# cv-stuttgart/PCFA

Measured on AMD Instinct MI355X. Metric: attack_steps_per_sec, higher is better.
Workload: dtype f32; 1 GPU; RAFT, 1 synthetic 436x1024 pair per GPU (padded 440x1024), disjoint delta, change_of_variables, delta_bound=0.005, zero target, L-BFGS max_iter=10; weights=random:1234, parallelism=pairs sharded 1/GPU, closure_launch=hipGraph replay

## Files before the change

### include/pcfa_hip.h

```cpp
#ifndef PCFA_HIP_H
#define PCFA_HIP_H

#include <stddef.h>
#include <stdint.h>

#ifdef __cplusplus
extern "C" {
#endif

#define PCFA_OK 0
#define PCFA_ERR_INVALID_ARG (-1)
#define PCFA_ERR_UNSUPPORTED (-2)
#define PCFA_ERR_WORKSPACE (-3)

#if defined(__GNUC__)
#define PCFA_API __attribute__((visibility("default")))
#else
#define PCFA_API
#endif

#define PCFA_MAX_LEVELS 8
#define PCFA_ABI_VERSION 2

#define PCFA_LOSS_AEE 0
#define PCFA_LOSS_MSE 1
#define PCFA_LOSS_COSIM 2

#define PCFA_BOX_CLIPPING 0
#define PCFA_BOX_CHANGE_OF_VARIABLES 1

PCFA_API int pcfa_abi_version(void);
PCFA_API int pcfa_timing_arm(void* start_event, void* stop_event, int nth);

PCFA_API int pcfa_null_launch(void* stream);
PCFA_API int pcfa_poison_lds(unsigned pattern, void* stream);
PCFA_API int pcfa_peek_lds(unsigned* out, int n, void* stream);
PCFA_API long long pcfa_calib_mfma_f32(float* scratch, int blocks, int iters, void* stream);
PCFA_API int pcfa_calib_copy(const float* src, float* dst, long long n_floats, void* stream);
PCFA_API const char* pcfa_status_string(int status);


PCFA_API long long pcfa_corr_slab_floats(int H, int W, int num_levels);
PCFA_API long long pcfa_corr_level_offset(int H, int W, int num_levels, int level, int* h_l, int* w_l);

PCFA_API long long pcfa_corr_tiled_index(int H, int W, int num_levels, int level, int y, int x);

PCFA_API int pcfa_corr_f2ext_fwd(const float* fmap2, float* f2ext, int B, int D, int H, int W,
                        int num_levels, void* stream);

PCFA_API int pcfa_corr_pyramid_fwd(const float* fmap1, const float* f2ext, float* pyr, int B, int D,
                          int H, int W, int num_levels, void* stream);

PCFA_API size_t pcfa_corr_pyramid_bwd_workspace_bytes(int B, int D, int H, int W, int num_levels);
PCFA_API int pcfa_corr_pyramid_bwd(const float* dpyr, const float* fmap1, const float* f2ext,
                          float* dfmap1, float* dfmap2, void* workspace, size_t workspace_bytes,
                          int B, int D, int H, int W, int num_levels, void* stream);
PCFA_API size_t pcfa_corr_pyramid_bwd_windows_workspace_bytes(int B, int D, int H, int W, int num_levels);
PCFA_API int pcfa_corr_pyramid_bwd_windows(const float* dpyr, const float* fmap1, const float* f2ext, float* dfmap1,
                                  float* dfmap2, void* workspace, size_t workspace_bytes,
                                  const float* const* coords, int n_coords, int radius, int B, int D, int H, int W,
                                  int num_levels, void* stream);

PCFA_API int pcfa_corr_lookup_fwd(const float* pyr, const float* coords, float* out, int B, int H, int W,
                         int num_levels, int radius, void* stream);

PCFA_API int pcfa_corr_lookup_bwd(float* dpyr, const float* coords, const float* grad_out, int B, int H,
                         int W, int num_levels, int radius, void* stream);

PCFA_API size_t pcfa_corr_ondemand_workspace_bytes(int B, int D, int H, int W, int num_levels);
PCFA_API int pcfa_corr_ondemand_prepare(const float* fmap1, const float* fmap2, void* workspace, int B, int D, int H,
                               int W, int num_levels, void* stream);
PCFA_API int pcfa_corr_ondemand_fwd(const void* workspace, const float* coords, float* out, int B, int D, int H, int W,
                           int num_levels, int radius, void* stream);
PCFA_API int pcfa_corr_ondemand_bwd(void* workspace, const float* coords, const float* grad_out, int accumulate, int B,
                           int D, int H, int W, int num_levels, int radius, void* stream);
PCFA_API int pcfa_corr_ondemand_finish(const void* workspace, float* dfmap1, float* dfmap2, int B, int D, int H, int W,
                              int num_levels, void* stream);

PCFA_API int pcfa_corr_ondemand_fwd_tiled(const void* workspace, const float* coords, float* out, int B, int D, int H,
                                 int W, int num_levels, int radius, void* stream);
PCFA_API int pcfa_corr_ondemand_bwd_tiled(void* workspace, const float* coords, const float* grad_out, int accumulate,
                                 int B, int D, int H, int W, int num_levels, int radius, void* stream);
PCFA_API int pcfa_corr_ondemand_tile_geometry(int* tile_w, int* tile_h, int* max_positions);
PCFA_API int pcfa_corr_ondemand_tile_routes(const void* workspace, int B, int D, int H, int W, int num_levels,
                                   int* counts, void* stream);

PCFA_API size_t pcfa_gemm_f32_workspace_bytes(int M, int N, int batch, int splits);
PCFA_API int pcfa_gemm_f32(const float* A, const float* B, float* C, int M, int N, int K, long long lda, long long ldb,
                  long long ldc, int a_kmajor, int b_kmajor, int batch, long long bsA, long long bsB, long long bsC,
                  float alpha, int splits, void* workspace, size_t workspace_bytes, void* stream);
PCFA_API size_t pcfa_gemm_bf16x3_workspace_bytes(int M, int N, int batch, int splits);
PCFA_API int pcfa_gemm_bf16x3(const float* A, const float* B, float* C, int M, int N, int K, long long lda,
                     long long ldb, long long ldc, int a_kmajor, int b_kmajor, int batch, long long bsA, long long bsB,
                     long long bsC, float alpha, int splits, void* workspace, size_t workspace_bytes, void* stream);
PCFA_API int pcfa_corr_pyramid_fwd_bf16x3(const float* fmap1, const float* f2ext, float* pyr, int B, int D, int H,
                                 int W, int num_levels, void* stream);
PCFA_API int pcfa_softmax_rows_fwd(const float* x, float* y, long long rows, int cols, void* stream);
PCFA_API int pcfa_softmax_rows_bwd(const float* y, const float* grad_y, float* grad_x, long long rows, int cols,
                          void* stream);

PCFA_API int pcfa_attn_stream_lse(const float* q, const float* k, float* lse, int BH, int N, int d, float scale,
                         void* stream);
PCFA_API int pcfa_attn_stream_fwd(const float* q, const float* k, const float* v, const float* lse, float* out, int BH,
                         int N, int d, float scale, void* stream);
PCFA_API int pcfa_attn_stream_dv(const float* q, const float* k, const float* g, const float* lse, float* dv, int BH,
                        int N, int d, float scale, void* stream);
PCFA_API int pcfa_attn_stream_delta(const float* g, const float* out, float* delta, long long rows, int d,
                           int accumulate, void* stream);
PCFA_API int pcfa_attn_stream_dqk(const float* q, const float* k, const float* lse, const float* G, const float* V,
                         const float* delta, float* dq, float* dk, int BH, int N, int d, int n, float scale,
                         void* stream);

PCFA_API long long pcfa_lookup_convc1_packed_floats(int Cout);
PCFA_API int pcfa_lookup_convc1_pack_weights(const float* weight, float* packed, int Cout, int Cin, void* stream);
PCFA_API int pcfa_lookup_convc1_fwd(const float* pyr, const float* coords, const float* packed, const float* bias,
                           float* out, int B, int H, int W, int num_levels, int radius, int Cout, int relu,
                           void* stream);
PCFA_API int pcfa_lookup_convc1_bwd(float* dpyr, const float* coords, const float* packed, const float* out,
                           const float* grad_out, int B, int H, int W, int num_levels, int radius, int Cout,
                           int relu, void* stream);

PCFA_API int pcfa_spatial_corr_out_size(int iH, int iW, int kH, int kW, int padH, int padW, int dilH,
                               int dilW, int dH, int dW, int* oH, int* oW);
PCFA_API int pcfa_spatial_corr_fwd(const float* in1, const float* in2, float* out, int B, int C, int iH,
                          int iW, int kH, int kW, int patchH, int patchW, int padH, int padW,
                          int dilH, int dilW, int dil_patchH, int dil_patchW, int dH, int dW,
                          void* stream);
PCFA_API int pcfa_spatial_corr_bwd(const float* in1, const float* in2, const float* grad_out,
                          float* grad_in1, float* grad_in2, int B, int C, int iH, int iW, int kH,
                          int kW, int patchH, int patchW, int padH, int padW, int dilH, int dilW,
                          int dil_patchH, int dil_patchW, int dH, int dW, void* stream);

PCFA_API int pcfa_cost_volume9_fwd(const float* in1, const float* in2, float* out, int B, int C, int iH, int iW,
                          float scale, float slope, void* stream);
PCFA_API int pcfa_cost_volume9_bwd(const float* in1, const float* in2, const float* fwd_out, const float* grad_out,
                          float* grad_in1, float* grad_in2, int B, int C, int iH, int iW, float scale,
                          float slope, void* stream);

PCFA_API int pcfa_flownet_corr_out_size(int H, int W, int pad_size, int kernel_size, int max_displacement,
                                        int stride1, int stride2, int* out_channels, int* oH, int* oW);
PCFA_API int pcfa_flownet_corr_fwd(const float* in1, const float* in2, float* out, int B, int C, int H, int W,
                                   int pad_size, int kernel_size, int max_displacement, int stride1, int stride2,
                                   void* stream);
PCFA_API int pcfa_flownet_corr_bwd(const float* in1, const float* in2, const float* grad_out, float* grad_in1,
                                   float* grad_in2, int B, int C, int H, int W, int pad_size, int kernel_size,
                                   int max_displacement, int stride1, int stride2, void* stream);
PCFA_API int pcfa_resample2d_fwd(const float* in1, const float* flow, float* out, int B, int C, int iH, int iW,
                                 int H, int W, int kernel_size, int bilinear, void* stream);
PCFA_API int pcfa_resample2d_bwd(const float* in1, const float* flow, const float* grad_out, float* grad_in1,
                                 float* grad_flow, int B, int C, int iH, int iW, int H, int W, int kernel_size,
                                 int bilinear, void* stream);
PCFA_API int pcfa_channelnorm_fwd(const float* in, float* out, int B, int C, long long plane, int norm_deg,
                                  void* stream);
PCFA_API int pcfa_channelnorm_bwd(const float* in, const float* out, const float* grad_out, float* grad_in, int B,
                                  int C, long long plane, int norm_deg, void* stream);


PCFA_API int pcfa_box_transform_fwd(const float* image, const float* delta, float* out, int B,
                           long long n_per_item, int change_of_variables, double eps_box,
                           float scale, void* stream);
PCFA_API int pcfa_box_transform_bwd(const float* image, const float* delta, const float* grad_out,
                           float* grad_image, float* grad_delta, int B, long long n_per_item,
                           int change_of_variables, double eps_box, float scale, void* stream);

PCFA_API int pcfa_pm1_pair_fwd(const float* image1, const float* image2, float* pair, float* ctx, int B, long long n,
                               void* stream);
PCFA_API int pcfa_pm1_pair_bwd(const float* grad_pair, const float* grad_ctx, float* grad_image1, float* grad_image2, int B,
                               long long n, void* stream);

PCFA_API int pcfa_extract_deltas_fwd(const float* nw_input, const float* image, float* delta,
                            long long n, int change_of_variables, double eps_box, void* stream);
PCFA_API int pcfa_extract_deltas_bwd(const float* nw_input, const float* grad_delta, float* grad_nw_input,
                            long long n, int change_of_variables, double eps_box, void* stream);

PCFA_API int pcfa_extract_deltas_joint_fwd(const float* nw_delta, const float* images_max,
                                  const float* images_min, float* delta, long long n,
                                  void* stream);
PCFA_API int pcfa_extract_deltas_joint_bwd(const float* nw_delta, const float* images_max,
                                  const float* images_min, const float* grad_delta,
                                  float* grad_nw_delta, long long n, void* stream);

PCFA_API int pcfa_fgsm_step(float* x1, float* x2, const float* g1, const float* g2, const float* img1, const float* img2,
                            float* d1, float* d2, float epsilon, int joint, long long n, void* stream);
PCFA_API int pcfa_fgsm_step_max_threads(void);

PCFA_API size_t pcfa_flow_loss_workspace_bytes(void);
PCFA_API int pcfa_flow_loss_fwd(const float* pred, const long long pred_strides[4], const float* target,
                       const long long target_strides[4], int B, int H, int W,
                       const float* delta1, long long n1, const float* delta2, long long n2,
                       float delta_bound, float mu, int f_type, float* out_scalars,
                       void* workspace, void* stream);
PCFA_API int pcfa_flow_loss_bwd(const float* pred, const long long pred_strides[4], const float* target,
                       const long long target_strides[4], int B, int H, int W,
                       const float* delta1, long long n1, const float* delta2, long long n2,
                       float mu, int f_type, int joint, const float* fwd_scalars,
                       const float* grad_loss, float* grad_pred, float* grad_delta1,
                       float* grad_delta2, void* stream);

PCFA_API int pcfa_gru_gates_fwd(const float* zc, const float* rc, const float* h, const float* bias_z,
                       const float* bias_r, const float* add_z, const float* add_r, float* z, float* r,
                       float* rh, long long n, int plane, int channels, void* stream);
PCFA_API int pcfa_gru_gates_bwd(const float* z, const float* r, const float* h, const float* dz, const float* drh,
                       float* dzc, float* drc, float* dh, long long n, void* stream);
PCFA_API int pcfa_gru_gates_bwd_acc(const float* z, const float* r, const float* h, const float* dz, const float* drh,
                           const float* dh_in, float* dzc, float* drc, float* dh, long long n, void* stream);
PCFA_API int pcfa_gru_update_fwd(const float* z, const float* qc, const float* h, const float* bias_q,
                        const float* add_q, float* q, float* hnew, long long n, int plane, int channels,
                        void* stream);
PCFA_API int pcfa_gru_update_bwd(const float* z, const float* q, const float* h, const float* g, float* dz,
                        float* dqc, float* dh, long long n, void* stream);

PCFA_API long long pcfa_sepconv5_packed_floats(int Cout, int Cin);
PCFA_API int pcfa_sepconv5_algo(int use_winograd);
PCFA_API int pcfa_sepconv5_uses_winograd(int B, int Ca, int Cb, int Cout, int H, int W, int vertical);
PCFA_API int pcfa_sepconv5_pack_weights(const float* w, float* fwd_packed, float* bwd_packed, int Cout, int Cin,
                               void* stream);
PCFA_API int pcfa_sepconv5_fwd(const float* in_a, int Ca, const float* in_b, int Cb, const float* w_packed,
                      float* out, int B, int Cout, int H, int W, int vertical, void* stream);

PCFA_API int pcfa_sepconv5_fwd_split(const float* in_a, int Ca, const float* in_b, int Cb, const float* w_packed,
                            float* out_a, int Cout_a, int accumulate_a, float* out_b, int accumulate_b, int B,
                            int Cout, int H, int W, int vertical, void* stream);
PCFA_API int pcfa_sepconv5_fwd_split_masked(const float* in_a, int Ca, const float* in_b, int Cb, const float* w_packed,
                                   float* out_a, int Cout_a, int accumulate_a, float* out_b, int accumulate_b,
                                   const float* mask_b, int mask_channels, int B, int Cout, int H, int W,
                                   int vertical, void* stream);

PCFA_API int pcfa_sepconv5_gru_gates_fwd(const float* h, int C, const float* rest, int Cr, const float* w_packed,
                                const float* add_zr, float* z, float* r, float* rh, int B, int H, int W,
                                int vertical, void* stream);
PCFA_API int pcfa_sepconv5_gru_update_fwd(const float* rh, int C, const float* rest, int Cr, const float* w_packed,
                                 const float* add_q, const float* z, const float* h, float* q, float* hnew, int B,
                                 int H, int W, int vertical, void* stream);
PCFA_API int pcfa_sepconv5_gru_gates_bwd(const float* dqc, int C, int Cr, const float* w_packed_bwd, const float* z,
                                const float* r, const float* h, const float* dz, const float* dh_in, float* dzr,
                                float* dh, float* d_rest, int accumulate_rest, int B, int H, int W, int vertical,
                                void* stream);
PCFA_API int pcfa_sepconv5_gru_update_bwd(const float* dzr, int C, int Cr, const float* w_packed_bwd, const float* dh_acc,
                                 const float* z_prev, const float* q_prev, const float* h_prev, float* dz_prev,
                                 float* dqc_prev, float* dh_prev, float* d_rest, int B, int H, int W, int vertical,
                                 void* stream);

PCFA_API long long pcfa_conv3x3_packed_floats(int K, int N);
PCFA_API int pcfa_conv3x3_pack_weights(const float* w, float* fwd_packed, float* bwd_packed, int Cout, int Cin,
                              void* stream);
PCFA_API int pcfa_conv3x3_fwd(const float* x, const float* packed, const float* bias, float* out, int B, int K, int N,
                     int H, int W, int relu, void* stream);
PCFA_API int pcfa_conv3x3_act_fwd(const float* x, const float* packed, const float* bias, float* out, int B, int K,
                         int N, int H, int W, int act, float slope, void* stream);
PCFA_API int pcfa_leaky_relu_fwd(const float* x, float* y, float slope, long long n, void* stream);
PCFA_API int pcfa_leaky_relu_bwd(const float* out, const float* grad_out, float* grad_x, float slope, long long n,
                        void* stream);
PCFA_API int pcfa_conv3x3_act_fwd_pair(const float* x, const float* packed, const float* bias, float* out, int K, int N,
                              const float* x2, const float* packed2, const float* bias2, float* out2, int K2, int N2,
                              int H, int W, int act, float slope, void* stream);
PCFA_API int pcfa_conv3x3_fused_bwd(const float* g, const float* packed_bwd, const float* mask, const float* addend,
                           float* grad_in, int B, int K, int N, int H, int W, void* stream);
PCFA_API int pcfa_conv3x3_masked_fwd(const float* x, const float* packed, const float* mask, float* out, int B, int K,
                            int N, int H, int W, void* stream);
PCFA_API int pcfa_conv3x3_algo(int B, int K, int N, int H, int W);
PCFA_API size_t pcfa_conv3x3_workspace_bytes(int B, int K, int N, int H, int W);
PCFA_API int pcfa_conv3x3_run(const float* x, const float* packed, const float* bias, const float* mask,
                     const float* addend, float* out, int B, int K, int N, int H, int W, int act, float slope,
                     int mask_channels, void* workspace, size_t workspace_bytes, void* stream);

PCFA_API int pcfa_bias_relu_fwd(const float* x, const float* bias, float* out, long long n, int plane, int channels,
                       void* stream);
PCFA_API int pcfa_relu_bwd(const float* out, const float* grad_out, float* grad_x, long long n, void* stream);
PCFA_API int pcfa_relu_bwd2(const float* out, const float* out2, const float* grad_out, float* grad_x, float* grad_x2,
                   long long n, void* stream);

PCFA_API int pcfa_conv_fewin_fwd(const float* x, const float* w, const float* bias, float* out, int B, int Cin, int N,
                                 int H, int W, int ksize, int relu, void* stream);
PCFA_API long long pcfa_conv_fewin_packed_floats(int Cin, int N, int ksize);
PCFA_API int pcfa_conv_fewin_pack(const float* w, float* packed, int Cin, int N, int ksize, void* stream);
PCFA_API int pcfa_conv_fewin_packed_fwd(const float* x, const float* packed, const float* bias, float* out, int B, int Cin,
                               int N, int H, int W, int ksize, int relu, void* stream);

PCFA_API int pcfa_conv_s2_supported(int Cin, int N, int ksize, int H, int W);
PCFA_API long long pcfa_conv_s2_packed_floats(int Cin, int N, int ksize);
PCFA_API int pcfa_conv_s2_pack(const float* w, float* packed, int Cin, int N, int ksize, void* stream);
PCFA_API int pcfa_conv_s2_fwd(const float* x, const float* packed, const float* bias, float* out, int B, int Cin, int N,
                              int H, int W, int ksize, int act, float slope, void* stream);
PCFA_API int pcfa_conv_s2_bwd_supported(int Cin, int N, int ksize, int H, int W);
PCFA_API long long pcfa_conv_s2_bwd_packed_floats(int Cin, int N, int ksize);
PCFA_API int pcfa_conv_s2_bwd_pack(const float* w, float* packed, int Cin, int N, int ksize, void* stream);
PCFA_API int pcfa_conv_s2_bwd(const float* grad_out, const float* packed, float* grad_x, int B, int Cin, int N, int H, int W,
                              int ksize, void* stream);
PCFA_API long long pcfa_conv_s2_ds_packed_floats(int Cin, int N);
PCFA_API int pcfa_conv_s2_ds_pack(const float* w, const float* wd, float* packed, int Cin, int N, void* stream);
PCFA_API int pcfa_conv_s2_ds_fwd(const float* x, const float* packed, const float* bias, float* out, const float* bias_d,
                                 float* out_d, int B, int Cin, int N, int H, int W, int act, float slope, void* stream);
PCFA_API long long pcfa_conv_s2_ds_bwd_packed_floats(int Cin, int N);
PCFA_API int pcfa_conv_s2_ds_bwd_pack(const float* w, const float* wd, float* packed, int Cin, int N, void* stream);
PCFA_API int pcfa_conv_s2_ds_bwd(const float* grad_out, const float* grad_out_d, const float* packed, float* grad_x, int B,
                                 int Cin, int N, int H, int W, void* stream);

PCFA_API int pcfa_pwc_warp_fwd(const float* x, const float* flo, float* out, int B, int C, int H, int W,
                               float mask_threshold, float flow_scale, void* stream);
PCFA_API int pcfa_pwc_warp_bwd(const float* x, const float* flo, const float* grad_out, float* grad_x,
                               float* grad_flo, int B, int C, int H, int W, float mask_threshold, float flow_scale,
                               void* stream);
PCFA_API size_t pcfa_pwc_warp_bwd_det_workspace_bytes(int B, int C, int H, int W);
PCFA_API int pcfa_pwc_warp_bwd_det(const float* x, const float* flo, const float* grad_out, float* grad_x,
                          float* grad_flo, void* workspace, size_t workspace_bytes, int B, int C, int H, int W,
                          float mask_threshold, float flow_scale, void* stream);

PCFA_API int pcfa_spynet_warp_fwd(const float* x, const float* flo, const float* hor, const float* ver, float* out, int B,
                                  int C, int H, int W, float sx, float sy, void* stream);
PCFA_API size_t pcfa_spynet_warp_bwd_workspace_bytes(int B, int C, int H, int W);
PCFA_API int pcfa_spynet_warp_bwd(const float* x, const float* flo, const float* hor, const float* ver,
                                  const float* grad_out, float* grad_x, float* grad_flo, void* workspace,
                                  size_t workspace_bytes, int B, int C, int H, int W, float sx, float sy, void* stream);

PCFA_API int pcfa_conv7x7_tile(int Cout, int* mt, int* cot);
PCFA_API long long pcfa_conv7x7_packed_floats(int Cin, int Cout);
PCFA_API int pcfa_conv7x7(const float* x, const float* mask, const float* packed, const float* bias, const float* addend,
                          float* out, int B, int Cin, int Cout, int H, int W, int relu, void* stream);

PCFA_API int pcfa_conv_gather_tile(int Cout, int* mt, int* cot);
PCFA_API int pcfa_conv_gather_supported(int stride, int taps, int npar);
PCFA_API long long pcfa_conv_gather_packed_floats(int Cin, int Cout, int taps, int npar);
PCFA_API int pcfa_conv_gather(const float* x, const float* mask, float mask_slope, const float* packed, const float* bias,
                              float* out, int B, int Cin, int H, int W, int Cout, int OH, int OW, int stride, int taps,
                              int npar, int off0, int off1, int act, float slope, void* stream);

PCFA_API size_t pcfa_resample2d_bwd_det_workspace_bytes(int B, int C, int H, int W);
PCFA_API int pcfa_resample2d_bwd_det(const float* in1, const float* flow, const float* grad_out, float* grad_in1,
                                     float* grad_flow, void* workspace, size_t workspace_bytes, int B, int C, int H, int W,
                                     void* stream);

PCFA_API int pcfa_upsample_nearest4_fwd(const float* in, float* out, int planes, int H, int W, float s, int div,
                                        void* stream);
PCFA_API int pcfa_upsample_nearest4_bwd(const float* grad_out, float* grad_in, int planes, int H, int W, float s, int div,
                                        void* stream);

PCFA_API size_t pcfa_conv3x3_fewout_workspace_bytes(int B, int K, int N, int H, int W);
PCFA_API int pcfa_conv3x3_fewout_fwd(const float* x, const float* w, const float* bias, float* out, void* workspace,
                                     int B, int K, int N, int H, int W, void* stream);
PCFA_API int pcfa_conv3x3_fewout_bwd(const float* grad_out, const float* w, const float* addend, float* grad_x, int B,
                                     int K, int N, int H, int W, void* stream);

PCFA_API size_t pcfa_deconv4s2_fewout_workspace_bytes(int B, int K, int N, int H, int W);
PCFA_API int pcfa_deconv4s2_fewout_fwd(const float* x, const float* w, const float* bias, float* out, void* workspace,
                                       int B, int K, int N, int H, int W, void* stream);
PCFA_API int pcfa_deconv4s2_fewout_bwd(const float* grad_out, const float* w, float* grad_x, int B, int K, int N, int H,
                                       int W, void* stream);

PCFA_API int pcfa_upsample_bilinear_fwd(const float* in, float* out, int planes, int H, int W, int factor, float mul,
                                        void* stream);
PCFA_API int pcfa_upsample_bilinear_bwd(const float* grad_out, float* grad_in, int planes, int H, int W, int factor,
                                        float mul, void* stream);

PCFA_API size_t pcfa_instnorm_workspace_bytes(int planes, long long plane);
PCFA_API int pcfa_instnorm_fwd(const float* x, float* y, float* mean_rstd, void* workspace, int planes,
                               long long plane, float eps, int relu, void* stream);
PCFA_API int pcfa_instnorm_bwd(const float* x, const float* mean_rstd, const float* grad_out, float* grad_x,
                               void* workspace, int planes, long long plane, int relu, void* stream);
PCFA_API int pcfa_add_relu_fwd(const float* a, const float* b, float* out, long long n, void* stream);
PCFA_API int pcfa_convex_upsample_fwd(const float* flow, const float* mask, float* out, int N, int H, int W, void* stream);
PCFA_API long long pcfa_convex_upsample_workspace_floats(int N, int H, int W);
PCFA_API int pcfa_convex_upsample_bwd(const float* flow, const float* mask, const float* grad_out, float* grad_flow,
                             float* grad_mask, float* workspace, int N, int H, int W, void* stream);

PCFA_API int pcfa_flow_step(const float* coords1, const float* delta, const float* coords0, float* coords1_new,
                   float* flow_new, long long n, void* stream);

PCFA_API int pcfa_sum_n(const float* const* srcs, int n, float* out, long long numel, void* stream);

PCFA_API int pcfa_avg_epe(const float* flow1, const long long strides1[4], const float* flow2,
                 const long long strides2[4], int B, int H, int W, float* out, void* workspace,
                 void* stream);
PCFA_API int pcfa_sum_squares(const float* x, long long n, float* out, void* workspace, void* stream);

PCFA_API size_t pcfa_lbfgs_workspace_floats(void);
PCFA_API int pcfa_lbfgs_pair(const float* g, float* g_prev, const float* d, float t, float* y_out, float* s_out,
                             float* scal4, float* workspace, int update_prev, long long n, void* stream);
PCFA_API int pcfa_lbfgs_direction(const float* g, const float* S, const float* Y, const float* ro, const float* H,
                                  float* al, float* d, float* workspace, int first, int count, int capacity,
                                  long long ld, long long n, void* stream);

PCFA_API size_t pcfa_lbfgs_gram_state_bytes(int capacity);
PCFA_API size_t pcfa_lbfgs_gram_workspace_bytes(int capacity, long long ld);
PCFA_API int pcfa_lbfgs_gram_reset(void* state, int capacity, void* stream);
PCFA_API int pcfa_lbfgs_gram_update(const float* g, float* g_prev, const float* d, float t, float* S, float* Y,
                                    void* state, void* workspace, int capacity, long long ld, void* stream);
PCFA_API int pcfa_lbfgs_gram_direction(const float* g, const float* S, const float* Y, void* state, float* d,
                                       float* out_gtd_dmax, void* workspace, int capacity, long long ld, void* stream);

#ifdef __cplusplus
}
#endif
#endif
```

### pcfa_amd/_hip.py

```python
import ctypes
import os
from ctypes import c_char_p, c_double, c_float, c_int, c_longlong, c_size_t, c_uint, c_void_p, POINTER

ABI_VERSION = 2
LIB_PATH = os.environ.get("PCFA_HIP_LIB") or os.path.join(os.path.dirname(os.path.abspath(__file__)), "lib",
                                                          "libpcfa_hip.so")

PCFA_LOSS = {"aee": 0, "mse": 1, "cosim": 2}


class HipLibraryError(RuntimeError):
    pass


_P = c_void_p
_S4 = POINTER(c_longlong)

SIGNATURES = {
    "pcfa_abi_version": (c_int, []),
    "pcfa_timing_arm": (c_int, [_P, _P, c_int]),
    "pcfa_null_launch": (c_int, [_P]),
    "pcfa_poison_lds": (c_int, [c_uint, _P]),
    "pcfa_peek_lds": (c_int, [_P, c_int, _P]),
    "pcfa_calib_mfma_f32": (c_longlong, [_P, c_int, c_int, _P]),
    "pcfa_calib_copy": (c_int, [_P, _P, c_longlong, _P]),
    "pcfa_status_string": (c_char_p, [c_int]),
    "pcfa_corr_slab_floats": (c_longlong, [c_int, c_int, c_int]),
    "pcfa_corr_level_offset": (c_longlong, [c_int, c_int, c_int, c_int, POINTER(c_int), POINTER(c_int)]),
    "pcfa_corr_tiled_index": (c_longlong, [c_int, c_int, c_int, c_int, c_int, c_int]),
    "pcfa_corr_f2ext_fwd": (c_int, [_P, _P, c_int, c_int, c_int, c_int, c_int, _P]),
    "pcfa_corr_pyramid_fwd": (c_int, [_P, _P, _P, c_int, c_int, c_int, c_int, c_int, _P]),
    "pcfa_corr_pyramid_bwd_workspace_bytes": (c_size_t, [c_int, c_int, c_int, c_int, c_int]),
    "pcfa_corr_pyramid_bwd": (c_int, [_P, _P, _P, _P, _P, _P, c_size_t, c_int, c_int, c_int, c_int, c_int, _P]),
    "pcfa_corr_pyramid_bwd_windows_workspace_bytes": (c_size_t, [c_int, c_int, c_int, c_int, c_int]),
    "pcfa_corr_pyramid_bwd_windows": (c_int, [_P, _P, _P, _P, _P, _P, c_size_t, POINTER(c_void_p), c_int, c_int, c_int,
                                              c_int, c_int, c_int, c_int, _P]),
    "pcfa_corr_lookup_fwd": (c_int, [_P, _P, _P, c_int, c_int, c_int, c_int, c_int, _P]),
    "pcfa_corr_lookup_bwd": (c_int, [_P, _P, _P, c_int, c_int, c_int, c_int, c_int, _P]),
    "pcfa_corr_ondemand_workspace_bytes": (c_size_t, [c_int, c_int, c_int, c_int, c_int]),
    "pcfa_corr_ondemand_prepare": (c_int, [_P, _P, _P, c_int, c_int, c_int, c_int, c_int, _P]),
    "pcfa_corr_ondemand_fwd": (c_int, [_P, _P, _P, c_int, c_int, c_int, c_int, c_int, c_int, _P]),
    "pcfa_corr_ondemand_bwd": (c_int, [_P, _P, _P, c_int, c_int, c_int, c_int, c_int, c_int, c_int, _P]),
    "pcfa_corr_ondemand_finish": (c_int, [_P, _P, _P, c_int, c_int, c_int, c_int, c_int, _P]),
    "pcfa_corr_ondemand_fwd_tiled": (c_int, [_P, _P, _P, c_int, c_int, c_int, c_int, c_int, c_int, _P]),
    "pcfa_corr_ondemand_bwd_tiled": (c_int, [_P, _P, _P, c_int, c_int, c_int, c_int, c_int, c_int, c_int, _P]),
    "pcfa_corr_ondemand_tile_geometry": (c_int, [POINTER(c_int), POINTER(c_int), POINTER(c_int)]),
    "pcfa_corr_ondemand_tile_routes": (c_int, [_P, c_int, c_int, c_int, c_int, c_int, _P, _P]),
    "pcfa_gemm_f32_workspace_bytes": (c_size_t, [c_int, c_int, c_int, c_int]),
    "pcfa_gemm_f32": (c_int, [_P, _P, _P, c_int, c_int, c_int, c_longlong, c_longlong, c_longlong, c_int, c_int, c_int,
                              c_longlong, c_longlong, c_longlong, c_float, c_int, _P, c_size_t, _P]),
    "pcfa_gemm_bf16x3_workspace_bytes": (c_size_t, [c_int, c_int, c_int, c_int]),
    "pcfa_gemm_bf16x3": (c_int, [_P, _P, _P, c_int, c_int, c_int, c_longlong, c_longlong, c_longlong, c_int, c_int,
                                 c_int, c_longlong, c_longlong, c_longlong, c_float, c_int, _P, c_size_t, _P]),
    "pcfa_corr_pyramid_fwd_bf16x3": (c_int, [_P, _P, _P, c_int, c_int, c_int, c_int, c_int, _P]),
    "pcfa_softmax_rows_fwd": (c_int, [_P, _P, c_longlong, c_int, _P]),
    "pcfa_softmax_rows_bwd": (c_int, [_P, _P, _P, c_longlong, c_int, _P]),
    "pcfa_attn_stream_lse": (c_int, [_P, _P, _P, c_int, c_int, c_int, c_float, _P]),
    "pcfa_attn_stream_fwd": (c_int, [_P, _P, _P, _P, _P, c_int, c_int, c_int, c_float, _P]),
    "pcfa_attn_stream_dv": (c_int, [_P, _P, _P, _P, _P, c_int, c_int, c_int, c_float, _P]),
    "pcfa_attn_stream_delta": (c_int, [_P, _P, _P, c_longlong, c_int, c_int, _P]),
    "pcfa_attn_stream_dqk": (c_int, [_P, _P, _P, _P, _P, _P, _P, _P, c_int, c_int, c_int, c_int, c_float, _P]),
    "pcfa_lookup_convc1_packed_floats": (c_longlong, [c_int]),
    "pcfa_lookup_convc1_pack_weights": (c_int, [_P, _P, c_int, c_int, _P]),
    "pcfa_lookup_convc1_fwd": (c_int, [_P, _P, _P, _P, _P, c_int, c_int, c_int, c_int, c_int, c_int, c_int, _P]),
    "pcfa_lookup_convc1_bwd": (c_int, [_P, _P, _P, _P, _P, c_int, c_int, c_int, c_int, c_int, c_int, c_int, _P]),
    "pcfa_spatial_corr_out_size": (c_int, [c_int] * 10 + [POINTER(c_int), POINTER(c_int)]),
    "pcfa_spatial_corr_fwd": (c_int, [_P, _P, _P] + [c_int] * 16 + [_P]),
    "pcfa_spatial_corr_bwd": (c_int, [_P, _P, _P, _P, _P] + [c_int] * 16 + [_P]),
    "pcfa_cost_volume9_fwd": (c_int, [_P, _P, _P, c_int, c_int, c_int, c_int, c_float, c_float, _P]),
    "pcfa_cost_volume9_bwd": (c_int, [_P, _P, _P, _P, _P, _P, c_int, c_int, c_int, c_int, c_float, c_float, _P]),
    "pcfa_flownet_corr_out_size": (c_int, [c_int] * 7 + [POINTER(c_int)] * 3),
    "pcfa_flownet_corr_fwd": (c_int, [_P, _P, _P] + [c_int] * 9 + [_P]),
    "pcfa_flownet_corr_bwd": (c_int, [_P, _P, _P, _P, _P] + [c_int] * 9 + [_P]),
    "pcfa_resample2d_fwd": (c_int, [_P, _P, _P] + [c_int] * 8 + [_P]),
    "pcfa_resample2d_bwd": (c_int, [_P, _P, _P, _P, _P] + [c_int] * 8 + [_P]),
    "pcfa_channelnorm_fwd": (c_int, [_P, _P, c_int, c_int, c_longlong, c_int, _P]),
    "pcfa_channelnorm_bwd": (c_int, [_P, _P, _P, _P, c_int, c_int, c_longlong, c_int, _P]),
    "pcfa_box_transform_fwd": (c_int, [_P, _P, _P, c_int, c_longlong, c_int, c_double, c_float, _P]),
    "pcfa_box_transform_bwd": (c_int, [_P, _P, _P, _P, _P, c_int, c_longlong, c_int, c_double, c_float, _P]),
    "pcfa_pm1_pair_fwd": (c_int, [_P, _P, _P, _P, c_int, c_longlong, _P]),
    "pcfa_pm1_pair_bwd": (c_int, [_P, _P, _P, _P, c_int, c_longlong, _P]),
    "pcfa_extract_deltas_fwd": (c_int, [_P, _P, _P, c_longlong, c_int, c_double, _P]),
    "pcfa_extract_deltas_bwd": (c_int, [_P, _P, _P, c_longlong, c_int, c_double, _P]),
    "pcfa_extract_deltas_joint_fwd": (c_int, [_P, _P, _P, _P, c_longlong, _P]),
    "pcfa_extract_deltas_joint_bwd": (c_int, [_P, _P, _P, _P, _P, c_longlong, _P]),
    "pcfa_fgsm_step": (c_int, [_P] * 8 + [c_float, c_int, c_longlong, _P]),
    "pcfa_fgsm_step_max_threads": (c_int, []),
    "pcfa_flow_loss_workspace_bytes": (c_size_t, []),
    "pcfa_flow_loss_fwd": (c_int, [_P, _S4, _P, _S4, c_int, c_int, c_int, _P, c_longlong, _P, c_longlong,
                                   c_float, c_float, c_int, _P, _P, _P]),
    "pcfa_flow_loss_bwd": (c_int, [_P, _S4, _P, _S4, c_int, c_int, c_int, _P, c_longlong, _P, c_longlong,
                                   c_float, c_int, c_int, _P, _P, _P, _P, _P, _P]),
    "pcfa_gru_gates_fwd": (c_int, [_P] * 10 + [c_longlong, c_int, c_int, _P]),
    "pcfa_gru_gates_bwd": (c_int, [_P] * 8 + [c_longlong, _P]),
    "pcfa_gru_update_fwd": (c_int, [_P] * 7 + [c_longlong, c_int, c_int, _P]),
    "pcfa_gru_update_bwd": (c_int, [_P] * 7 + [c_longlong, _P]),
    "pcfa_sepconv5_packed_floats": (c_longlong, [c_int, c_int]),
    "pcfa_sepconv5_algo": (c_int, [c_int]),
    "pcfa_sepconv5_uses_winograd": (c_int, [c_int] * 7),
    "pcfa_sepconv5_pack_weights": (c_int, [_P, _P, _P, c_int, c_int, _P]),
    "pcfa_sepconv5_fwd": (c_int, [_P, c_int, _P, c_int, _P, _P, c_int, c_int, c_int, c_int, c_int, _P]),
    "pcfa_sepconv5_fwd_split": (c_int, [_P, c_int, _P, c_int, _P, _P, c_int, c_int, _P, c_int, c_int, c_int, c_int, c_int,
                                        c_int, _P]),
    "pcfa_gru_gates_bwd_acc": (c_int, [_P, _P, _P, _P, _P, _P, _P, _P, _P, c_longlong, _P]),
    "pcfa_sepconv5_fwd_split_masked": (c_int, [_P, c_int, _P, c_int, _P, _P, c_int, c_int, _P, c_int, _P, c_int, c_int,
                                               c_int, c_int, c_int, c_int, _P]),
    "pcfa_sepconv5_gru_gates_fwd": (c_int, [_P, c_int, _P, c_int, _P, _P, _P, _P, _P, c_int, c_int, c_int, c_int, _P]),
    "pcfa_sepconv5_gru_update_fwd": (c_int, [_P, c_int, _P, c_int, _P, _P, _P, _P, _P, _P, c_int, c_int, c_int, c_int, _P]),
    "pcfa_sepconv5_gru_gates_bwd": (c_int, [_P, c_int, c_int, _P, _P, _P, _P, _P, _P, _P, _P, _P, c_int, c_int, c_int,
                                            c_int, c_int, _P]),
    "pcfa_sepconv5_gru_update_bwd": (c_int, [_P, c_int, c_int, _P, _P, _P, _P, _P, _P, _P, _P, _P, c_int, c_int, c_int,
                                             c_int, _P]),
    "pcfa_convex_upsample_fwd": (c_int, [_P, _P, _P, c_int, c_int, c_int, _P]),
    "pcfa_convex_upsample_workspace_floats": (c_longlong, [c_int, c_int, c_int]),
    "pcfa_convex_upsample_bwd": (c_int, [_P, _P, _P, _P, _P, _P, c_int, c_int, c_int, _P]),
    "pcfa_flow_step": (c_int, [_P, _P, _P, _P, _P, c_longlong, _P]),
    "pcfa_conv3x3_act_fwd_pair": (c_int, [_P, _P, _P, _P, c_int, c_int, _P, _P, _P, _P, c_int, c_int, c_int, c_int, c_int,
                                          c_float, _P]),
    "pcfa_relu_bwd2": (c_int, [_P, _P, _P, _P, _P, c_longlong, _P]),
    "pcfa_conv3x3_fused_bwd": (c_int, [_P, _P, _P, _P, _P, c_int, c_int, c_int, c_int, c_int, _P]),
    "pcfa_conv3x3_masked_fwd": (c_int, [_P, _P, _P, _P, c_int, c_int, c_int, c_int, c_int, _P]),
    "pcfa_conv3x3_algo": (c_int, [c_int] * 5),
    "pcfa_conv3x3_workspace_bytes": (c_size_t, [c_int] * 5),
    "pcfa_conv3x3_run": (c_int, [_P] * 6 + [c_int] * 6 + [c_float, c_int, _P, c_size_t, _P]),
    "pcfa_conv3x3_packed_floats": (c_longlong, [c_int, c_int]),
    "pcfa_conv3x3_pack_weights": (c_int, [_P, _P, _P, c_int, c_int, _P]),
    "pcfa_conv3x3_fwd": (c_int, [_P, _P, _P, _P, c_int, c_int, c_int, c_int, c_int, c_int, _P]),
    "pcfa_conv3x3_act_fwd": (c_int, [_P, _P, _P, _P, c_int, c_int, c_int, c_int, c_int, c_int, c_float, _P]),
    "pcfa_leaky_relu_fwd": (c_int, [_P, _P, c_float, c_longlong, _P]),
    "pcfa_leaky_relu_bwd": (c_int, [_P, _P, _P, c_float, c_longlong, _P]),
    "pcfa_lbfgs_gram_state_bytes": (c_size_t, [c_int]),
    "pcfa_lbfgs_gram_workspace_bytes": (c_size_t, [c_int, c_longlong]),
    "pcfa_lbfgs_gram_reset": (c_int, [_P, c_int, _P]),
    "pcfa_lbfgs_gram_update": (c_int, [_P, _P, _P, c_float, _P, _P, _P, _P, c_int, c_longlong, _P]),
    "pcfa_lbfgs_gram_direction": (c_int, [_P, _P, _P, _P, _P, _P, _P, c_int, c_longlong, _P]),
    "pcfa_lbfgs_workspace_floats": (c_size_t, []),
    "pcfa_lbfgs_pair": (c_int, [_P, _P, _P, c_float, _P, _P, _P, _P, c_int, c_longlong, _P]),
    "pcfa_lbfgs_direction": (c_int, [_P, _P, _P, _P, _P, _P, _P, _P, c_int, c_int, c_int, c_longlong, c_longlong,
                                     _P]),
    "pcfa_bias_relu_fwd": (c_int, [_P, _P, _P, c_longlong, c_int, c_int, _P]),
    "pcfa_relu_bwd": (c_int, [_P, _P, _P, c_longlong, _P]),
    "pcfa_conv_fewin_packed_floats": (c_longlong, [c_int, c_int, c_int]),
    "pcfa_conv_s2_supported": (c_int, [c_int, c_int, c_int, c_int, c_int]),
    "pcfa_conv_s2_packed_floats": (c_longlong, [c_int, c_int, c_int]),
    "pcfa_conv_s2_pack": (c_int, [_P, _P, c_int, c_int, c_int, _P]),
    "pcfa_conv_s2_fwd": (c_int, [_P, _P, _P, _P, c_int, c_int, c_int, c_int, c_int, c_int, c_int, c_float, _P]),
    "pcfa_conv_s2_bwd_supported": (c_int, [c_int, c_int, c_int, c_int, c_int]),
    "pcfa_conv_s2_bwd_packed_floats": (c_longlong, [c_int, c_int, c_int]),
    "pcfa_conv_s2_bwd_pack": (c_int, [_P, _P, c_int, c_int, c_int, _P]),
    "pcfa_conv_s2_bwd": (c_int, [_P, _P, _P, c_int, c_int, c_int, c_int, c_int, c_int, _P]),
    "pcfa_conv_s2_ds_packed_floats": (c_longlong, [c_int, c_int]),
    "pcfa_conv_s2_ds_pack": (c_int, [_P, _P, _P, c_int, c_int, _P]),
    "pcfa_conv_s2_ds_fwd": (c_int, [_P, _P, _P, _P, _P, _P, c_int, c_int, c_int, c_int, c_int, c_int, c_float, _P]),
    "pcfa_conv_s2_ds_bwd_packed_floats": (c_longlong, [c_int, c_int]),
    "pcfa_conv_s2_ds_bwd_pack": (c_int, [_P, _P, _P, c_int, c_int, _P]),
    "pcfa_conv_s2_ds_bwd": (c_int, [_P, _P, _P, _P, c_int, c_int, c_int, c_int, c_int, _P]),
    "pcfa_conv_fewin_pack": (c_int, [_P, _P, c_int, c_int, c_int, _P]),
    "pcfa_conv_fewin_packed_fwd": (c_int, [_P, _P, _P, _P, c_int, c_int, c_int, c_int, c_int, c_int, c_int, _P]),
    "pcfa_conv_fewin_fwd": (c_int, [_P, _P, _P, _P, c_int, c_int, c_int, c_int, c_int, c_int, c_int, _P]),
    "pcfa_pwc_warp_fwd": (c_int, [_P, _P, _P, c_int, c_int, c_int, c_int, c_float, c_float, _P]),
    "pcfa_pwc_warp_bwd": (c_int, [_P, _P, _P, _P, _P, c_int, c_int, c_int, c_int, c_float, c_float, _P]),
    "pcfa_pwc_warp_bwd_det_workspace_bytes": (c_size_t, [c_int, c_int, c_int, c_int]),
    "pcfa_pwc_warp_bwd_det": (c_int, [_P, _P, _P, _P, _P, _P, c_size_t, c_int, c_int, c_int, c_int, c_float, c_float, _P]),
    "pcfa_conv3x3_fewout_workspace_bytes": (c_size_t, [c_int, c_int, c_int, c_int, c_int]),
    "pcfa_conv3x3_fewout_fwd": (c_int, [_P, _P, _P, _P, _P, c_int, c_int, c_int, c_int, c_int, _P]),
    "pcfa_conv3x3_fewout_bwd": (c_int, [_P, _P, _P, _P, c_int, c_int, c_int, c_int, c_int, _P]),
    "pcfa_deconv4s2_fewout_workspace_bytes": (c_size_t, [c_int, c_int, c_int, c_int, c_int]),
    "pcfa_deconv4s2_fewout_fwd": (c_int, [_P, _P, _P, _P, _P, c_int, c_int, c_int, c_int, c_int, _P]),
    "pcfa_deconv4s2_fewout_bwd": (c_int, [_P, _P, _P, c_int, c_int, c_int, c_int, c_int, _P]),
    "pcfa_spynet_warp_fwd": (c_int, [_P, _P, _P, _P, _P, c_int, c_int, c_int, c_int, c_float, c_float, _P]),
    "pcfa_spynet_warp_bwd_workspace_bytes": (c_size_t, [c_int, c_int, c_int, c_int]),
    "pcfa_spynet_warp_bwd": (c_int, [_P, _P, _P, _P, _P, _P, _P, _P, c_size_t, c_int, c_int, c_int, c_int, c_float, c_float,
                                     _P]),
    "pcfa_conv7x7_tile": (c_int, [c_int, POINTER(c_int), POINTER(c_int)]),
    "pcfa_conv7x7_packed_floats": (c_longlong, [c_int, c_int]),
    "pcfa_conv7x7": (c_int, [_P, _P, _P, _P, _P, _P, c_int, c_int, c_int, c_int, c_int, c_int, _P]),
    "pcfa_conv_gather_tile": (c_int, [c_int, POINTER(c_int), POINTER(c_int)]),
    "pcfa_conv_gather_supported": (c_int, [c_int, c_int, c_int]),
    "pcfa_conv_gather_packed_floats": (c_longlong, [c_int, c_int, c_int, c_int]),
    "pcfa_conv_gather": (c_int, [_P, _P, c_float, _P, _P, _P] + [c_int] * 12 + [c_int, c_float, _P]),
    "pcfa_resample2d_bwd_det_workspace_bytes": (c_size_t, [c_int, c_int, c_int, c_int]),
    "pcfa_resample2d_bwd_det": (c_int, [_P, _P, _P, _P, _P, _P, c_size_t, c_int, c_int, c_int, c_int, _P]),
    "pcfa_upsample_nearest4_fwd": (c_int, [_P, _P, c_int, c_int, c_int, c_float, c_int, _P]),
    "pcfa_upsample_nearest4_bwd": (c_int, [_P, _P, c_int, c_int, c_int, c_float, c_int, _P]),
    "pcfa_upsample_bilinear_fwd": (c_int, [_P, _P, c_int, c_int, c_int, c_int, c_float, _P]),
    "pcfa_upsample_bilinear_bwd": (c_int, [_P, _P, c_int, c_int, c_int, c_int, c_float, _P]),
    "pcfa_instnorm_workspace_bytes": (c_size_t, [c_int, c_longlong]),
    "pcfa_instnorm_fwd": (c_int, [_P, _P, _P, _P, c_int, c_longlong, c_float, c_int, _P]),
    "pcfa_instnorm_bwd": (c_int, [_P, _P, _P, _P, _P, c_int, c_longlong, c_int, _P]),
    "pcfa_add_relu_fwd": (c_int, [_P, _P, _P, c_longlong, _P]),
    "pcfa_sum_n": (c_int, [POINTER(c_void_p), c_int, _P, c_longlong, _P]),
    "pcfa_avg_epe": (c_int, [_P, _S4, _P, _S4, c_int, c_int, c_int, _P, _P, _P]),
    "pcfa_sum_squares": (c_int, [_P, c_longlong, _P, _P, _P]),
}

_lib = None


def load(path=None):
    global _lib
    if _lib is not None and path is None:
        return _lib
    p = path or LIB_PATH
    if not os.path.exists(p):
        raise HipLibraryError(
            "libpcfa_hip.so not found at %s -- build it with `python -c 'import __graft_entry__ as g; g.build()'` "
            "or `make -C pcfa_amd/csrc`. pcfa_amd has no CPU fallback." % p)
    try:
        lib = ctypes.CDLL(p)
    except OSError as e:
        raise HipLibraryError("cannot load %s: %s" % (p, e))
    for name, (res, args) in SIGNATURES.items():
        try:
            fn = getattr(lib, name)
        except AttributeError:
            raise HipLibraryError("%s does not export %s (stale build?)" % (p, name))
        fn.restype = res
        fn.argtypes = args
    v = lib.pcfa_abi_version()
    if v != ABI_VERSION:
        raise HipLibraryError("ABI version mismatch: library %d, binding %d" % (v, ABI_VERSION))
    if path is None:
        _lib = lib
    return lib


def check(status, what):
    if status != 0:
        msg = load().pcfa_status_string(status)
        raise RuntimeError("%s failed: %s (status %d)" % (what, msg.decode() if msg else "?", status))


def strides4(t):
    return (c_longlong * 4)(*t.stride())
```

### pcfa_amd/config.py

```python
import dataclasses
import os


def _env_bool(name, default):
    v = os.environ.get(name)
    return default if v is None else v not in ("0", "", "false", "False")


@dataclasses.dataclass(frozen=True)
class Config:
    fused_lookup: bool = True
    overlap_encoders: bool = False
    conv_s2: bool = True
    conv_s2_bwd: bool = True
    fused_downsample: bool = True
    defer_relu: bool = True
    pyramid_bwd_windows: bool = True
    gma_gemm: str = "lib"
    gma_attention: str = "materialised"
    conv1x1: str = "lib"
    corr: str = "all_pairs"
    ondemand_lookup: str = "per_query"
    mfma: str = "f32"
    dilated_as_subgrids: tuple = (2, 4, 8, 16)
    deconv_fewout: bool = True
    defer_leaky: bool = True
    dense_block_fused_masks: bool = True
    warp_bwd_deterministic: bool = True
    pwc_fold_glue: bool = True
    spynet_ops: str = "lib"
    flownet2_ops: str = "lib"
    reuse_pair_graphs: bool = True
    max_cached_shapes: int = 4

    @classmethod
    def from_env(cls):
        return cls(fused_lookup=_env_bool("PCFA_FUSED_LOOKUP", True),
                   overlap_encoders=_env_bool("PCFA_OVERLAP_ENCODERS", False),
                   defer_relu=_env_bool("PCFA_DEFER_RELU", True),
                   gma_gemm=os.environ.get("PCFA_GMA_GEMM", "lib"),
                   gma_attention=os.environ.get("PCFA_GMA_ATTENTION", "materialised"),
                   conv1x1=os.environ.get("PCFA_CONV1X1", "lib"),
                   corr=os.environ.get("PCFA_CORR", "all_pairs"),
                   ondemand_lookup=os.environ.get("PCFA_ONDEMAND_LOOKUP", "per_query"),
                   mfma=os.environ.get("PCFA_MFMA", "f32"),
                   spynet_ops=os.environ.get("PCFA_SPYNET_OPS", "lib"),
                   flownet2_ops=os.environ.get("PCFA_FLOWNET2_OPS", "lib"),
                   max_cached_shapes=int(os.environ.get("PCFA_MAX_CACHED_SHAPES", "4")))

    def __post_init__(self):
        if self.gma_gemm not in ("lib", "hip"):
            raise ValueError("Config.gma_gemm must be 'lib' or 'hip', got %r" % (self.gma_gemm,))
        if self.gma_attention not in ("materialised", "streamed"):
            raise ValueError("Config.gma_attention must be 'materialised' or 'streamed', got %r" % (self.gma_attention,))
        if self.conv1x1 not in ("lib", "hip"):
            raise ValueError("Config.conv1x1 must be 'lib' or 'hip', got %r" % (self.conv1x1,))
        if self.corr not in ("all_pairs", "on_demand"):
            raise ValueError("Config.corr must be 'all_pairs' or 'on_demand', got %r" % (self.corr,))
        if self.ondemand_lookup not in ("per_query", "tiled"):
            raise ValueError("Config.ondemand_lookup must be 'per_query' or 'tiled', got %r" % (self.ondemand_lookup,))
        if self.mfma not in ("f32", "bf16x3"):
            raise ValueError("Config.mfma must be 'f32' or 'bf16x3', got %r" % (self.mfma,))
        if self.spynet_ops not in ("lib", "hip"):
            raise ValueError("Config.spynet_ops must be 'lib' or 'hip', got %r" % (self.spynet_ops,))
        if self.flownet2_ops not in ("lib", "hip"):
            raise ValueError("Config.flownet2_ops must be 'lib' or 'hip', got %r" % (self.flownet2_ops,))
        if self.max_cached_shapes < 1:
            raise ValueError("Config.max_cached_shapes must be >= 1")


DEFAULT = Config.from_env()


def attach(model, config=None):
    config = DEFAULT if config is None else config
    if not isinstance(config, Config):
        raise TypeError("config must be a pcfa_amd.config.Config")
    for m in model.modules():
        object.__setattr__(m, "_pcfa_config", config)
    return model


def cfg(module):
    return getattr(module, "_pcfa_config", DEFAULT)
```

### pcfa_amd/csrc/conv3x3.hip

```cpp
#include "common.hpp"
#include "conv3x3_f43.hpp"
#include "conv_tail.hpp"
#include <cstdlib>

namespace {

typedef float f32x16 __attribute__((ext_vector_type(16)));

constexpr int TC = 8;
constexpr int PC = 2 * TC + 2;
constexpr int PCP = 20;
constexpr int KC = 8;
constexpr int CB = 64;

__global__ void conv3x3_pack_kernel(const float* __restrict__ w, float* __restrict__ P, int Cout, int Cin,
                                    int backward, int K, int N, int nchunk, long long total) {
  for (long long e = (long long)blockIdx.x * blockDim.x + threadIdx.x; e < total;
       e += (long long)gridDim.x * blockDim.x) {
    const int pos = (int)(e & 15), lane = (int)((e >> 4) & 63), wv = (int)((e >> 10) & 3);
    const long long blk = e >> 12;
    const int c = (int)(blk % nchunk), nb = (int)(blk / nchunk);
    const int a = pos >> 2, kpi = pos & 3;
    const int i = wv, j = a;
    const int k = 8 * c + 2 * kpi + (lane >> 5), n = 32 * nb + (lane & 31);
    float g[3][3];
#pragma unroll
    for (int p = 0; p < 3; ++p)
#pragma unroll
      for (int q = 0; q < 3; ++q) {
        float v = 0.f;
        if (n < N && k < K) v = backward ? w[(((long long)k * Cin + n) * 3 + (2 - p)) * 3 + (2 - q)]
                                         : w[(((long long)n * Cin + k) * 3 + p) * 3 + q];
        g[p][q] = v;
      }
    float r[3];
#pragma unroll
    for (int q = 0; q < 3; ++q)
      r[q] = i == 0 ? g[0][q] : i == 1 ? 0.5f * (g[0][q] + g[1][q] + g[2][q])
                              : i == 2 ? 0.5f * (g[0][q] - g[1][q] + g[2][q]) : g[2][q];
    P[e] = j == 0 ? r[0] : j == 1 ? 0.5f * (r[0] + r[1] + r[2]) : j == 2 ? 0.5f * (r[0] - r[1] + r[2]) : r[2];
  }
}

#ifdef PCFA_C3_STAMPS
__device__ unsigned long long c3_stamp_sums[8];
__device__ __forceinline__ unsigned long long c3_now() {
  unsigned long long t;
  __builtin_amdgcn_sched_barrier(0);
  asm volatile("s_memtime %0\n\ts_waitcnt lgkmcnt(0)" : "=s"(t)::"memory");
  __builtin_amdgcn_sched_barrier(0);
  return t;
}
#define C3_STAMP(k)                                                                              \
  do {                                                                                           \
    const unsigned long long now_ = c3_now();                                                    \
    if (k != 0) stamp_acc[k] += now_ - stamp_prev;                                               \
    stamp_prev = now_;                                                                           \
  } while (0)
#else
#define C3_STAMP(k) do {} while (0)
#endif

struct Second {
  const float* x;
  const float* U;
  const float* bias;
  float* out;
  int K, N, nb0;
  int mask_n;
  int ksl;
  int cper;
  PcfaXcdMap xcd;
};

template <int ACT, int CBT, int MT, bool KFULL, int NRING, int KS = 1>
__global__ __launch_bounds__(256 * MT * KS) __attribute__((amdgpu_waves_per_eu(KS == 2 ? 2 : (MT == 1 && NRING == 2 && CBT == 32 ? 3 : (CBT == 64 ? 1 : 2))))) void conv3x3_winograd_kernel(
    const float* __restrict__ x, const float* __restrict__ U, const float* __restrict__ bias,
    const float* __restrict__ mask, const float* __restrict__ addend, float* __restrict__ out, int K, int N, int Npad,
    int H, int W, int blocks_x, float slope, Second second) {
  constexpr int NT = 256 * MT;
  constexpr int TR = 4 * MT, TB = TR * TC;
  constexpr int PR = 2 * TR + 2;
  constexpr int RAW = KC * PR * PCP;
  constexpr int RAW_LOADS = (KC * PR * PC + NT - 1) / NT;
  constexpr int MS = TB + 1;
  constexpr int NB = CBT / 32;
  static_assert(KS == 1 || (KS == 2 && MT == 1 && CBT == 32), "split-K rides on the 256-thread tile");
  constexpr int EPI = 16 * 16 * (TB + 1);
  constexpr int RED = KS == 2 ? 4 * 4 * 16 * 64 : 0;
  constexpr int LDS0 = 2 * KS * RAW > EPI ? 2 * KS * RAW : EPI;
  constexpr int LDSF = RED > LDS0 ? RED : LDS0;
  __shared__ __attribute__((aligned(16))) float smem[LDSF];
  const int kgrp = KS == 1 ? 0 : (int)(threadIdx.x >> 8);
  float* sRaw = smem + kgrp * 2 * RAW;

  const int tid = KS == 1 ? (int)threadIdx.x : (int)(threadIdx.x & 255);
  const int lane = tid & 63, wave = (tid >> 6) & 3, mt = tid >> 8;
  const int l31 = lane & 31, lh = lane >> 5;
  int tileblk = blockIdx.x, nby = blockIdx.y;
  if (second.xcd.a != 0 && !pcfa_xcd_item(second.xcd, (int)blockIdx.x, tileblk, nby)) return;
  const int by = tileblk / blocks_x, bx = tileblk - by * blocks_x;
  const int y0 = by * (2 * TR), x0 = bx * (2 * TC);
  if (nby >= second.nb0) {
    nby -= second.nb0;
    x = second.x;
    U = second.U;
    bias = second.bias;
    out = second.out;
    K = second.K;
    N = second.N;
    mask = nullptr;
    addend = nullptr;
  }
  const int mask_n = second.mask_n;
  const int n0 = nby * CBT;
  if (n0 >= N) return;
  const long long plane = (long long)H * W;
  const int ksl = second.ksl, img = blockIdx.z / ksl, slice = blockIdx.z - img * ksl;
  x += (long long)img * K * plane;
  out += ((long long)slice * (gridDim.z / ksl) + img) * N * plane;
  if (mask != nullptr) mask += (long long)img * N * plane;
  if (addend != nullptr) addend += (long long)img * N * plane;

  unsigned praw[RAW_LOADS];
  int rdst[RAW_LOADS];
  int rch[RAW_LOADS];
  bool rok[RAW_LOADS];
#pragma unroll
  for (int i = 0; i < RAW_LOADS; ++i) {
    const int e = tid + NT * i;
    const int ch = e / (PR * PC), rem = e - ch * (PR * PC);
    const int r = rem / PC, c = rem - r * PC;
    const int yy = y0 - 1 + r, xx = x0 - 1 + c;
    rch[i] = min(ch, KC - 1);
    rdst[i] = e < KC * PR * PC ? (ch * PR + r) * PCP + c : PC;
    rok[i] = e < KC * PR * PC && yy >= 0 && yy < H && xx >= 0 && xx < W;
    praw[i] = (unsigned)(min(max(yy, 0), H - 1) * W + min(max(xx, 0), W - 1) + (KFULL ? rch[i] * (int)plane : 0));
  }
  static_assert(CBT == 32, "the packed weight layout is per 32-channel block");
  const int nchunk = (K + KC - 1) / KC;
  const float* pu = U + (((long long)nby * nchunk * 4 + wave) * 64 + lane) * 16;

  float ring_raw[NRING][RAW_LOADS];
  float4 ring_u[NRING][4];
  auto load_u = [&](int c0, float4 (&ru)[4]) {
    const float4* q = reinterpret_cast<const float4*>(pu + (long long)(c0 / KC) * (4 * 64 * 16));
#pragma unroll
    for (int i = 0; i < 4; ++i) ru[i] = q[i];
  };
  auto load_raw = [&](int c0, float (&rraw)[RAW_LOADS]) {
    if (KFULL) {
      const unsigned xo = (unsigned)(c0 * (int)plane);
#pragma unroll
      for (int i = 0; i < RAW_LOADS; ++i)
#ifdef PCFA_C3_TIMING_NO_RAW
        rraw[i] = (float)(praw[i] + xo);
#else
        rraw[i] = x[praw[i] + xo];
#endif
    } else {
#pragma unroll
      for (int i = 0; i < RAW_LOADS; ++i)
        rraw[i] = x[praw[i] + (unsigned)(min(c0 + rch[i], K - 1) * (int)plane)];
    }
  };
  auto store_chunk = [&](int c0, int buf, const float (&rraw)[RAW_LOADS]) {
    float* sRawb = sRaw + buf * RAW;
#pragma unroll
    for (int i = 0; i < RAW_LOADS; ++i)
      sRawb[rdst[i]] = (rok[i] && (KFULL || c0 + rch[i] < K)) ? rraw[i] : 0.f;
  };
  f32x16 acc[4][NB];
#pragma unroll
  for (int a = 0; a < 4; ++a)
#pragma unroll
    for (int b = 0; b < NB; ++b)
#pragma unroll
      for (int r = 0; r < 16; ++r) acc[a][b][r] = 0.f;

  const int ra = wave == 0 ? 0 : 1, rb = wave == 3 ? 3 : 2;
  const float sa = wave == 2 ? -1.f : 1.f, sb = (wave == 1 || wave == 2) ? 1.f : -1.f;
  const int m_tile = mt * 32 + l31;
  const float* prow = sRaw + (lh * PR + 2 * (m_tile >> 3)) * PCP + 2 * (m_tile & 7);
  auto load_chunk = [&](int c0, float (&rraw)[RAW_LOADS], float4 (&ru)[4]) {
    load_u(c0, ru);
    load_raw(c0, rraw);
  };
  auto mfma_chunk = [&](int buf, const float4 (&ru)[4], auto&& mid1, auto&& mid2) {
    const float* p0 = prow + buf * RAW;
    float2 a0 = *reinterpret_cast<const float2*>(p0 + ra * PCP), a1 = *reinterpret_cast<const float2*>(p0 + ra * PCP + 2);
    float2 b0 = *reinterpret_cast<const float2*>(p0 + rb * PCP), b1 = *reinterpret_cast<const float2*>(p0 + rb * PCP + 2);
#pragma unroll
    for (int kp = 0; kp < KC; kp += 2) {
      float2 na0 = a0, na1 = a1, nb0 = b0, nb1 = b1;
      if (kp + 2 < KC) {
        const float* p = p0 + (kp + 2) * (PR * PCP);
        na0 = *reinterpret_cast<const float2*>(p + ra * PCP);
        na1 = *reinterpret_cast<const float2*>(p + ra * PCP + 2);
        nb0 = *reinterpret_cast<const float2*>(p + rb * PCP);
        nb1 = *reinterpret_cast<const float2*>(p + rb * PCP + 2);
        __builtin_amdgcn_sched_barrier(0);
      }
      const float t0 = fmaf(sb, b0.x, sa * a0.x), t1 = fmaf(sb, b0.y, sa * a0.y);
      const float t2 = fmaf(sb, b1.x, sa * a1.x), t3 = fmaf(sb, b1.y, sa * a1.y);
      const float av[4] = {t0 - t2, t1 + t2, t2 - t1, t1 - t3};
#pragma unroll
      for (int a = 0; a < 4; ++a) {
        const float bv = kp == 0 ? ru[a].x : kp == 2 ? ru[a].y : kp == 4 ? ru[a].z : ru[a].w;
        acc[a][0] = __builtin_amdgcn_mfma_f32_32x32x2f32(av[a], bv, acc[a][0], 0, 0, 0);
      }
      if (kp == 0) {
        mid1();
        __builtin_amdgcn_sched_barrier(0);
      } else if (kp == 2) {
        mid2();
        __builtin_amdgcn_sched_barrier(0);
      }
      a0 = na0; a1 = na1; b0 = nb0; b1 = nb1;
    }
  };

  const int cbeg = ksl > 1 ? slice * second.cper : 0, cend = ksl > 1 ? min(nchunk, cbeg + second.cper) : nchunk;
  const int nchunk_g = (cend - cbeg) / KS;
  auto gc0 = [&](int cl) { return (cbeg + cl * KS + kgrp) * KC; };
  const int lastc = gc0(nchunk_g - 1);
#ifdef PCFA_C3_STAMPS
  unsigned long long stamp_prev = 0, stamp_acc[5] = {0, 0, 0, 0, 0};
#endif
#pragma unroll
  for (int j = 0; j < NRING; ++j) load_chunk(min(gc0(j), lastc), ring_raw[j], ring_u[j]);
  store_chunk(gc0(0), 0, ring_raw[0]);
  __syncthreads();
  for (int cbase = 0; cbase < nchunk_g; cbase += NRING) {
#pragma unroll
    for (int j = 0; j < NRING; ++j) {
      const int c = cbase + j;
      if (c < nchunk_g) {
        const int cur = c & 1, nxt = cur ^ 1;
        C3_STAMP(0);
        mfma_chunk(cur, ring_u[j],
                   [&] {
                     store_chunk(gc0(c + 1), nxt, ring_raw[(j + 1) % NRING]);
                     load_u(min(gc0(c - 1 + NRING), lastc), ring_u[(j + NRING - 1) % NRING]);
                   },
                   [&] { load_raw(min(gc0(c + NRING), lastc), ring_raw[j]); });
        __builtin_amdgcn_sched_barrier(0);
        C3_STAMP(1);
        C3_STAMP(2);
        C3_STAMP(3);
        __syncthreads();
        C3_STAMP(4);
      }
    }
  }

#ifdef PCFA_C3_STAMPS
  if (lane == 0 && wave == 0) {
    for (int k = 1; k < 5; ++k) atomicAdd(&c3_stamp_sums[k], stamp_acc[k]);
    atomicAdd(&c3_stamp_sums[0], (unsigned long long)nchunk);
  }
#endif
  if (KS == 2) {
    float* red = smem;
    if (kgrp == 1) {
#pragma unroll
      for (int a = 0; a < 4; ++a)
#pragma unroll
        for (int r = 0; r < 16; ++r) red[((wave * 4 + a) * 16 + r) * 64 + lane] = acc[a][0][r];
    }
    __syncthreads();
    if (kgrp == 0) {
#pragma unroll
      for (int a = 0; a < 4; ++a)
#pragma unroll
        for (int r = 0; r < 16; ++r) acc[a][0][r] += red[((wave * 4 + a) * 16 + r) * 64 + lane];
    }
    __syncthreads();
  }
  const bool worker = kgrp == 0;
  static_assert(EPI == 16 * 16 * MS, "epilogue image size");
  float* sM = smem;
  const int e_tile = tid % TB, e_cl = tid / TB;
  const int e_tr = e_tile >> 3, e_tc = e_tile & 7;
  const int oy = y0 + 2 * e_tr, ox = x0 + 2 * e_tc;
#pragma unroll
  for (int pass = 0; pass < CBT / 16; ++pass) {
    const int nb = pass >> 1, half = pass & 1;
    float mk[2][4] = {{1.f, 1.f, 1.f, 1.f}, {1.f, 1.f, 1.f, 1.f}};
    float ad[2][4] = {{0.f, 0.f, 0.f, 0.f}, {0.f, 0.f, 0.f, 0.f}};
    if (addend != nullptr && worker) {
#pragma unroll
      for (int q = 0; q < 2; ++q) {
        const int n = n0 + pass * 16 + e_cl + 8 * q;
        if (n < N && oy < H && ox < W) {
          const float* ap = addend + (long long)n * plane + (long long)oy * W + ox;
          ad[q][0] = ap[0];
          if (ox + 1 < W) ad[q][1] = ap[1];
          if (oy + 1 < H) {
            ad[q][2] = ap[W];
            if (ox + 1 < W) ad[q][3] = ap[W + 1];
          }
        }
      }
    }
    if (mask != nullptr && worker) {
#pragma unroll
      for (int q = 0; q < 2; ++q) {
        const int n = n0 + pass * 16 + e_cl + 8 * q;
        if (n < N && (mask_n == 0 || n < mask_n) && oy < H && ox < W) {
          const float* mp = mask + (long long)n * plane + (long long)oy * W + ox;
          mk[q][0] = mp[0];
          if (ox + 1 < W) mk[q][1] = mp[1];
          if (oy + 1 < H) {
            mk[q][2] = mp[W];
            if (ox + 1 < W) mk[q][3] = mp[W + 1];
          }
        }
      }
    }
    if ((l31 >> 4) == half && worker) {
      const int cl = l31 & 15;
#pragma unroll
      for (int a = 0; a < 4; ++a) {
        float* m = &sM[((wave * 4 + a) * 16 + cl) * MS];
#pragma unroll
        for (int r = 0; r < 16; ++r) m[mt * 32 + (r & 3) + 8 * (r >> 2) + 4 * lh] = acc[a][nb][r];
      }
    }
    __syncthreads();
#pragma unroll
    for (int q = 0; q < 2; ++q) {
      const int cl = e_cl + 8 * q;
      const int n = n0 + pass * 16 + cl;
      float m[16];
#pragma unroll
      for (int xi = 0; xi < 16; ++xi) m[xi] = sM[(xi * 16 + cl) * MS + e_tile];
      float t0[4], t1[4];
#pragma unroll
      for (int j = 0; j < 4; ++j) {
        t0[j] = m[j] + m[4 + j] + m[8 + j];
        t1[j] = m[4 + j] - m[8 + j] - m[12 + j];
      }
      const float bv = (bias != nullptr && n < N) ? bias[n] : 0.f;
      const float y00 = t0[0] + t0[1] + t0[2] + bv, y01 = t0[1] - t0[2] - t0[3] + bv;
      const float y10 = t1[0] + t1[1] + t1[2] + bv, y11 = t1[1] - t1[2] - t1[3] + bv;
      if (n < N && oy < H && ox < W && worker) {
        const long long oo = (long long)n * plane + (long long)oy * W + ox;
        const bool mall = mask != nullptr && mask_n == 0, mpre = mask != nullptr && mask_n > 0 && n < mask_n;
        const bool add = addend != nullptr;
        const float4 y = conv_tail<ACT>(make_float4(y00, y01, y10, y11), slope, mall, mpre,
                                        [&] { return make_float4(mk[q][0], mk[q][1], mk[q][2], mk[q][3]); }, add,
                                        [&] { return make_float4(ad[q][0], ad[q][1], ad[q][2], ad[q][3]); });
        float* o = out + oo;
        o[0] = y.x;
        if (ox + 1 < W) o[1] = y.y;
        if (oy + 1 < H) {
          o[W] = y.z;
          if (ox + 1 < W) o[W + 1] = y.w;
        }
      }
    }
    __syncthreads();
  }
}

}

static long long f23_packed_floats(int K, int N) {
  return 16LL * (((long long)K + KC - 1) / KC * KC) * (((long long)N + CB - 1) / CB * CB);
}

extern "C" long long pcfa_conv3x3_packed_floats(int K, int N) {
  if (K < 1 || N < 1) return -1;
  return f23_packed_floats(K, N) + pcfa_f43_packed_floats(K, N);
}

extern "C" int pcfa_conv3x3_pack_weights(const float* w, float* fwd_packed, float* bwd_packed, int Cout, int Cin,
                                         void* stream) {
  if (!w || (!fwd_packed && !bwd_packed) || Cout < 1 || Cin < 1) return PCFA_ERR_INVALID_ARG;
  hipStream_t s = (hipStream_t)stream;
  for (int dir = 0; dir < 2; ++dir) {
    float* dst = dir == 0 ? fwd_packed : bwd_packed;
    if (!dst) continue;
    const int K = dir == 0 ? Cin : Cout, N = dir == 0 ? Cout : Cin;
    const int nchunk = (K + KC - 1) / KC;
    const long long total = f23_packed_floats(K, N);
    pcfa_launch(conv3x3_pack_kernel, dim3((unsigned)min((total + 255) / 256, 8192LL)), dim3(256), 0, s, w, dst, Cout,
                Cin, dir, K, N, nchunk, total);
    PCFA_LAUNCH_CHECK();
    const int rc = pcfa_f43_pack(w, dst + total, Cout, Cin, dir, s);
    if (rc != PCFA_OK) return rc;
  }
  return PCFA_OK;
}

__global__ void leaky_relu_bwd_kernel(const float* __restrict__ out, const float* __restrict__ g, float* __restrict__ gx,
                                      float slope, long long n) {
  for (long long i = (long long)blockIdx.x * blockDim.x + threadIdx.x; i < n; i += (long long)gridDim.x * blockDim.x)
    gx[i] = out[i] > 0.f ? g[i] : g[i] * slope;
}

__global__ void leaky_relu_fwd_kernel(const float* __restrict__ x, float* __restrict__ y, float slope, long long n) {
  for (long long i = (long long)blockIdx.x * blockDim.x + threadIdx.x; i < n; i += (long long)gridDim.x * blockDim.x)
    y[i] = act_apply<2>(x[i], slope);
}

#ifdef PCFA_C3_STAMPS
extern "C" __attribute__((visibility("default"))) int dev_c3_stamps(unsigned long long* host8, int reset) {
  if (hipMemcpyFromSymbol(host8, HIP_SYMBOL(c3_stamp_sums), 8 * sizeof(unsigned long long)) != hipSuccess) return -1;
  if (reset) {
    unsigned long long z[8] = {0, 0, 0, 0, 0, 0, 0, 0};
    if (hipMemcpyToSymbol(HIP_SYMBOL(c3_stamp_sums), z, sizeof(z)) != hipSuccess) return -1;
  }
  return 0;
}
#endif

extern "C" int pcfa_leaky_relu_fwd(const float* x, float* y, float slope, long long n, void* stream) {
  if (!x || !y || n < 1) return PCFA_ERR_INVALID_ARG;
  pcfa_launch(leaky_relu_fwd_kernel, dim3((unsigned)min((n + 255) / 256, 4096LL)), dim3(256), 0, (hipStream_t)stream, x, y,
              slope, n);
  PCFA_LAUNCH_CHECK();
  return PCFA_OK;
}

extern "C" int pcfa_leaky_relu_bwd(const float* out, const float* grad_out, float* grad_x, float slope, long long n,
                                   void* stream) {
  if (!out || !grad_out || !grad_x || n < 1) return PCFA_ERR_INVALID_ARG;
  pcfa_launch(leaky_relu_bwd_kernel, dim3((unsigned)min((n + 255) / 256, 4096LL)), dim3(256), 0, (hipStream_t)stream,
              out, grad_out, grad_x, slope, n);
  PCFA_LAUNCH_CHECK();
  return PCFA_OK;
}

static int conv3x3_launch(const float* x, const float* packed, const float* bias, const float* mask, float* out, int B,
                          int K, int N, int H, int W, int act, float slope, void* stream, const float* x2 = nullptr,
                          const float* packed2 = nullptr, const float* bias2 = nullptr, float* out2 = nullptr,
                          int K2 = 0, int N2 = 0, const float* addend = nullptr, int mask_n = 0, int ksl = 1);

extern "C" int pcfa_conv3x3_fwd(const float* x, const float* packed, const float* bias, float* out, int B, int K,
                                int N, int H, int W, int relu, void* stream) {
  return conv3x3_launch(x, packed, bias, nullptr, out, B, K, N, H, W, relu ? 1 : 0, 0.f, stream);
}

extern "C" int pcfa_conv3x3_act_fwd(const float* x, const float* packed, const float* bias, float* out, int B, int K,
                                    int N, int H, int W, int act, float slope, void* stream) {
  return conv3x3_launch(x, packed, bias, nullptr, out, B, K, N, H, W, act, slope, stream);
}

extern "C" int pcfa_conv3x3_masked_fwd(const float* x, const float* packed, const float* mask, float* out, int B, int K,
                                       int N, int H, int W, void* stream) {
  if (!mask) return PCFA_ERR_INVALID_ARG;
  return conv3x3_launch(x, packed, nullptr, mask, out, B, K, N, H, W, 0, 0.f, stream);
}

extern "C" int pcfa_conv3x3_act_fwd_pair(const float* x, const float* packed, const float* bias, float* out, int K, int N,
                                         const float* x2, const float* packed2, const float* bias2, float* out2, int K2,
                                         int N2, int H, int W, int act, float slope, void* stream) {
  if (!x2 || !packed2 || !out2 || K2 < 1 || N2 < 1 || !aligned16(packed2)) return PCFA_ERR_INVALID_ARG;
  if ((K % KC == 0) != (K2 % KC == 0)) return PCFA_ERR_UNSUPPORTED;
  if (f23_packed_floats(K2, N2) > 0x7fffffffLL || (long long)K2 * H * W > 0x7fffffffLL) return PCFA_ERR_UNSUPPORTED;
  return conv3x3_launch(x, packed, bias, nullptr, out, 1, K, N, H, W, act, slope, stream, x2, packed2, bias2, out2, K2,
                        N2);
}

extern "C" int pcfa_conv3x3_fused_bwd(const float* g, const float* packed_bwd, const float* mask, const float* addend,
                                      float* grad_in, int B, int K, int N, int H, int W, void* stream) {
  return conv3x3_launch(g, packed_bwd, nullptr, mask, grad_in, B, K, N, H, W, 0, 0.f, stream, nullptr, nullptr, nullptr,
                        nullptr, 0, 0, addend);
}

static int f23_kslices(int B, int K, int N, int H, int W) {
  static const int env = getenv("PCFA_CONV3X3_KSL") ? atoi(getenv("PCFA_CONV3X3_KSL")) : -1;
  if (env == 0 || ((long long)H * W) % 4 != 0) return 1;
  const int nchunk = (K + KC - 1) / KC;
  const long long nwg = (long long)pcfa_cdiv(W, 2 * TC) * pcfa_cdiv(H, 8) * ((N + 31) / 32) * B;
  long long want = env > 0 ? env : min(256 / max(nwg, 1LL), (long long)nchunk / 2);
  if (env < 0 && (B > 2 || (long long)H * W > 2048 || nwg > 128)) want = 1;
  if (want < 2 || nchunk < 2) return 1;
  want = min(want, (long long)nchunk);
  const int cper = (int)((nchunk + want - 1) / want);
  return (nchunk + cper - 1) / cper;
}

static bool use_f43(int B, int K, int N, int H, int W) {
  static const int forced = [] {
    const char* e = getenv("PCFA_CONV3X3_ALGO");
    if (e == nullptr) return 0;
    if (e[0] == 'r') return 4;
    return e[1] == '4' ? 43 : 23;
  }();
  if (!pcfa_f43_supported(B, K, N, H, W)) return false;
  if (forced == 43 || forced == 23) return forced == 43;
  if (B == 1) {
    const long long px = (long long)H * W;
    if (px <= 2048 && f23_kslices(B, K, N, H, W) > 1) return false;
    if (px <= 4096 && K >= 176) return true;
    if (px > 4096 && px <= 16384 && K >= 384) return true;
    if (px >= 16384 && px < 100000 && (long long)K * N >= 15000) return true;
  }
  if (forced != 4) return false;
  if (H < 24 || W < 64 || K < 16) return false;
  const int ks = pcfa_f43_ksplit(B, K, N, H, W);
  if (ks > 1) return ks == 2 && (long long)K * N >= 192LL * 256;
  return (long long)H * W >= 100000;
}

extern "C" int pcfa_conv3x3_algo(int B, int K, int N, int H, int W) {
  if (B < 1 || K < 1 || N < 1 || H < 1 || W < 1) return 0;
  return use_f43(B, K, N, H, W) ? 43 : 23;
}

extern "C" size_t pcfa_conv3x3_workspace_bytes(int B, int K, int N, int H, int W) {
  if (B < 1 || K < 1 || N < 1 || H < 1 || W < 1) return 0;
  const int ksl = f23_kslices(B, K, N, H, W);
  const size_t sliced = ksl > 1 ? (size_t)ksl * B * N * H * W * sizeof(float) : 0;
  return max(use_f43(B, K, N, H, W) ? pcfa_f43_workspace_bytes(B, K, N, H, W) : (size_t)0, sliced);
}

extern "C" int pcfa_conv3x3_run(const float* x, const float* packed, const float* bias, const float* mask,
                                const float* addend, float* out, int B, int K, int N, int H, int W, int act,
                                float slope, int mask_channels, void* workspace, size_t workspace_bytes, void* stream) {
  if (!x || !packed || !out || B < 1 || K < 1 || N < 1 || H < 1 || W < 1 || act < 0 || act > 2 || mask_channels < 0 ||
      mask_channels > N || (mask_channels > 0 && (!mask || act != 0)) || (mask && act == 2))
    return PCFA_ERR_INVALID_ARG;
  if (use_f43(B, K, N, H, W)) {
    const int rc = pcfa_f43_run(x, packed + f23_packed_floats(K, N), bias, mask, addend, out, B, K, N, H, W, act,
                                slope, mask_channels, workspace, workspace_bytes, (hipStream_t)stream);
    if (rc != PCFA_ERR_UNSUPPORTED) return rc;
  }
  const int ksl = f23_kslices(B, K, N, H, W);
  if (ksl > 1 && workspace && aligned16(workspace) && aligned16(out) && (!mask || aligned16(mask)) &&
      (!addend || aligned16(addend)) && workspace_bytes >= (size_t)ksl * B * N * H * W * sizeof(float)) {
    float* part = (float*)workspace;
    const int rc = conv3x3_launch(x, packed, nullptr, nullptr, part, B, K, N, H, W, 0, 0.f, stream, nullptr, nullptr,
                                  nullptr, nullptr, 0, 0, nullptr, 0, ksl);
    if (rc != PCFA_OK) return rc;
    return pcfa_f43_finish(part, bias, mask, addend, out, ksl, B, N, H, W, act, slope, mask_channels, (hipStream_t)stream,
                           23);
  }
  return conv3x3_launch(x, packed, bias, mask, out, B, K, N, H, W, act, slope, stream, nullptr, nullptr, nullptr,
                        nullptr, 0, 0, addend, mask_channels);
}

static int conv3x3_launch(const float* x, const float* packed, const float* bias, const float* mask, float* out, int B,
                          int K, int N, int H, int W, int act, float slope, void* stream, const float* x2,
                          const float* packed2, const float* bias2, float* out2, int K2, int N2, const float* addend,
                          int mask_n, int ksl) {
  if (act < 0 || act > 2 || mask_n < 0 || (mask_n > 0 && (act != 0 || !mask))) return PCFA_ERR_INVALID_ARG;
  if (!x || !packed || !out || B < 1 || K < 1 || N < 1 || H < 1 || W < 1 || !aligned16(packed))
    return PCFA_ERR_INVALID_ARG;
  const int Npad = (N + CB - 1) / CB * CB;
  const int blocks_x = pcfa_cdiv(W, 2 * TC), blocks_y = pcfa_cdiv(H, 8);
  const long long gx = (long long)blocks_x * blocks_y;
  if (gx > 0x7fffffffLL || B > 65535 || Npad / CB > 65535 || (long long)K * H * W > 0x7fffffffLL ||
      f23_packed_floats(K, N) > 0x7fffffffLL)
    return PCFA_ERR_UNSUPPORTED;
  dim3 grid((unsigned)gx, Npad / CB, B), block(256);
  hipStream_t s = (hipStream_t)stream;
  int mt = 1;
  if (const char* e = getenv("PCFA_CONV3X3_MT")) mt = atoi(e) == 2 ? 2 : 1;
  if (ksl > 1 || x2 != nullptr) mt = 1;
  if (mt == 2) {
    const int by2 = pcfa_cdiv(H, 16);
    grid.x = (unsigned)(blocks_x * by2);
    block.x = 512;
  }
  grid.y = Npad / 32;
  const int nchunk_all = (K + KC - 1) / KC, cper = (nchunk_all + ksl - 1) / ksl;
  if (ksl > 1) {
    if (x2 != nullptr || bias || mask || addend || act != 0 || (cper * (ksl - 1)) >= nchunk_all) return PCFA_ERR_INVALID_ARG;
    grid.z = (unsigned)(B * ksl);
    if (grid.z > 65535) return PCFA_ERR_UNSUPPORTED;
  }
  Second second{x2, packed2, bias2, out2, K2, N2, (int)grid.y, mask_n, ksl, cper, PcfaXcdMap{0, 0, 0, 0}};
  if (x2 != nullptr) {
    grid.y += (unsigned)((N2 + CB - 1) / CB * CB / 32);
    if (grid.y > 65535) return PCFA_ERR_UNSUPPORTED;
  }
  const long long nwg = (long long)grid.x * grid.y * grid.z;
  static const bool xcd_on = !(getenv("PCFA_XCD_MAP") && atoi(getenv("PCFA_XCD_MAP")) == 0);
  if (xcd_on && mt == 1 && (long long)grid.x * grid.y >= 1024) {
    second.xcd = pcfa_xcd_pick((int)grid.x, (int)grid.y, 4.0 * K * H * W, 4.0 * 16 * K * 32 * grid.y);
    if (second.xcd.a != 0) {
      grid.x = pcfa_xcd_grid(second.xcd);
      grid.y = 1;
    }
  }
#define PCFA_C3_ARGS grid, block, 0, s, x, packed, bias, mask, addend, out, K, N, Npad, H, W, blocks_x, slope, second
#define PCFA_C3_LAUNCH(MT_, KF_, NR_)                                                              \
  do {                                                                                             \
    if (act == 1) pcfa_launch(conv3x3_winograd_kernel<1, 32, MT_, KF_, NR_>, PCFA_C3_ARGS);        \
    else if (act == 2) pcfa_launch(conv3x3_winograd_kernel<2, 32, MT_, KF_, NR_>, PCFA_C3_ARGS);   \
    else pcfa_launch(conv3x3_winograd_kernel<0, 32, MT_, KF_, NR_>, PCFA_C3_ARGS);                 \
  } while (0)
  const bool kfull = K % KC == 0;
  static const int ks_env = getenv("PCFA_CONV3X3_KS") ? atoi(getenv("PCFA_CONV3X3_KS")) : 0;
  if (ksl == 1 && mt == 1 && x2 == nullptr && K % (2 * KC) == 0 && (ks_env ? ks_env == 2 : nwg <= 256)) {
    block.x = 512;
    if (act == 1) pcfa_launch(conv3x3_winograd_kernel<1, 32, 1, true, 2, 2>, PCFA_C3_ARGS);
    else if (act == 2) pcfa_launch(conv3x3_winograd_kernel<2, 32, 1, true, 2, 2>, PCFA_C3_ARGS);
    else pcfa_launch(conv3x3_winograd_kernel<0, 32, 1, true, 2, 2>, PCFA_C3_ARGS);
    PCFA_LAUNCH_CHECK();
    return PCFA_OK;
  }
  int deep = 0;
  if (const char* e = getenv("PCFA_CONV3X3_RING")) deep = atoi(e) == 3;
  if (mt == 2) {
    if (kfull) PCFA_C3_LAUNCH(2, true, 2); else PCFA_C3_LAUNCH(2, false, 2);
  } else if (deep) {
    if (kfull) PCFA_C3_LAUNCH(1, true, 3); else PCFA_C3_LAUNCH(1, false, 3);
  } else {
    if (kfull) PCFA_C3_LAUNCH(1, true, 2); else PCFA_C3_LAUNCH(1, false, 2);
  }
#undef PCFA_C3_LAUNCH
#undef PCFA_C3_ARGS
  PCFA_LAUNCH_CHECK();
  return PCFA_OK;
}
```

### pcfa_amd/nets/raft.py

```python

import torch
import torch.nn as nn
import torch.nn.functional as F

from .. import ops
from ..config import cfg


def _norm(kind, planes):
    if kind == 'batch':
        return nn.BatchNorm2d(planes)
    if kind == 'instance':
        return nn.InstanceNorm2d(planes)
    if kind == 'group':
        return nn.GroupNorm(num_groups=planes // 8, num_channels=planes)
    if kind == 'none':
        return nn.Sequential()
    raise ValueError("unknown norm_fn %r" % kind)


def _fold_batchnorm(conv, bn, cache, tag):
    tensors = (conv.weight, conv.bias, bn.weight, bn.bias, bn.running_mean, bn.running_var)
    key = tuple((t.data_ptr(), t._version) for t in tensors if t is not None) + (conv.weight.device,)
    hit = cache.get(tag)
    if hit is None or hit[0] != key:
        with torch.no_grad():
            s = torch.rsqrt(bn.running_var + bn.eps)
            if bn.weight is not None:
                s = s * bn.weight
            b = -bn.running_mean if conv.bias is None else conv.bias - bn.running_mean
            b = b * s
            if bn.bias is not None:
                b = b + bn.bias
            hit = (key, (conv.weight * s[:, None, None, None]).contiguous(), b.contiguous())
        cache[tag] = hit
    return hit[1], hit[2]




def _conv_norm(conv, norm, x, relu, cache, tag, skip=False, grad_premasked=False, mask_input_grad=False):
    frozen = not (conv.weight.requires_grad or (conv.bias is not None and conv.bias.requires_grad))
    if (frozen and isinstance(norm, nn.BatchNorm2d) and not norm.training and norm.track_running_stats
            and not (norm.affine and (norm.weight.requires_grad or norm.bias.requires_grad))):
        w, b = _fold_batchnorm(conv, norm, cache, tag)
        if _is_plain3x3(conv):
            return ops.get().conv3x3(x, w, b, relu, skip=skip, grad_premasked=grad_premasked,
                                     mask_input_grad=mask_input_grad)
        assert not (skip or grad_premasked or mask_input_grad)
        if _is_stride2(conv, x, cfg(conv)):
            return ops.get().conv_s2(x, w, b, relu, own_bwd=cfg(conv).conv_s2_bwd)
        if relu:
            return ops.get().bias_relu(conv._conv_forward(x, w, None), b)
        return conv._conv_forward(x, w, b)
    if (frozen and isinstance(norm, nn.InstanceNorm2d) and not norm.affine and not norm.track_running_stats):
        xs = None
        if _is_plain3x3(conv):
            y = ops.get().conv3x3(x, conv.weight, None, False, skip=skip)
            if skip:
                y, xs = y
        elif _is_stride2(conv, x, cfg(conv)):
            assert not skip
            y = ops.get().conv_s2(x, conv.weight, None, False, own_bwd=cfg(conv).conv_s2_bwd)
        else:
            assert not skip
            y = conv._conv_forward(x, conv.weight, None)
        y = ops.get().instance_norm_relu(y, norm.eps, relu)
        return (y, xs) if skip else y
    assert not skip
    y = norm(conv(x))
    return F.relu(y, inplace=True) if relu else y


def _is_stride2(conv, x, conf):
    k = conv.kernel_size[0]
    return (conf.conv_s2 and conv.kernel_size == (k, k) and conv.stride == (2, 2) and conv.padding == (k // 2, k // 2)
            and conv.dilation == (1, 1) and conv.groups == 1 and conv.padding_mode == "zeros"
            and ops.get().conv_s2_supported(x, conv.weight))


def _can_skip(conv, norm):
    frozen = not (conv.weight.requires_grad or (conv.bias is not None and conv.bias.requires_grad))
    if not (frozen and _is_plain3x3(conv)):
        return False
    if isinstance(norm, nn.BatchNorm2d):
        return (not norm.training and norm.track_running_stats
                and not (norm.affine and (norm.weight.requires_grad or norm.bias.requires_grad)))
    return isinstance(norm, nn.InstanceNorm2d) and not norm.affine and not norm.track_running_stats


class ResidualBlock(nn.Module):
    def __init__(self, in_planes, planes, norm_fn='group', stride=1):
        super().__init__()
        self.conv1 = nn.Conv2d(in_planes, planes, kernel_size=3, padding=1, stride=stride)
        self.conv2 = nn.Conv2d(planes, planes, kernel_size=3, padding=1)
        self.relu = nn.ReLU(inplace=True)
        self.norm1 = _norm(norm_fn, planes)
        self.norm2 = _norm(norm_fn, planes)
        self.downsample = None
        if stride != 1:
            self.norm3 = _norm(norm_fn, planes)
            self.downsample = nn.Sequential(nn.Conv2d(in_planes, planes, kernel_size=1, stride=stride), self.norm3)
        self._fold_cache = {}

    def _entry_pair(self, x):
        conv1, convd, n1, nd = self.conv1, self.downsample[0], self.norm1, self.downsample[1]
        o = ops.get()
        if not (cfg(self).fused_downsample and _all_frozen(self) and conv1.stride == (2, 2) and convd.stride == (2, 2)
                and convd.kernel_size == (1, 1) and convd.padding == (0, 0) and _is_stride2(conv1, x, cfg(self))
                and o.conv_s2_ds_supported(x, conv1.weight, convd.weight)):
            return None
        if all(isinstance(n, nn.BatchNorm2d) and not n.training and n.track_running_stats for n in (n1, nd)):
            w1, b1 = _fold_batchnorm(conv1, n1, self._fold_cache, "1")
            wd, bd = _fold_batchnorm(convd, nd, self._fold_cache, "d")
            if not o.conv_s2_ds_supported(x, w1, wd):
                return None
            return o.conv_s2_ds(x, w1, wd, b1, bd, relu=True)
        if all(isinstance(n, nn.InstanceNorm2d) and not n.affine and not n.track_running_stats for n in (n1, nd)):
            y, xd = o.conv_s2_ds(x, conv1.weight, convd.weight)
            return o.instance_norm_relu(y, n1.eps, True), o.instance_norm_relu(xd, nd.eps, False)
        return None

    def forward(self, x):
        pair = self._entry_pair(x) if self.downsample is not None else None
        if pair is not None:
            y, xd = pair
            y = _conv_norm(self.conv2, self.norm2, y, True, self._fold_cache, "2")
            return ops.get().add_relu(xd, y)
        if self.downsample is None and _all_frozen(self) and _can_skip(self.conv1, self.norm1):
            y, x = _conv_norm(self.conv1, self.norm1, x, True, self._fold_cache, "1", skip=True,
                              grad_premasked=cfg(self).defer_relu and isinstance(self.norm1, nn.BatchNorm2d) and isinstance(self.norm2, nn.BatchNorm2d)
                              and _can_skip(self.conv2, self.norm2))
        else:
            y = _conv_norm(self.conv1, self.norm1, x, True, self._fold_cache, "1")
        chain = (cfg(self).defer_relu and _all_frozen(self) and isinstance(self.norm2, nn.BatchNorm2d) and _can_skip(self.conv2, self.norm2)
                 and _can_skip(self.conv1, self.norm1) and self.downsample is None)
        y = _conv_norm(self.conv2, self.norm2, y, True, self._fold_cache, "2", grad_premasked=chain, mask_input_grad=chain)
        if self.downsample is not None:
            x = _conv_norm(self.downsample[0], self.downsample[1], x, False, self._fold_cache, "d")
        if _all_frozen(self):
            return ops.get().add_relu(x, y, b_is_relu=chain)
        return self.relu(x + y)


class BasicEncoder(nn.Module):

    def __init__(self, output_dim=128, norm_fn='batch', dropout=0.0):
        super().__init__()
        self.norm_fn = norm_fn
        self.norm1 = nn.GroupNorm(num_groups=8, num_channels=64) if norm_fn == 'group' else _norm(norm_fn, 64)
        self.conv1 = nn.Conv2d(3, 64, kernel_size=7, stride=2, padding=3)
        self.relu1 = nn.ReLU(inplace=True)
        self.layer1 = self._stage(64, 64, 1)
        self.layer2 = self._stage(64, 96, 2)
        self.layer3 = self._stage(96, 128, 2)
        self.conv2 = nn.Conv2d(128, output_dim, kernel_size=1)
        self.dropout = nn.Dropout2d(p=dropout) if dropout > 0 else None
        self._fold_cache = {}
        for m in self.modules():
            if isinstance(m, nn.Conv2d):
                nn.init.kaiming_normal_(m.weight, mode='fan_out', nonlinearity='relu')
            elif isinstance(m, (nn.BatchNorm2d, nn.InstanceNorm2d, nn.GroupNorm)):
                if m.weight is not None:
                    nn.init.constant_(m.weight, 1)
                if m.bias is not None:
                    nn.init.constant_(m.bias, 0)

    def _stage(self, cin, cout, stride):
        return nn.Sequential(ResidualBlock(cin, cout, self.norm_fn, stride=stride),
                             ResidualBlock(cout, cout, self.norm_fn, stride=1))

    def forward(self, x, split=None):
        pair = isinstance(x, (tuple, list)) or split is not None
        if split is not None:
            n = split
        elif pair:
            n = x[0].shape[0]
            x = torch.cat(x, dim=0)
        x = _conv_norm(self.conv1, self.norm1, x, True, self._fold_cache, "1")
        x = self.layer3(self.layer2(self.layer1(x)))
        x = _conv1x1(self.conv2, x, cfg(self))
        if self.training and self.dropout is not None:
            x = self.dropout(x)
        if pair:
            x = torch.split(x, [n, n], dim=0)
        return x


def _all_frozen(module):
    return not any(p.requires_grad for p in module.parameters())


def _conv_nobias(conv, x):
    return conv._conv_forward(x, conv.weight, None)


def _is_plain3x3(conv, min_out=16):
    return (conv.kernel_size == (3, 3) and conv.stride == (1, 1) and conv.padding == (1, 1) and conv.dilation == (1, 1)
            and conv.groups == 1 and conv.padding_mode == "zeros" and conv.out_channels >= min_out)


def _is_plain1x1(conv):
    return (conv.kernel_size == (1, 1) and conv.stride == (1, 1) and conv.padding == (0, 0) and conv.dilation == (1, 1)
            and conv.groups == 1)


def mfma_kw(config):
    return {} if config.mfma == "f32" else {"mfma": config.mfma}


def _conv1x1(conv, x, config):
    if config.conv1x1 == "hip" and x.is_cuda and _is_plain1x1(conv) and _frozen_conv(conv):
        return ops.get().conv1x1(x, conv.weight, conv.bias, mfma=config.mfma)
    return conv(x)


def _frozen_conv(conv):
    return not (conv.weight.requires_grad or (conv.bias is not None and conv.bias.requires_grad))


def _conv_relu(conv, x):
    if _is_plain3x3(conv) and _frozen_conv(conv):
        return ops.get().conv3x3(x, conv.weight, conv.bias, True)
    o = ops.get()
    k = conv.kernel_size[0]
    if (_frozen_conv(conv) and not x.requires_grad and conv.kernel_size == (k, k) and conv.stride == (1, 1)
            and conv.padding == (k // 2, k // 2) and conv.dilation == (1, 1) and conv.groups == 1
            and conv.padding_mode == "zeros" and (conv.in_channels, k) in o.FEWIN_SHAPES):
        return o.conv_fewin(x, conv.weight, conv.bias, True)
    return o.bias_relu(_conv_nobias(conv, x), conv.bias)


def _predict_flow(conv, x):
    if (conv.kernel_size == (3, 3) and conv.stride == (1, 1) and conv.padding == (1, 1) and conv.dilation == (1, 1)
            and conv.groups == 1 and conv.padding_mode == "zeros" and conv.out_channels <= 4 and _frozen_conv(conv)):
        return ops.get().conv3x3_fewout(x, conv.weight, conv.bias)
    return conv(x)


class FlowHead(nn.Module):
    def __init__(self, input_dim=128, hidden_dim=256):
        super().__init__()
        self.conv1 = nn.Conv2d(input_dim, hidden_dim, 3, padding=1)
        self.conv2 = nn.Conv2d(hidden_dim, 2, 3, padding=1)
        self.relu = nn.ReLU(inplace=True)

    def forward(self, x):
        return _predict_flow(self.conv2, _conv_relu(self.conv1, x))


class SepConvGRU(nn.Module):

    def __init__(self, hidden_dim=128, input_dim=192 + 128, const_dim=128):
        super().__init__()
        c = hidden_dim + input_dim
        self.hidden_dim, self.const_dim = hidden_dim, const_dim
        self.convz1 = nn.Conv2d(c, hidden_dim, (1, 5), padding=(0, 2))
        self.convr1 = nn.Conv2d(c, hidden_dim, (1, 5), padding=(0, 2))
        self.convq1 = nn.Conv2d(c, hidden_dim, (1, 5), padding=(0, 2))
        self.convz2 = nn.Conv2d(c, hidden_dim, (5, 1), padding=(2, 0))
        self.convr2 = nn.Conv2d(c, hidden_dim, (5, 1), padding=(2, 0))
        self.convq2 = nn.Conv2d(c, hidden_dim, (5, 1), padding=(2, 0))
        self._split_cache = {}

    @staticmethod
    def _half(h, x, convz, convr, convq):
        o = ops.get()
        hx = torch.cat([h, x], dim=1)
        z, rh = o.gru_gates(_conv_nobias(convz, hx), _conv_nobias(convr, hx), h, convz.bias, convr.bias)
        return o.gru_update(z, _conv_nobias(convq, torch.cat([rh, x], dim=1)), h, convq.bias)

    def forward(self, h, x):
        h = self._half(h, x, self.convz1, self.convr1, self.convq1)
        return self._half(h, x, self.convz2, self.convr2, self.convq2)

    def frozen(self):
        return not any(p.requires_grad for p in self.parameters())

    def _split(self, tag, convs):
        key = tuple((c.weight.data_ptr(), c.weight._version) for c in convs) + (convs[0].weight.device,)
        hit = self._split_cache.get(tag)
        if hit is None or hit[0] != key:
            hd, cd = self.hidden_dim, self.const_dim
            with torch.no_grad():
                w = torch.cat([c.weight for c in convs], dim=0)
                b = torch.cat([c.bias for c in convs], dim=0).contiguous()
                w_dyn = torch.cat([w[:, :hd], w[:, hd + cd:]], dim=1).contiguous()
                w_const = w[:, hd:hd + cd].contiguous()
            hit = (key, w_dyn, w_const, b)
            self._split_cache[tag] = hit
        return hit[1:]

    def precompute(self, inp):
        ctx = {}
        for tag, convs in (("zr1", (self.convz1, self.convr1)), ("q1", (self.convq1,)),
                           ("zr2", (self.convz2, self.convr2)), ("q2", (self.convq2,))):
            w_dyn, w_const, b = self._split(tag, convs)
            ctx[tag] = (w_dyn, ops.get().sepconv5(inp, None, w_const) + b.view(1, -1, 1, 1))
        return ctx

    def per_iteration(self, ctx, iters):
        fans = {tag: ops.get().fanout(p, iters) for tag, (_, p) in ctx.items()}
        return [{tag: (ctx[tag][0], fans[tag][i]) for tag in ctx} for i in range(iters)]

    def step(self, h, ctx, rest, rest_relu_channels=0):
        return ops.get().gru_step(h, rest, tuple(ctx[zr] + ctx[q] for zr, q in (("zr1", "q1"), ("zr2", "q2"))),
                                  rest_relu_channels)


class LookupRef:

    def __init__(self, corr_fn, coords):
        self.corr_fn, self.coords = corr_fn, coords

    def tensor(self):
        return self.corr_fn(self.coords)

    def conv_relu(self, conv):
        fused = getattr(self.corr_fn, "lookup_conv_relu", None)
        if fused is not None and _frozen_conv(conv) and cfg(conv).fused_lookup:
            out = fused(self.coords, conv.weight, conv.bias, True)
            if out is not None:
                return out
        x = self.tensor()
        c = cfg(conv)
        if c.corr == "on_demand" and c.conv1x1 == "hip" and x.is_cuda and _is_plain1x1(conv) and _frozen_conv(conv):
            return ops.get().bias_relu(ops.get().conv1x1(x, conv.weight, None, mfma=c.mfma), conv.bias)
        return _conv_relu(conv, x)


class BasicMotionEncoder(nn.Module):
    def __init__(self, corr_levels=4, corr_radius=4):
        super().__init__()
        cor_planes = corr_levels * (2 * corr_radius + 1) ** 2
        self.convc1 = nn.Conv2d(cor_planes, 256, 1, padding=0)
        self.convc2 = nn.Conv2d(256, 192, 3, padding=1)
        self.convf1 = nn.Conv2d(2, 128, 7, padding=3)
        self.convf2 = nn.Conv2d(128, 64, 3, padding=1)
        self.conv = nn.Conv2d(64 + 192, 128 - 2, 3, padding=1)

    RELU_CHANNELS = 128 - 2

    def can_defer_relu(self, flow):
        return (flow.shape[0] == 1 and _all_frozen(self)
                and all(_is_plain3x3(c) for c in (self.convc2, self.convf2, self.conv)))

    def forward(self, flow, corr, defer_relu=False):
        cor1 = corr.conv_relu(self.convc1) if isinstance(corr, LookupRef) else _conv_relu(self.convc1, corr)
        if self.can_defer_relu(flow):
            o = ops.get()
            flo1 = _conv_relu(self.convf1, flow)
            cf = o.conv3x3_cat([(cor1, self.convc2.weight, self.convc2.bias), (flo1, self.convf2.weight, self.convf2.bias)],
                               grad_premasked=defer_relu)
            return o.conv3x3_cat([(cf, self.conv.weight, self.conv.bias)], (flow,), grad_premasked=defer_relu,
                                 mask_input_grads=defer_relu)
        if defer_relu:
            raise RuntimeError("BasicMotionEncoder: defer_relu needs the in-place path (check can_defer_relu first)")
        cor = _conv_relu(self.convc2, cor1)
        flo = _conv_relu(self.convf2, _conv_relu(self.convf1, flow))
        out = _conv_relu(self.conv, torch.cat([cor, flo], dim=1))
        return torch.cat([out, flow], dim=1)


def _mask_head():
    return nn.Sequential(nn.Conv2d(128, 256, 3, padding=1), nn.ReLU(inplace=True), nn.Conv2d(256, 64 * 9, 1, padding=0))


def mask_logits(head, net, cache):
    c0, c2 = head[0], head[2]
    if not (_frozen_conv(c0) and _frozen_conv(c2) and _is_plain3x3(c0)):
        return .25 * head(net)
    key = (c2.weight.data_ptr(), c2.weight._version, c2.bias.data_ptr(), c2.bias._version)
    if cache.get("key") != key:
        with torch.no_grad():
            cache["key"], cache["w"], cache["b"] = key, (.25 * c2.weight).contiguous(), (.25 * c2.bias).contiguous()
    y = _conv_relu(c0, net)
    if cfg(head).conv1x1 == "hip" and y.is_cuda and _is_plain1x1(c2):
        return ops.get().conv1x1(y, cache["w"], cache["b"], mfma=cfg(head).mfma)
    return c2._conv_forward(y, cache["w"], cache["b"])


class BasicUpdateBlock(nn.Module):
    def __init__(self, corr_levels=4, corr_radius=4, hidden_dim=128):
        super().__init__()
        self.encoder = BasicMotionEncoder(corr_levels, corr_radius)
        self.gru = SepConvGRU(hidden_dim=hidden_dim, input_dim=128 + hidden_dim)
        self.flow_head = FlowHead(hidden_dim, hidden_dim=256)
        self.mask = _mask_head()
        self._mask_cache = {}

    def forward(self, net, inp, corr, flow, want_mask=True, gru_ctx=None):
        defer = cfg(self).defer_relu and gru_ctx is not None and self.encoder.can_defer_relu(flow)
        motion_features = self.encoder(flow, corr, defer_relu=defer)
        if gru_ctx is not None:
            net = self.gru.step(net, gru_ctx, motion_features, self.encoder.RELU_CHANNELS if defer else 0)
        else:
            net = self.gru(net, torch.cat([inp, motion_features], dim=1))
        delta_flow = self.flow_head(net)
        mask = mask_logits(self.mask, net, self._mask_cache) if want_mask else None
        return net, mask, delta_flow


def _f32(x):
    return x if x.dtype == torch.float64 else x.float()


def coords_grid(batch, ht, wd, device, dtype=torch.float32):
    ys, xs = torch.meshgrid(torch.arange(ht, device=device), torch.arange(wd, device=device), indexing="ij")
    return torch.stack([xs, ys], dim=0).to(dtype)[None].repeat(batch, 1, 1, 1)


def convex_upsample(flow, mask):
    return ops.get().convex_upsample(flow, mask)


class RAFT(nn.Module):
    def __init__(self, args=None):
        super().__init__()
        self.args = dict(args or {})
        if self.args.get("small", False):
            raise NotImplementedError("RAFT-small is not part of the PCFA configurations (raft_config.json: small=false)")
        self.hidden_dim = hdim = 128
        self.context_dim = cdim = 128
        self.args["corr_levels"] = 4
        self.args["corr_radius"] = 4
        self.args.setdefault("dropout", 0)
        self.fnet = BasicEncoder(output_dim=256, norm_fn='instance', dropout=self.args["dropout"])
        self.cnet = BasicEncoder(output_dim=hdim + cdim, norm_fn='batch', dropout=self.args["dropout"])
        self.update_block = BasicUpdateBlock(4, 4, hidden_dim=hdim)

    def freeze_bn(self):
        for m in self.modules():
            if isinstance(m, nn.BatchNorm2d):
                m.eval()

    def forward(self, image1, image2, iters=12, flow_init=None, upsample=True, test_mode=False):
        images12, image1 = ops.get().pm1_pair(image1, image2)
        hdim, cdim = self.hidden_dim, self.context_dim

        side = None
        if cfg(self).overlap_encoders and image1.is_cuda and hasattr(ops.get(), "side_stream"):
            main = torch.cuda.current_stream()
            side = ops.get().side_stream(image1.device)
            side.wait_stream(main)
            with torch.cuda.stream(side):
                cnet_out = self.cnet(image1)
        fmap1, fmap2 = self.fnet(images12, split=image1.shape[0])
        if cfg(self).corr == "on_demand":
            corr_fn = ops.get().OnDemandCorrBlock(_f32(fmap1), _f32(fmap2), num_levels=self.args["corr_levels"],
                                                  radius=self.args["corr_radius"], lookup=cfg(self).ondemand_lookup)
        else:
            corr_fn = ops.get().CorrBlock(_f32(fmap1), _f32(fmap2), num_levels=self.args["corr_levels"],
                                          radius=self.args["corr_radius"], bwd_windows=cfg(self).pyramid_bwd_windows,
                                          **mfma_kw(cfg(self)))
        if side is not None:
            main.wait_stream(side)
        else:
            cnet_out = self.cnet(image1)

        net, inp = torch.split(cnet_out, [hdim, cdim], dim=1)
        net, inp = torch.tanh(net), torch.relu(inp)

        N, _, H, W = image1.shape
        coords0 = coords_grid(N, H // 8, W // 8, image1.device, _f32(image1).dtype)
        coords1 = coords_grid(N, H // 8, W // 8, image1.device, _f32(image1).dtype)
        if flow_init is not None:
            coords1 = coords1 + flow_init

        gru = self.update_block.gru
        gru_ctx = gru.per_iteration(gru.precompute(inp), iters) if gru.frozen() else None
        flow_predictions = []
        flow_up = None
        flow_cur = coords1 - coords0
        for itr in range(iters):
            coords1 = coords1.detach()
            corr = LookupRef(corr_fn, coords1)
            flow = flow_cur.detach()
            need_up = (not test_mode) or itr == iters - 1
            net, up_mask, delta_flow = self.update_block(net, inp, corr, flow, want_mask=need_up,
                                                         gru_ctx=None if gru_ctx is None else gru_ctx[itr])
            coords1, flow_cur = ops.get().flow_step(coords1, delta_flow, coords0)
            if need_up:
                flow_up = convex_upsample(flow_cur, up_mask)
                flow_predictions.append(flow_up)
        if test_mode:
            return flow_cur, flow_up
        return flow_predictions
```

### pcfa_amd/ops/conv.py

```python
import ctypes
import os

import torch

from .. import _hip
from . import core
from .core import _call, _dev, _ptr, _ptr_off, cached_pack, current_lane


FEWIN_SHAPES = {(2, 7), (1, 7), (2, 5), (2, 3)}
_FEWIN_PACKED = os.environ.get("PCFA_FEWIN_PACKED", "1") != "0"


def _pack_cin_n_k(w, pack, packed_floats):
    N, Cin, k, _ = w.shape
    w = w.contiguous()
    packed = torch.empty(int(getattr(_hip.load(), packed_floats)(Cin, N, k)), device=w.device, dtype=torch.float32)
    _call(pack, _ptr(w), _ptr(packed), Cin, N, k)
    return packed


def _fewin_packed(weight):
    return cached_pack("fewin", (weight,),
                       lambda w: _pack_cin_n_k(w, "pcfa_conv_fewin_pack", "pcfa_conv_fewin_packed_floats"))


class _Conv1x1(torch.autograd.Function):

    @staticmethod
    def forward(ctx, x, w, b, mfma="f32"):
        _dev(x, w)
        if mfma not in ("f32", "bf16x3"):
            raise ValueError("conv1x1: mfma must be 'f32' or 'bf16x3', got %r" % (mfma,))
        entry = "pcfa_gemm_f32" if mfma == "f32" else "pcfa_gemm_bf16x3"
        if w.dim() != 4 or tuple(w.shape[2:]) != (1, 1) or x.dim() != 4 or x.shape[1] != w.shape[1]:
            raise ValueError("conv1x1: weight %s does not fit input %s" % (tuple(w.shape), tuple(x.shape)))
        if x.dtype != torch.float32 or w.dtype != torch.float32:
            raise ValueError("conv1x1: float32 only")
        x = x.contiguous()
        B, K, H, W = x.shape
        N, hw = w.shape[0], H * W
        w2 = w.reshape(N, K).contiguous()
        out = torch.empty((B, N, H, W), device=x.device, dtype=torch.float32)
        _call(entry, _ptr(w2), _ptr(x), _ptr(out), N, hw, K, K, hw, hw, 0, 1, B, 0, K * hw, N * hw, 1.0, 1,
              _ptr(None), ctypes.c_size_t(0))
        if b is not None:
            out.add_(b.view(1, N, 1, 1))
        ctx.save_for_backward(w2)
        ctx.dims = (B, K, N, H, W)
        ctx.entry = entry
        return out

    @staticmethod
    @torch.autograd.function.once_differentiable
    def backward(ctx, g):
        if ctx.needs_input_grad[1] or ctx.needs_input_grad[2]:
            raise RuntimeError("conv1x1 is the frozen-weight path: no weight / bias gradient")
        (w2,) = ctx.saved_tensors
        B, K, N, H, W = ctx.dims
        hw = H * W
        g = g.contiguous()
        gx = torch.empty((B, K, H, W), device=g.device, dtype=torch.float32)
        _call(ctx.entry, _ptr(w2), _ptr(g), _ptr(gx), K, hw, N, K, hw, hw, 1, 1, B, 0, N * hw, K * hw, 1.0, 1,
              _ptr(None), ctypes.c_size_t(0))
        return gx, None, None, None


def conv1x1(x, weight, bias=None, mfma="f32"):
    return _Conv1x1.apply(x, weight, bias, mfma)


def conv_fewin(x, weight, bias=None, relu=False):
    _dev(x, weight, bias)
    if x.requires_grad or weight.requires_grad or (bias is not None and bias.requires_grad):
        raise RuntimeError("conv_fewin is forward-only: input and parameters must not require gradients")
    N, Cin, kh, kw = weight.shape
    if kh != kw or (Cin, kh) not in FEWIN_SHAPES or x.shape[1] != Cin:
        raise ValueError("conv_fewin: unsupported weight %s for input %s" % (tuple(weight.shape), tuple(x.shape)))
    x = x.contiguous()
    B, _, H, W = x.shape
    out = torch.empty((B, N, H, W), device=x.device, dtype=torch.float32)
    if _FEWIN_PACKED:
        _call("pcfa_conv_fewin_packed_fwd", _ptr(x), _ptr(_fewin_packed(weight)), _ptr(bias), _ptr(out), B, Cin, N, H, W,
              kh, int(bool(relu)))
    else:
        _call("pcfa_conv_fewin_fwd", _ptr(x), _ptr(weight.contiguous()), _ptr(bias), _ptr(out), B, Cin, N, H, W, kh,
              int(bool(relu)))
    return out


def _s2_packed(weight):
    return cached_pack("s2", (weight,), lambda w: _pack_cin_n_k(w, "pcfa_conv_s2_pack", "pcfa_conv_s2_packed_floats"))


def _s2_bwd_packed(weight):
    return cached_pack("s2_bwd", (weight,),
                       lambda w: _pack_cin_n_k(w, "pcfa_conv_s2_bwd_pack", "pcfa_conv_s2_bwd_packed_floats"))


def conv_s2_supported(x, weight):
    N, Cin, kh, kw = weight.shape
    return bool(x.dim() == 4 and kh == kw and x.shape[1] == Cin and not weight.requires_grad and x.is_cuda
                and _hip.load().pcfa_conv_s2_supported(Cin, N, kh, x.shape[2], x.shape[3]))


def _act_bwd(out, g, act, slope=0.):
    if not act:
        return g
    gm = torch.empty_like(g)
    if act == 1:
        _call("pcfa_relu_bwd", _ptr(out), _ptr(g), _ptr(gm), g.numel())
    else:
        _call("pcfa_leaky_relu_bwd", _ptr(out), _ptr(g), _ptr(gm), float(slope), g.numel())
    return gm


class _ConvS2(torch.autograd.Function):
    @staticmethod
    def forward(ctx, x, weight, bias, act, slope, grad_premasked=False, own_bwd=True):
        _dev(x, weight, bias)
        ctx.grad_premasked = bool(grad_premasked)
        ctx.own_bwd = bool(own_bwd)
        x = x.contiguous()
        B, Cin, H, W = x.shape
        N, _, k, _ = weight.shape
        Ho, Wo = (H + 2 * (k // 2) - k) // 2 + 1, (W + 2 * (k // 2) - k) // 2 + 1
        out = torch.empty((B, N, Ho, Wo), device=x.device, dtype=torch.float32)
        _call("pcfa_conv_s2_fwd", _ptr(x), _ptr(_s2_packed(weight)), _ptr(bias), _ptr(out), B, Cin, N, H, W, k, act,
              float(slope))
        ctx.act, ctx.slope, ctx.xshape = act, float(slope), tuple(x.shape)
        ctx.save_for_backward(weight, out if (act and not ctx.grad_premasked) else None)
        return out

    @staticmethod
    def backward(ctx, g):
        weight, out = ctx.saved_tensors
        g = g.contiguous()
        if not ctx.grad_premasked:
            g = _act_bwd(out, g, ctx.act, ctx.slope)
        N, Cin, k, _ = weight.shape
        B, _, H, W = ctx.xshape
        if ctx.own_bwd and _hip.load().pcfa_conv_s2_bwd_supported(Cin, N, k, H, W):
            gx = torch.empty(ctx.xshape, device=g.device, dtype=torch.float32)
            _call("pcfa_conv_s2_bwd", _ptr(g), _ptr(_s2_bwd_packed(weight)), _ptr(gx), B, Cin, N, H, W, k)
        else:
            gx = torch.nn.grad.conv2d_input(ctx.xshape, weight, g, stride=2, padding=k // 2)
        return gx, None, None, None, None, None, None


def _s2_ds_packed(weight, weight_d):
    def make(w, wd):
        lib = _hip.load()
        N, Cin, _, _ = w.shape
        w, wd = w.contiguous(), wd.contiguous()
        pf = torch.empty(int(lib.pcfa_conv_s2_ds_packed_floats(Cin, N)), device=w.device, dtype=torch.float32)
        pb = torch.empty(int(lib.pcfa_conv_s2_ds_bwd_packed_floats(Cin, N)), device=w.device, dtype=torch.float32)
        _call("pcfa_conv_s2_ds_pack", _ptr(w), _ptr(wd), _ptr(pf), Cin, N)
        _call("pcfa_conv_s2_ds_bwd_pack", _ptr(w), _ptr(wd), _ptr(pb), Cin, N)
        return pf, pb
    return cached_pack("s2_ds", (weight, weight_d), make)


def conv_s2_ds_supported(x, weight, weight_d):
    N, Cin, kh, kw = weight.shape
    if not (x.dim() == 4 and x.is_cuda and (kh, kw) == (3, 3) and tuple(weight_d.shape) == (N, Cin, 1, 1)
            and x.shape[1] == Cin and not weight.requires_grad and not weight_d.requires_grad):
        return False
    lib = _hip.load()
    return bool(lib.pcfa_conv_s2_supported(Cin, N, 3, x.shape[2], x.shape[3])
                and lib.pcfa_conv_s2_bwd_supported(Cin, N, 3, x.shape[2], x.shape[3]))


class _ConvS2DS(torch.autograd.Function):
    @staticmethod
    def forward(ctx, x, weight, weight_d, bias, bias_d, act):
        _dev(x, weight, weight_d, bias, bias_d)
        x = x.contiguous()
        B, Cin, H, W = x.shape
        N = weight.shape[0]
        Ho, Wo = (H - 1) // 2 + 1, (W - 1) // 2 + 1
        out = torch.empty((B, N, Ho, Wo), device=x.device, dtype=torch.float32)
        out_d = torch.empty_like(out)
        pf, pb = _s2_ds_packed(weight, weight_d)
        _call("pcfa_conv_s2_ds_fwd", _ptr(x), _ptr(pf), _ptr(bias), _ptr(out), _ptr(bias_d), _ptr(out_d), B, Cin, N, H, W,
              act, 0.0)
        ctx.act, ctx.xshape, ctx.packed_bwd = act, tuple(x.shape), pb
        ctx.save_for_backward(out if act else None)
        return out, out_d

    @staticmethod
    def backward(ctx, g, gd):
        (out,) = ctx.saved_tensors
        B, Cin, H, W = ctx.xshape
        g = g.contiguous()
        gd = gd.contiguous()
        g = _act_bwd(out, g, ctx.act)
        gx = torch.empty(ctx.xshape, device=g.device, dtype=torch.float32)
        _call("pcfa_conv_s2_ds_bwd", _ptr(g), _ptr(gd), _ptr(ctx.packed_bwd), _ptr(gx), B, Cin, g.shape[1], H, W)
        return gx, None, None, None, None, None


def conv_s2_ds(x, weight, weight_d, bias=None, bias_d=None, relu=False):
    _dev(x, weight, weight_d, bias, bias_d)
    if not conv_s2_ds_supported(x, weight, weight_d):
        raise ValueError("conv_s2_ds: unsupported weights %s / %s for input %s"
                         % (tuple(weight.shape), tuple(weight_d.shape), tuple(x.shape)))
    if any(b is not None and b.requires_grad for b in (bias, bias_d)):
        raise RuntimeError("conv_s2_ds: frozen parameters only")
    return _ConvS2DS.apply(x, weight, weight_d, bias, bias_d, int(bool(relu)))


def conv_s2(x, weight, bias=None, relu=False, leaky_slope=None, grad_premasked=False, own_bwd=True):
    _dev(x, weight, bias)
    if weight.requires_grad or (bias is not None and bias.requires_grad):
        raise RuntimeError("conv_s2: frozen parameters only")
    if not conv_s2_supported(x, weight):
        raise ValueError("conv_s2: unsupported weight %s for input %s" % (tuple(weight.shape), tuple(x.shape)))
    act = 2 if leaky_slope is not None else int(bool(relu))
    if grad_premasked and not act:
        raise ValueError("conv_s2: grad_premasked needs an activation")
    return _ConvS2.apply(x, weight, bias, act, 0.0 if leaky_slope is None else leaky_slope, bool(grad_premasked),
                         bool(own_bwd))


class _Conv3x3FewOut(torch.autograd.Function):
    @staticmethod
    def forward(ctx, x, weight, bias, skip=False):
        _dev(x, weight, bias)
        ctx.set_materialize_grads(False)
        if weight.dim() != 4 or tuple(weight.shape[2:]) != (3, 3) or not 1 <= weight.shape[0] <= 4:
            raise ValueError("conv3x3_fewout expects a [N<=4, K, 3, 3] weight, got %s" % (tuple(weight.shape),))
        x = x.contiguous()
        B, K, H, W = x.shape
        N = weight.shape[0]
        if weight.shape[1] != K:
            raise ValueError("conv3x3_fewout: input %s does not match weight %s" % (tuple(x.shape), tuple(weight.shape)))
        w = weight.detach().contiguous()
        out = torch.empty((B, N, H, W), device=x.device, dtype=torch.float32)
        nws = int(_hip.load().pcfa_conv3x3_fewout_workspace_bytes(B, K, N, H, W))
        ws = torch.empty(nws // 4, device=x.device, dtype=torch.float32) if nws else None
        _call("pcfa_conv3x3_fewout_fwd", _ptr(x), _ptr(w), _ptr(bias), _ptr(out), _ptr(ws), B, K, N, H, W)
        ctx.save_for_backward(w)
        ctx.dims = (B, K, N, H, W)
        if skip:
            return out, x.view_as(x)
        return out

    @staticmethod
    @torch.autograd.function.once_differentiable
    def backward(ctx, g, g_skip=None):
        if ctx.needs_input_grad[1] or ctx.needs_input_grad[2]:
            raise RuntimeError("conv3x3_fewout is the frozen-weight path: no weight / bias gradient")
        if g is None:
            return g_skip, None, None, None
        (w,) = ctx.saved_tensors
        B, K, N, H, W = ctx.dims
        g = g.contiguous()
        gx = torch.empty((B, K, H, W), device=g.device, dtype=torch.float32)
        _call("pcfa_conv3x3_fewout_bwd", _ptr(g), _ptr(w), _ptr(None if g_skip is None else g_skip.contiguous()), _ptr(gx),
              B, K, N, H, W)
        return gx, None, None, None


def conv3x3_fewout(x, weight, bias=None, skip=False):
    return _Conv3x3FewOut.apply(x, weight, bias, skip)


class _InstNormRelu(torch.autograd.Function):

    @staticmethod
    def forward(ctx, x, eps, relu):
        _dev(x)
        x = x.contiguous()
        B, C, H, W = x.shape
        planes, plane = B * C, H * W
        lib = _hip.load()
        ws = torch.empty((int(lib.pcfa_instnorm_workspace_bytes(planes, plane)) + 3) // 4, device=x.device,
                         dtype=torch.float32)
        y = torch.empty_like(x)
        stats = torch.empty((planes, 2), device=x.device, dtype=torch.float32)
        _call("pcfa_instnorm_fwd", _ptr(x), _ptr(y), _ptr(stats), _ptr(ws), planes, plane, float(eps), int(bool(relu)))
        ctx.save_for_backward(x, stats)
        ctx.dims = (planes, plane, int(bool(relu)))
        return y

    @staticmethod
    @torch.autograd.function.once_differentiable
    def backward(ctx, g):
        x, stats = ctx.saved_tensors
        planes, plane, relu = ctx.dims
        g = g.contiguous()
        lib = _hip.load()
        ws = torch.empty((int(lib.pcfa_instnorm_workspace_bytes(planes, plane)) + 3) // 4, device=x.device,
                         dtype=torch.float32)
        gx = torch.empty_like(x)
        _call("pcfa_instnorm_bwd", _ptr(x), _ptr(stats), _ptr(g), _ptr(gx), _ptr(ws), planes, plane, relu)
        return gx, None, None


def instance_norm_relu(x, eps=1e-5, relu=False):
    return _InstNormRelu.apply(x, eps, relu)


class _AddRelu(torch.autograd.Function):
    @staticmethod
    def forward(ctx, a, b, b_is_relu):
        _dev(a, b)
        if a.shape != b.shape:
            raise ValueError("add_relu: shapes differ: %s vs %s" % (tuple(a.shape), tuple(b.shape)))
        a, b = a.contiguous(), b.contiguous()
        out = torch.empty_like(a)
        _call("pcfa_add_relu_fwd", _ptr(a), _ptr(b), _ptr(out), a.numel())
        ctx.b_is_relu = bool(b_is_relu)
        ctx.save_for_backward(out, *((b,) if ctx.b_is_relu else ()))
        return out

    @staticmethod
    @torch.autograd.function.once_differentiable
    def backward(ctx, g):
        out = ctx.saved_tensors[0]
        g = g.contiguous()
        gm = torch.empty_like(g)
        if ctx.b_is_relu:
            gb = torch.empty_like(g)
            _call("pcfa_relu_bwd2", _ptr(out), _ptr(ctx.saved_tensors[1]), _ptr(g), _ptr(gm), _ptr(gb), g.numel())
            return gm, gb, None
        _call("pcfa_relu_bwd", _ptr(out), _ptr(g), _ptr(gm), g.numel())
        return gm, gm, None


def add_relu(a, b, b_is_relu=False):
    return _AddRelu.apply(a, b, b_is_relu)


def _sepconv5_packed(weight):
    def make(w):
        cout, cin = w.shape[:2]
        w = w.contiguous()
        lib = _hip.load()
        fwd = torch.empty(int(lib.pcfa_sepconv5_packed_floats(cout, cin)), device=w.device, dtype=torch.float32)
        bwd = torch.empty(int(lib.pcfa_sepconv5_packed_floats(cin, cout)), device=w.device, dtype=torch.float32)
        _call("pcfa_sepconv5_pack_weights", _ptr(w), _ptr(fwd), _ptr(bwd), cout, cin)
        return fwd, bwd
    return cached_pack("sepconv5", (weight,), make)


class _SepConv5(torch.autograd.Function):
    @staticmethod
    def forward(ctx, a, b, weight):
        _dev(a, b, weight)
        if weight.dim() != 4 or tuple(weight.shape[2:]) not in ((1, 5), (5, 1)) or weight.dtype != torch.float32:
            raise ValueError("sepconv5 expects a float32 (1,5) or (5,1) Conv2d weight, got %s" % (tuple(weight.shape),))
        vertical = int(weight.shape[2] == 5)
        a = a.contiguous()
        b = None if b is None else b.contiguous()
        B, Ca, H, W = a.shape
        Cb = 0 if b is None else b.shape[1]
        cout = weight.shape[0]
        if weight.shape[1] != Ca + Cb or (b is not None and (b.shape[0], b.shape[2], b.shape[3]) != (B, H, W)):
            raise ValueError("sepconv5: operands %s / %s do not match weight %s"
                             % (tuple(a.shape), None if b is None else tuple(b.shape), tuple(weight.shape)))
        fwd, bwd = _sepconv5_packed(weight)
        out = torch.empty((B, cout, H, W), device=a.device, dtype=torch.float32)
        _call("pcfa_sepconv5_fwd", _ptr(a), Ca, _ptr(b), Cb, _ptr(fwd), _ptr(out), B, cout, H, W, vertical)
        ctx.bwd, ctx.dims = bwd, (B, Ca, Cb, cout, H, W, vertical)
        return out

    @staticmethod
    def backward(ctx, grad_out):
        if ctx.needs_input_grad[2]:
            raise RuntimeError("sepconv5 is the frozen-weight path: no weight gradient (use the module's "
                               "reference forward when training)")
        B, Ca, Cb, cout, H, W, vertical = ctx.dims
        g = grad_out.contiguous()
        gin = torch.empty((B, Ca + Cb, H, W), device=g.device, dtype=torch.float32)
        _call("pcfa_sepconv5_fwd", _ptr(g), cout, None, 0, _ptr(ctx.bwd), _ptr(gin), B, Ca + Cb, H, W, vertical)
        return gin[:, :Ca], (gin[:, Ca:] if Cb else None), None


def _conv3x3_packed(weight):
    def make(w):
        cout, cin = w.shape[:2]
        lib = _hip.load()
        w = w.contiguous()
        fwd = torch.empty(int(lib.pcfa_conv3x3_packed_floats(cin, cout)), device=w.device, dtype=torch.float32)
        bwd = torch.empty(int(lib.pcfa_conv3x3_packed_floats(cout, cin)), device=w.device, dtype=torch.float32)
        _call("pcfa_conv3x3_pack_weights", _ptr(w), _ptr(fwd), _ptr(bwd), cout, cin)
        return fwd, bwd
    return cached_pack("conv3x3", (weight,), make)


_CONV_WS = {}
_CONV_WS_RETIRED = []


_SIDE_STREAMS = {}
_SIDE_HANDLES = set()


def side_stream(device):
    idx = device.index if device.index is not None else torch.cuda.current_device()
    k = current_lane()
    s = _SIDE_STREAMS.get((idx, k))
    if s is None:
        s = _SIDE_STREAMS[(idx, k)] = core.own_stream(device, k)
        _SIDE_HANDLES.add(s.cuda_stream)
    return s


def _conv_workspace(device, nbytes):
    dev_idx = device.index if device.index is not None else torch.cuda.current_device()
    idx = (dev_idx, torch.cuda.current_stream(device).cuda_stream in _SIDE_HANDLES, current_lane())
    ws = _CONV_WS.get(idx)
    if ws is None or ws.numel() * 4 < nbytes:
        if torch.cuda.is_current_stream_capturing():
            raise RuntimeError("conv3x3 workspace would have to grow inside a graph capture (no eager warm-up of this "
                               "shape ran before it)")
        if ws is not None:
            _CONV_WS_RETIRED.append(ws)
        ws = torch.empty((nbytes + 3) // 4, device=device, dtype=torch.float32)
        _CONV_WS[idx] = ws
    return ws


def _conv3x3_run(device, x_ptr, packed, bias_ptr, mask_ptr, addend_ptr, out_ptr, B, K, N, H, W, act=0, slope=0.,
                 mask_channels=0):
    nws = int(_hip.load().pcfa_conv3x3_workspace_bytes(B, K, N, H, W))
    ws = _conv_workspace(device, nws) if nws else None
    _call("pcfa_conv3x3_run", x_ptr, _ptr(packed), bias_ptr, mask_ptr, addend_ptr, out_ptr, B, K, N, H, W, int(act),
          float(slope), int(mask_channels), _ptr(ws), nws)


class _Conv3x3(torch.autograd.Function):
    @staticmethod
    def forward(ctx, x, weight, bias, relu, slope=None, skip=False, flags=0, input_slope=0.):
        _dev(x, weight, bias)
        ctx.skip = bool(skip)
        ctx.grad_premasked, ctx.mask_input_grad = bool(flags & 1), bool(flags & 2)
        ctx.input_slope = float(input_slope)
        ctx.set_materialize_grads(False)
        if weight.dim() != 4 or tuple(weight.shape[2:]) != (3, 3) or weight.dtype != torch.float32:
            raise ValueError("conv3x3 expects a float32 3x3 Conv2d weight, got %s" % (tuple(weight.shape),))
        x = x.contiguous()
        B, K, H, W = x.shape
        N = weight.shape[0]
        if weight.shape[1] != K:
            raise ValueError("conv3x3: input %s does not match weight %s" % (tuple(x.shape), tuple(weight.shape)))
        fwd, bwd = _conv3x3_packed(weight)
        out = torch.empty((B, N, H, W), device=x.device, dtype=torch.float32)
        act = 2 if slope is not None else int(bool(relu))
        _conv3x3_run(x.device, _ptr(x), fwd, _ptr(bias), None, None, _ptr(out), B, K, N, H, W, act, float(slope or 0.))
        ctx.bwd, ctx.dims, ctx.act, ctx.slope = bwd, (B, K, N, H, W), act, float(slope or 0.)
        if ctx.grad_premasked and not act:
            raise ValueError("conv3x3: grad_premasked needs an activation (relu=True or leaky_slope)")
        ctx.save_for_backward(*(([out] if act and not ctx.grad_premasked else []) + ([x] if ctx.mask_input_grad else [])))
        if ctx.skip:
            return out, x.view_as(x)
        return out

    @staticmethod
    def backward(ctx, g, g_skip=None):
        if ctx.needs_input_grad[1] or ctx.needs_input_grad[2]:
            raise RuntimeError("conv3x3 is the frozen-weight path: no weight / bias gradient")
        B, K, N, H, W = ctx.dims
        if g is None:
            return (None if g_skip is None else g_skip), None, None, None, None, None, None, None
        g = g.contiguous()
        if ctx.act and not ctx.grad_premasked:
            g = _act_bwd(ctx.saved_tensors[0], g, ctx.act, ctx.slope)
        gin = torch.empty((B, K, H, W), device=g.device, dtype=torch.float32)
        if g_skip is not None or ctx.mask_input_grad:
            xin = ctx.saved_tensors[-1] if ctx.mask_input_grad else None
            _conv3x3_run(g.device, _ptr(g), ctx.bwd, None, _ptr(xin),
                         _ptr(None if g_skip is None else g_skip.contiguous()), _ptr(gin), B, N, K, H, W,
                         slope=ctx.input_slope if ctx.mask_input_grad else 0.)
        else:
            _conv3x3_run(g.device, _ptr(g), ctx.bwd, None, None, None, _ptr(gin), B, N, K, H, W)
        return gin, None, None, None, None, None, None, None


_PAIR_LAUNCH = os.environ.get("PCFA_CONV3X3_PAIR", "1") != "0"


class _Conv3x3Cat(torch.autograd.Function):

    @staticmethod
    def forward(ctx, n_conv, flags, *args):
        xs, ws, bs = args[0:3 * n_conv:3], args[1:3 * n_conv:3], args[2:3 * n_conv:3]
        tails = args[3 * n_conv:]
        ctx.grad_premasked, ctx.mask_input_grads = bool(flags & 1), bool(flags & 2)
        _dev(*xs, *ws, *tails)
        xs = [x.contiguous() for x in xs]
        B, _, H, W = xs[0].shape
        if B != 1:
            raise ValueError("conv3x3_cat: batch size 1 only")
        plane = H * W
        widths = [w.shape[0] for w in ws] + [t.shape[1] for t in tails]
        buf = torch.empty((1, sum(widths), H, W), device=xs[0].device, dtype=torch.float32)
        off, packs, fwds, offs = 0, [], [], []
        for x, w, b in zip(xs, ws, bs):
            if tuple(x.shape) != (1, w.shape[1], H, W) or tuple(w.shape[2:]) != (3, 3):
                raise ValueError("conv3x3_cat: input %s does not fit weight %s" % (tuple(x.shape), tuple(w.shape)))
            fwd, bwd = _conv3x3_packed(w)
            fwds.append(fwd)
            offs.append(off)
            packs.append((bwd, w.shape[1], w.shape[0], off))
            off += w.shape[0]
        lib = _hip.load()
        f23 = all(lib.pcfa_conv3x3_algo(1, w.shape[1], w.shape[0], H, W) == 23 for w in ws)
        if n_conv == 2 and (ws[0].shape[1] % 8 == 0) == (ws[1].shape[1] % 8 == 0) and _PAIR_LAUNCH and f23:
            i, j = (0, 1) if ws[0].shape[0] * ws[0].shape[1] >= ws[1].shape[0] * ws[1].shape[1] else (1, 0)
            _call("pcfa_conv3x3_act_fwd_pair", _ptr(xs[i]), _ptr(fwds[i]), _ptr(bs[i]), _ptr_off(buf, offs[i] * plane),
                  ws[i].shape[1], ws[i].shape[0], _ptr(xs[j]), _ptr(fwds[j]), _ptr(bs[j]),
                  _ptr_off(buf, offs[j] * plane), ws[j].shape[1], ws[j].shape[0], H, W, 1, 0.)
        else:
            for x, w, b, fwd, o_ in zip(xs, ws, bs, fwds, offs):
                _conv3x3_run(x.device, _ptr(x), fwd, _ptr(b), None, None, _ptr_off(buf, o_ * plane), 1, w.shape[1],
                             w.shape[0], H, W, 1, 0.)
        for t in tails:
            buf[:, off:off + t.shape[1]].copy_(t)
            off += t.shape[1]
        ctx.packs, ctx.dims, ctx.n_conv, ctx.tail_widths = packs, (H, W), n_conv, [t.shape[1] for t in tails]
        ctx.save_for_backward(buf, *(xs if ctx.mask_input_grads else ()))
        return buf

    @staticmethod
    def backward(ctx, g):
        buf = ctx.saved_tensors[0]
        H, W = ctx.dims
        plane = H * W
        g = g.contiguous()
        grads = [None, None]
        for i, (bwd, k, n, off) in enumerate(ctx.packs):
            if ctx.needs_input_grad[3 + 3 * i] or ctx.needs_input_grad[4 + 3 * i]:
                raise RuntimeError("conv3x3_cat is the frozen-weight path: no weight / bias gradient")
            gx = None
            if ctx.needs_input_grad[2 + 3 * i]:
                if ctx.grad_premasked:
                    gm = g[:, off:off + n]
                else:
                    gm = torch.empty((1, n, H, W), device=g.device, dtype=torch.float32)
                    _call("pcfa_relu_bwd", _ptr_off(buf, off * plane), _ptr_off(g, off * plane), _ptr(gm), n * plane)
                gx = torch.empty((1, k, H, W), device=g.device, dtype=torch.float32)
                if ctx.mask_input_grads:
                    _conv3x3_run(g.device, _ptr(gm), bwd, None, _ptr(ctx.saved_tensors[1 + i]), None, _ptr(gx), 1, n, k,
                                 H, W)
                else:
                    _conv3x3_run(g.device, _ptr(gm), bwd, None, None, None, _ptr(gx), 1, n, k, H, W)
            grads += [gx, None, None]
        off = sum(p[2] for p in ctx.packs)
        for j, tw in enumerate(ctx.tail_widths):
            grads.append(g[:, off:off + tw] if ctx.needs_input_grad[2 + 3 * ctx.n_conv + j] else None)
            off += tw
        return tuple(grads)


def conv3x3_cat(convs, tails=(), grad_premasked=False, mask_input_grads=False):
    flat = []
    for x, w, b in convs:
        flat += [x, w, b]
    return _Conv3x3Cat.apply(len(convs), int(bool(grad_premasked)) | 2 * int(bool(mask_input_grads)), *flat, *tails)


class _DenseBlock(torch.autograd.Function):

    @staticmethod
    def forward(ctx, slope, fused_masks, nparts, *rest):
        parts, wb = rest[:nparts], rest[nparts:]
        weights, biases = wb[0::2], wb[1::2]
        ctx.fused_masks = bool(fused_masks)
        _dev(*parts, *weights)
        x0 = parts[0]
        B, _, H, W = x0.shape
        if B != 1:
            raise ValueError("dense_block: batch size 1 only")
        if any(p.shape[0] != 1 or tuple(p.shape[2:]) != (H, W) or p.dtype != torch.float32 for p in parts):
            raise ValueError("dense_block: input parts %s do not share batch 1 / size / fp32" % ([tuple(p.shape) for p in parts],))
        ctx.part_widths = [p.shape[1] for p in parts]
        K0 = sum(ctx.part_widths)
        widths = [w.shape[0] for w in weights]
        total = K0 + sum(widths)
        buf = torch.empty((1, total, H, W), device=x0.device, dtype=torch.float32)
        plane = H * W
        start = total - K0
        if nparts == 1:
            buf[:, start:].copy_(x0)
        else:
            torch.cat(parts, 1, out=buf[:, start:])
        packs = []
        k = K0
        for w, b, n in zip(weights, biases, widths):
            if tuple(w.shape[1:]) != (k, 3, 3):
                raise ValueError("dense_block: weight %s does not fit %d input channels" % (tuple(w.shape), k))
            fwd, bwd = _conv3x3_packed(w)
            _conv3x3_run(x0.device, _ptr_off(buf, start * plane), fwd, _ptr(b), None, None,
                         _ptr_off(buf, (start - n) * plane), 1, k, n, H, W, 2, float(slope))
            packs.append((bwd, k, n, start))
            start -= n
            k += n
        ctx.packs, ctx.dims, ctx.slope = packs, (total, K0, H, W), float(slope)
        ctx.save_for_backward(buf)
        return buf

    @staticmethod
    def backward(ctx, g):
        if any(ctx.needs_input_grad[3 + len(ctx.part_widths):]):
            raise RuntimeError("dense_block is the frozen-weight path: no weight / bias gradient")
        (buf,) = ctx.saved_tensors
        total, K0, H, W = ctx.dims
        plane = H * W
        g = g.contiguous()
        gb = torch.empty_like(g)
        npk = len(ctx.packs)
        for i in range(npk - 1, -1, -1):
            bwd, k, n, start = ctx.packs[i]
            if i == npk - 1 or not ctx.fused_masks:
                gm = torch.empty((1, n, H, W), device=g.device, dtype=torch.float32)
                _call("pcfa_leaky_relu_bwd", _ptr_off(buf, (start - n) * plane),
                      _ptr_off(g if i == npk - 1 else gb, (start - n) * plane), _ptr(gm), ctx.slope, n * plane)
                gm_ptr = _ptr(gm)
            else:
                gm_ptr = _ptr_off(gb, (start - n) * plane)
            dst = _ptr_off(gb, start * plane)
            src = _ptr_off(g, start * plane) if i == npk - 1 else dst
            if i > 0 and ctx.fused_masks:
                _conv3x3_run(g.device, gm_ptr, bwd, None, _ptr_off(buf, start * plane), src, dst, 1, n, k, H, W,
                             slope=ctx.slope, mask_channels=ctx.packs[i - 1][2])
            else:
                _conv3x3_run(g.device, gm_ptr, bwd, None, None, src, dst, 1, n, k, H, W)
        grads, c0 = [], total - K0
        for wdt, need in zip(ctx.part_widths, ctx.needs_input_grad[3:]):
            grads.append(gb[:, c0:c0 + wdt] if need else None)
            c0 += wdt
        return (None, None, None) + tuple(grads) + (None,) * (2 * len(ctx.packs))


def dense_block(x, layers, slope=0.1, fused_masks=True):
    flat = []
    for w, b in layers:
        flat += [w, b]
    parts = tuple(x) if isinstance(x, (tuple, list)) else (x,)
    return _DenseBlock.apply(slope, fused_masks, len(parts), *[p.contiguous() for p in parts], *flat)


def conv3x3(x, weight, bias=None, relu=False, leaky_slope=None, skip=False, grad_premasked=False, mask_input_grad=False,
            input_slope=0.):
    return _Conv3x3.apply(x, weight, bias, relu, leaky_slope, skip,
                          int(bool(grad_premasked)) | 2 * int(bool(mask_input_grad)), float(input_slope))
```

### pcfa_amd/ops/corr.py

```python
import ctypes
import os

import torch

from .. import _hip
from . import core
from .core import _call, _dev, _note_work, _pair, _ptr, _ptr_off, _stream, cached_pack


class _CorrState:
    __slots__ = ("B", "D", "H", "W", "L", "r", "slab", "pyr", "f2ext", "dpyr", "token_grad", "coords_bwd", "bwd_windows", "mfma")


class _CorrBuild(torch.autograd.Function):

    @staticmethod
    def forward(ctx, fmap1, fmap2, state):
        lib = _hip.load()
        B, D, H, W = fmap1.shape
        f1 = fmap1.contiguous()
        f2 = fmap2.contiguous()
        slab = state.slab
        state.f2ext = torch.empty((B, D, slab), device=f1.device, dtype=torch.float32)
        state.pyr = torch.empty((B * H * W, slab), device=f1.device, dtype=torch.float32)
        _call("pcfa_corr_f2ext_fwd", _ptr(f2), _ptr(state.f2ext), B, D, H, W, state.L)
        _call("pcfa_corr_pyramid_fwd" if state.mfma == "f32" else "pcfa_corr_pyramid_fwd_bf16x3", _ptr(f1),
              _ptr(state.f2ext), _ptr(state.pyr), B, D, H, W, state.L)
        ctx.state = state
        ctx.save_for_backward(f1)
        return torch.zeros(1, device=f1.device, dtype=torch.float32)

    @staticmethod
    def backward(ctx, grad_token):
        st = ctx.state
        (f1,) = ctx.saved_tensors
        if st.dpyr is None:
            z = torch.zeros_like(f1)
            st.token_grad = None
            return z, z.clone(), None
        lib = _hip.load()
        B, D, H, W = st.B, st.D, st.H, st.W
        df1 = torch.empty_like(f1)
        df2 = torch.empty_like(f1)
        cs = st.coords_bwd if (st.coords_bwd and len(st.coords_bwd) <= 32 and st.bwd_windows and st.L <= 4) else []
        if cs:
            nbytes = lib.pcfa_corr_pyramid_bwd_windows_workspace_bytes(B, D, H, W, st.L)
            ws = torch.empty((nbytes + 3) // 4, device=f1.device, dtype=torch.float32)
            ptrs = (ctypes.c_void_p * len(cs))(*[c.data_ptr() for c in cs])
            _call("pcfa_corr_pyramid_bwd_windows", _ptr(st.dpyr), _ptr(f1), _ptr(st.f2ext), _ptr(df1), _ptr(df2), _ptr(ws),
                  ctypes.c_size_t(nbytes), ptrs, len(cs), st.r, B, D, H, W, st.L)
            if core.work_recorder() is not None:
                base = (int(lib.pcfa_corr_pyramid_bwd_workspace_bytes(B, D, H, W, st.L)) + 15) & ~15
                nbA, nbB = -(-(H * W) // 128), -(-st.slab // 128)
                seg = ws.view(torch.int32)[base // 4: base // 4 + 10 * B * (nbA + nbB)].cpu().view(-1, 10).long()
                live = torch.arange(4)[None, :] < seg[:, :1]
                k = ((seg[:, 2:9:2] - seg[:, 1:8:2]) * live).sum(1)
                dense = 2.0 * B * D * (H * W) ** 2
                _note_work("corr_pyramid_gemm_dfmap1", dense, 2.0 * D * 128 * float(k[:B * nbA].sum()))
                _note_work("corr_pyramid_gemm_df2ext", dense, 2.0 * D * 128 * float(k[B * nbA:].sum()))
        else:
            nbytes = lib.pcfa_corr_pyramid_bwd_workspace_bytes(B, D, H, W, st.L)
            ws = torch.empty((nbytes + 3) // 4, device=f1.device, dtype=torch.float32)
            _call("pcfa_corr_pyramid_bwd", _ptr(st.dpyr), _ptr(f1), _ptr(st.f2ext), _ptr(df1), _ptr(df2), _ptr(ws),
                  ctypes.c_size_t(nbytes), B, D, H, W, st.L)
        st.dpyr = None
        st.token_grad = None
        st.coords_bwd = None
        return df1, df2, None


def _token_grad(st, device):
    if st.token_grad is None:
        st.token_grad = torch.zeros(1, device=device, dtype=torch.float32)
        return st.token_grad
    return None


class _CorrLookup(torch.autograd.Function):
    @staticmethod
    def forward(ctx, token, coords, state):
        if coords.requires_grad and torch.is_grad_enabled():
            raise RuntimeError("CorrBlock lookup: coords.requires_grad is not supported (detach the coordinates, as "
                               "models/raft/raft.py:122-123 does)")
        lib = _hip.load()
        st = state
        c = coords.contiguous()
        n1 = 2 * st.r + 1
        out = torch.empty((st.B, st.L * n1 * n1, st.H, st.W), device=c.device, dtype=torch.float32)
        _call("pcfa_corr_lookup_fwd", _ptr(st.pyr), _ptr(c), _ptr(out), st.B, st.H, st.W, st.L, st.r)
        ctx.state = st
        ctx.save_for_backward(c)
        return out

    @staticmethod
    def backward(ctx, grad_out):
        st = ctx.state
        (c,) = ctx.saved_tensors
        lib = _hip.load()
        if st.dpyr is None:
            st.dpyr = torch.zeros_like(st.pyr)
            st.coords_bwd = []
        st.coords_bwd.append(c)
        g = grad_out.contiguous()
        _call("pcfa_corr_lookup_bwd", _ptr(st.dpyr), _ptr(c), _ptr(g), st.B, st.H, st.W, st.L, st.r)
        return _token_grad(st, g.device), None, None


def _convc1_packed(weight):
    def make(w):
        cout = w.shape[0]
        w = w.reshape(cout, -1).contiguous()
        packed = torch.empty(int(_hip.load().pcfa_lookup_convc1_packed_floats(cout)), device=w.device, dtype=torch.float32)
        _call("pcfa_lookup_convc1_pack_weights", _ptr(w), _ptr(packed), cout, w.shape[1])
        return packed
    return cached_pack("convc1", (weight,), make)


class _CorrLookupConv(torch.autograd.Function):

    @staticmethod
    def forward(ctx, token, coords, state, weight, bias, relu):
        if coords.requires_grad and torch.is_grad_enabled():
            raise RuntimeError("CorrBlock lookup: coords.requires_grad is not supported (detach the coordinates, as "
                               "models/raft/raft.py:122-123 does)")
        st = state
        c = coords.contiguous()
        packed = _convc1_packed(weight)
        out = torch.empty((st.B, weight.shape[0], st.H, st.W), device=c.device, dtype=torch.float32)
        _call("pcfa_lookup_convc1_fwd", _ptr(st.pyr), _ptr(c), _ptr(packed), _ptr(bias), _ptr(out), st.B, st.H, st.W,
              st.L, st.r, weight.shape[0], int(relu))
        ctx.state, ctx.packed, ctx.relu, ctx.cout = st, packed, int(relu), weight.shape[0]
        ctx.save_for_backward(c, out)
        return out

    @staticmethod
    def backward(ctx, grad_out):
        if ctx.needs_input_grad[3] or ctx.needs_input_grad[4]:
            raise RuntimeError("lookup_conv is the frozen-weight path: no weight / bias gradient")
        st = ctx.state
        c, out = ctx.saved_tensors
        if st.dpyr is None:
            st.dpyr = torch.zeros_like(st.pyr)
            st.coords_bwd = []
        st.coords_bwd.append(c)
        g = grad_out.contiguous()
        _call("pcfa_lookup_convc1_bwd", _ptr(st.dpyr), _ptr(c), _ptr(ctx.packed), _ptr(out), _ptr(g), st.B, st.H, st.W,
              st.L, st.r, ctx.cout, ctx.relu)
        return _token_grad(st, g.device), None, None, None, None, None


class CorrBlock:

    def __init__(self, fmap1, fmap2, num_levels=4, radius=4, bwd_windows=True, mfma="f32"):
        _dev(fmap1, fmap2)
        if mfma not in ("f32", "bf16x3"):
            raise ValueError("CorrBlock: mfma must be 'f32' or 'bf16x3', got %r" % (mfma,))
        if fmap1.shape != fmap2.shape or fmap1.dim() != 4:
            raise ValueError("CorrBlock expects two [B,D,H,W] feature maps of equal shape")
        lib = _hip.load()
        self.num_levels = num_levels
        self.radius = radius
        st = _CorrState()
        st.B, st.D, st.H, st.W = fmap1.shape
        st.L, st.r = num_levels, radius
        st.slab = lib.pcfa_corr_slab_floats(st.H, st.W, num_levels)
        if st.slab <= 0 or (st.H >> (num_levels - 1)) < 1 or (st.W >> (num_levels - 1)) < 1:
            raise ValueError("feature map %dx%d too small for %d pyramid levels" % (st.H, st.W, num_levels))
        st.dpyr = None
        st.token_grad = None
        st.coords_bwd = None
        st.bwd_windows = bool(bwd_windows)
        st.mfma = mfma
        self._state = st
        self._token = _CorrBuild.apply(fmap1, fmap2, st)

    def __call__(self, coords):
        _dev(coords)
        return _CorrLookup.apply(self._token, coords, self._state)

    def lookup_conv_relu(self, coords, weight, bias, relu=True):
        if (self.num_levels != 4 or self.radius != 4 or bias is None or weight.dim() != 4
                or tuple(weight.shape) != (256, 324, 1, 1) or weight.requires_grad or bias.requires_grad):
            return None
        _dev(coords, weight, bias)
        return _CorrLookupConv.apply(self._token, coords, self._state, weight, bias, relu)

    @property
    def corr_pyramid(self):
        st = self._state
        return [st.pyr[:, idx.to(st.pyr.device)].reshape(-1, 1, h, w)
                for (idx, h, w) in tiled_index_maps(st.H, st.W, st.L)]


class _OnDemandState:
    __slots__ = ("B", "D", "H", "W", "L", "r", "ws", "token_grad", "accumulating", "suffix")


class _OnDemandBuild(torch.autograd.Function):

    @staticmethod
    def forward(ctx, fmap1, fmap2, state):
        lib = _hip.load()
        st = state
        f1 = fmap1.contiguous()
        f2 = fmap2.contiguous()
        nbytes = int(lib.pcfa_corr_ondemand_workspace_bytes(st.B, st.D, st.H, st.W, st.L))
        st.ws = torch.empty(nbytes, device=f1.device, dtype=torch.uint8)
        _call("pcfa_corr_ondemand_prepare", _ptr(f1), _ptr(f2), _ptr(st.ws), st.B, st.D, st.H, st.W, st.L)
        ctx.state = st
        ctx.shape = f1.shape
        return torch.zeros(1, device=f1.device, dtype=torch.float32)

    @staticmethod
    def backward(ctx, grad_token):
        st = ctx.state
        if not st.accumulating:
            z = torch.zeros(ctx.shape, device=st.ws.device, dtype=torch.float32)
            st.token_grad = None
            return z, z.clone(), None
        df1 = torch.empty(ctx.shape, device=st.ws.device, dtype=torch.float32)
        df2 = torch.empty_like(df1)
        _call("pcfa_corr_ondemand_finish", _ptr(st.ws), _ptr(df1), _ptr(df2), st.B, st.D, st.H, st.W, st.L)
        st.accumulating = False
        st.token_grad = None
        return df1, df2, None


class _OnDemandLookup(torch.autograd.Function):
    @staticmethod
    def forward(ctx, token, coords, state):
        st = state
        c = coords.contiguous()
        n1 = 2 * st.r + 1
        out = torch.empty((st.B, st.L * n1 * n1, st.H, st.W), device=c.device, dtype=torch.float32)
        _call("pcfa_corr_ondemand_fwd" + st.suffix, _ptr(st.ws), _ptr(c), _ptr(out), st.B, st.D, st.H, st.W, st.L, st.r)
        ctx.state = st
        ctx.save_for_backward(c)
        return out

    @staticmethod
    def backward(ctx, grad_out):
        st = ctx.state
        (c,) = ctx.saved_tensors
        g = grad_out.contiguous()
        _call("pcfa_corr_ondemand_bwd" + st.suffix, _ptr(st.ws), _ptr(c), _ptr(g), int(st.accumulating), st.B, st.D, st.H, st.W,
              st.L, st.r)
        st.accumulating = True
        return _token_grad(st, g.device), None, None


class OnDemandCorrBlock:

    def __init__(self, fmap1, fmap2, num_levels=4, radius=4, lookup="per_query"):
        _dev(fmap1, fmap2)
        if lookup not in ("per_query", "tiled"):
            raise ValueError("OnDemandCorrBlock: lookup must be 'per_query' or 'tiled', got %r" % (lookup,))
        if fmap1.shape != fmap2.shape or fmap1.dim() != 4:
            raise ValueError("OnDemandCorrBlock expects two [B,D,H,W] feature maps of equal shape")
        lib = _hip.load()
        self.num_levels = num_levels
        self.radius = radius
        st = _OnDemandState()
        st.B, st.D, st.H, st.W = fmap1.shape
        st.L, st.r = num_levels, radius
        if (st.H >> (num_levels - 1)) < 1 or (st.W >> (num_levels - 1)) < 1:
            raise ValueError("feature map %dx%d too small for %d pyramid levels" % (st.H, st.W, num_levels))
        if lib.pcfa_corr_ondemand_workspace_bytes(st.B, st.D, st.H, st.W, num_levels) == 0 or not 1 <= radius <= 4:
            raise ValueError("OnDemandCorrBlock: D=%d, %d levels, radius %d not served (D %% 4 == 0, D <= 512, radius 1..4)"
                             % (st.D, num_levels, radius))
        st.token_grad = None
        st.accumulating = False
        st.suffix = "_tiled" if lookup == "tiled" else ""
        self._state = st
        self._token = _OnDemandBuild.apply(fmap1, fmap2, st)

    def __call__(self, coords):
        _dev(coords)
        if coords.requires_grad and torch.is_grad_enabled():
            raise RuntimeError("OnDemandCorrBlock lookup: coords.requires_grad is not supported (detach the coordinates, "
                               "as models/raft/raft.py:122-123 does)")
        return _OnDemandLookup.apply(self._token, coords, self._state)

    def lookup_conv_relu(self, coords, weight, bias, relu=True):
        return None


def tiled_index_maps(H, W, num_levels):
    out, off, h, w = [], 0, H, W
    for _ in range(num_levels):
        tw = (w + 3) // 4
        ys, xs = torch.meshgrid(torch.arange(h), torch.arange(w), indexing="ij")
        idx = off + ((ys // 4) * tw + xs // 4) * 16 + (ys % 4) * 4 + xs % 4
        out.append((idx.reshape(-1), h, w))
        off += ((h + 3) // 4) * tw * 16
        h, w = h // 2, w // 2
    return out
```

### pcfa_amd/ops/gru.py

```python
import ctypes
import os
import weakref

import torch

from .. import _hip
from . import core
from .core import _call, _dev, _note_work, _pair, _ptr, _ptr_off, _stream
from .conv import _sepconv5_packed, _SepConv5


def _plane_channels(t):
    return t.shape[-2] * t.shape[-1], t.shape[-3]


class _GruGates(torch.autograd.Function):
    @staticmethod
    def forward(ctx, zc, rc, h, bias_z, bias_r, add_z, add_r):
        _dev(zc, rc, h, bias_z, bias_r, add_z, add_r)
        zc, rc, h = zc.contiguous(), rc.contiguous(), h.contiguous()
        az = None if add_z is None else add_z.contiguous()
        ar = None if add_r is None else add_r.contiguous()
        z, r, rh = torch.empty_like(zc), torch.empty_like(zc), torch.empty_like(zc)
        plane, C = _plane_channels(zc)
        _call("pcfa_gru_gates_fwd", _ptr(zc), _ptr(rc), _ptr(h), _ptr(bias_z), _ptr(bias_r), _ptr(az), _ptr(ar),
              _ptr(z), _ptr(r), _ptr(rh), zc.numel(), plane, C)
        ctx.save_for_backward(z, r, h)
        ctx.has_add = (add_z is not None, add_r is not None)
        return z, rh

    @staticmethod
    def backward(ctx, dz, drh):
        z, r, h = ctx.saved_tensors
        dz = torch.zeros_like(z) if dz is None else dz.contiguous()
        drh = torch.zeros_like(z) if drh is None else drh.contiguous()
        dzc, drc, dh = torch.empty_like(z), torch.empty_like(z), torch.empty_like(z)
        _call("pcfa_gru_gates_bwd", _ptr(z), _ptr(r), _ptr(h), _ptr(dz), _ptr(drh), _ptr(dzc), _ptr(drc), _ptr(dh),
              z.numel())
        return dzc, drc, dh, None, None, (dzc if ctx.has_add[0] else None), (drc if ctx.has_add[1] else None)


class _GruGatesPacked(torch.autograd.Function):

    @staticmethod
    def forward(ctx, zr, h, bias_zr, add_zr):
        _dev(zr, h, bias_zr, add_zr)
        zr, h = zr.contiguous(), h.contiguous()
        add = None if add_zr is None else add_zr.contiguous()
        B, C2, H, W = zr.shape
        C, plane = C2 // 2, H * W
        z, r, rh = torch.empty_like(h), torch.empty_like(h), torch.empty_like(h)
        bz = None if bias_zr is None else bias_zr[:C]
        br = None if bias_zr is None else bias_zr[C:]
        n = C * plane
        for b in range(B):
            o, oz = b * n, b * 2 * n
            _call("pcfa_gru_gates_fwd", _ptr_off(zr, oz), _ptr_off(zr, oz + n), _ptr_off(h, o), _ptr(bz), _ptr(br),
                  _ptr_off(add, oz), _ptr_off(add, oz + n), _ptr_off(z, o), _ptr_off(r, o), _ptr_off(rh, o), n,
                  plane, C)
        ctx.save_for_backward(z, r, h)
        ctx.has_add = add_zr is not None
        return z, rh

    @staticmethod
    def backward(ctx, dz, drh):
        z, r, h = ctx.saved_tensors
        B, C, H, W = z.shape
        n = C * H * W
        dz = torch.zeros_like(z) if dz is None else dz.contiguous()
        drh = torch.zeros_like(z) if drh is None else drh.contiguous()
        dzr = torch.empty((B, 2 * C, H, W), device=z.device, dtype=torch.float32)
        dh = torch.empty_like(z)
        for b in range(B):
            o, oz = b * n, b * 2 * n
            _call("pcfa_gru_gates_bwd", _ptr_off(z, o), _ptr_off(r, o), _ptr_off(h, o), _ptr_off(dz, o),
                  _ptr_off(drh, o), _ptr_off(dzr, oz), _ptr_off(dzr, oz + n), _ptr_off(dh, o), n)
        return dzr, dh, None, (dzr if ctx.has_add else None)


class _GruUpdate(torch.autograd.Function):
    @staticmethod
    def forward(ctx, z, qc, h, bias_q, add_q):
        _dev(z, qc, h, bias_q, add_q)
        z, qc, h = z.contiguous(), qc.contiguous(), h.contiguous()
        aq = None if add_q is None else add_q.contiguous()
        q, hnew = torch.empty_like(z), torch.empty_like(z)
        plane, C = _plane_channels(z)
        _call("pcfa_gru_update_fwd", _ptr(z), _ptr(qc), _ptr(h), _ptr(bias_q), _ptr(aq), _ptr(q), _ptr(hnew),
              z.numel(), plane, C)
        ctx.save_for_backward(z, q, h)
        ctx.has_add = add_q is not None
        return hnew

    @staticmethod
    def backward(ctx, g):
        z, q, h = ctx.saved_tensors
        g = g.contiguous()
        dz, dqc, dh = torch.empty_like(z), torch.empty_like(z), torch.empty_like(z)
        _call("pcfa_gru_update_bwd", _ptr(z), _ptr(q), _ptr(h), _ptr(g), _ptr(dz), _ptr(dqc), _ptr(dh), z.numel())
        return dz, dqc, dh, None, (dqc if ctx.has_add else None)


class _BiasRelu(torch.autograd.Function):
    @staticmethod
    def forward(ctx, x, bias):
        _dev(x, bias)
        x = x.contiguous()
        out = torch.empty_like(x)
        plane, C = _plane_channels(x)
        _call("pcfa_bias_relu_fwd", _ptr(x), _ptr(bias), _ptr(out), x.numel(), plane, C)
        ctx.save_for_backward(out)
        return out

    @staticmethod
    def backward(ctx, g):
        (out,) = ctx.saved_tensors
        g = g.contiguous()
        gx = torch.empty_like(out)
        _call("pcfa_relu_bwd", _ptr(out), _ptr(g), _ptr(gx), out.numel())
        return gx, None


_GRU_EPILOGUES = os.environ.get("PCFA_GRU_EPILOGUES", "1") != "0"


class _GruStep(torch.autograd.Function):

    @staticmethod
    def forward(ctx, h, rest, w_zr1, p_zr1, w_q1, p_q1, w_zr2, p_zr2, w_q2, p_q2, rest_relu_channels=0):
        _dev(h, rest, w_zr1, p_zr1, w_q1, p_q1, w_zr2, p_zr2, w_q2, p_q2)
        h, rest = h.contiguous(), rest.contiguous()
        B, C, H, W = h.shape
        Cr = rest.shape[1]
        n, plane = C * H * W, H * W
        new = lambda c: torch.empty((B, c, H, W), device=h.device, dtype=torch.float32)
        saved, packs = [], []
        for w_zr, p_zr, w_q, p_q in ((w_zr1, p_zr1, w_q1, p_q1), (w_zr2, p_zr2, w_q2, p_q2)):
            if tuple(w_zr.shape[:2]) != (2 * C, C + Cr) or tuple(w_q.shape[:2]) != (C, C + Cr):
                raise ValueError("gru_step: weights %s / %s do not fit h %s, rest %s"
                                 % (tuple(w_zr.shape), tuple(w_q.shape), tuple(h.shape), tuple(rest.shape)))
            vertical = int(w_zr.shape[2] == 5)
            f_zr, b_zr = _sepconv5_packed(w_zr)
            f_q, b_q = _sepconv5_packed(w_q)
            p_zr, p_q = p_zr.contiguous(), p_q.contiguous()
            z, r, rh, q, hnew = new(C), new(C), new(C), new(C), new(C)
            if C % 32 == 0 and _GRU_EPILOGUES:
                _call("pcfa_sepconv5_gru_gates_fwd", _ptr(h), C, _ptr(rest), Cr, _ptr(f_zr), _ptr(p_zr), _ptr(z), _ptr(r),
                      _ptr(rh), B, H, W, vertical)
                _call("pcfa_sepconv5_gru_update_fwd", _ptr(rh), C, _ptr(rest), Cr, _ptr(f_q), _ptr(p_q), _ptr(z), _ptr(h),
                      _ptr(q), _ptr(hnew), B, H, W, vertical)
            else:
                zr, qc = new(2 * C), new(C)
                _call("pcfa_sepconv5_fwd", _ptr(h), C, _ptr(rest), Cr, _ptr(f_zr), _ptr(zr), B, 2 * C, H, W, vertical)
                for b in range(B):
                    o, oz = b * n, b * 2 * n
                    _call("pcfa_gru_gates_fwd", _ptr_off(zr, oz), _ptr_off(zr, oz + n), _ptr_off(h, o), None, None,
                          _ptr_off(p_zr, oz), _ptr_off(p_zr, oz + n), _ptr_off(z, o), _ptr_off(r, o), _ptr_off(rh, o),
                          n, plane, C)
                _call("pcfa_sepconv5_fwd", _ptr(rh), C, _ptr(rest), Cr, _ptr(f_q), _ptr(qc), B, C, H, W, vertical)
                _call("pcfa_gru_update_fwd", _ptr(z), _ptr(qc), _ptr(h), None, _ptr(p_q), _ptr(q), _ptr(hnew),
                      z.numel(), plane, C)
            saved += [z, r, q, h]
            packs.append((b_zr, b_q, vertical))
            h = hnew
        ctx.rest_relu = int(rest_relu_channels)
        if not 0 <= ctx.rest_relu <= Cr:
            raise ValueError("gru_step: rest_relu_channels %d outside [0, %d]" % (ctx.rest_relu, Cr))
        ctx.save_for_backward(*saved, *((rest,) if ctx.rest_relu else ()))
        ctx.packs, ctx.dims = packs, (B, C, Cr, H, W)
        return h

    @staticmethod
    def backward(ctx, g):
        if any(ctx.needs_input_grad[i] for i in (2, 4, 6, 8)):
            raise RuntimeError("gru_step is the frozen-weight path: no weight gradient")
        B, C, Cr, H, W = ctx.dims
        n = C * H * W
        new = lambda c: torch.empty((B, c, H, W), device=g.device, dtype=torch.float32)
        g = g.contiguous()
        d_rest = new(Cr)
        grads_p = [None, None, None, None]
        if C % 32 == 0 and _GRU_EPILOGUES:
            z1, r1, q1, h1 = ctx.saved_tensors[4:8]
            z0, r0, q0, h0 = ctx.saved_tensors[0:4]
            (b_zr1, b_q1, v1), (b_zr0, b_q0, v0) = ctx.packs[1], ctx.packs[0]
            dz1, dqc1, dh1, dzr1 = new(C), new(C), new(C), new(2 * C)
            _call("pcfa_gru_update_bwd", _ptr(z1), _ptr(q1), _ptr(h1), _ptr(g), _ptr(dz1), _ptr(dqc1), _ptr(dh1), z1.numel())
            _call("pcfa_sepconv5_gru_gates_bwd", _ptr(dqc1), C, Cr, _ptr(b_q1), _ptr(z1), _ptr(r1), _ptr(h1), _ptr(dz1),
                  _ptr(dh1), _ptr(dzr1), _ptr(dh1), _ptr(d_rest), 0, B, H, W, v1)
            dz0, dqc0, dh0, dzr0 = new(C), new(C), new(C), new(2 * C)
            _call("pcfa_sepconv5_gru_update_bwd", _ptr(dzr1), C, Cr, _ptr(b_zr1), _ptr(dh1), _ptr(z0), _ptr(q0), _ptr(h0),
                  _ptr(dz0), _ptr(dqc0), _ptr(dh0), _ptr(d_rest), B, H, W, v1)
            _call("pcfa_sepconv5_gru_gates_bwd", _ptr(dqc0), C, Cr, _ptr(b_q0), _ptr(z0), _ptr(r0), _ptr(h0), _ptr(dz0),
                  _ptr(dh0), _ptr(dzr0), _ptr(dh0), _ptr(d_rest), 1, B, H, W, v0)
            if ctx.rest_relu:
                _call("pcfa_sepconv5_fwd_split_masked", _ptr(dzr0), 2 * C, None, 0, _ptr(b_zr0), _ptr(dh0), C, 1,
                      _ptr(d_rest), 1, _ptr(ctx.saved_tensors[8]), ctx.rest_relu, B, C + Cr, H, W, v0)
            else:
                _call("pcfa_sepconv5_fwd_split", _ptr(dzr0), 2 * C, None, 0, _ptr(b_zr0), _ptr(dh0), C, 1, _ptr(d_rest), 1,
                      B, C + Cr, H, W, v0)
            return dh0, d_rest, None, dzr0, None, dqc0, None, dzr1, None, dqc1, None
        rest_started = 0
        for half in (1, 0):
            z, r, q, h = ctx.saved_tensors[4 * half: 4 * half + 4]
            b_zr, b_q, vertical = ctx.packs[half]
            dz, dqc, dh, drh, dzr = new(C), new(C), new(C), new(C), new(2 * C)
            _call("pcfa_gru_update_bwd", _ptr(z), _ptr(q), _ptr(h), _ptr(g), _ptr(dz), _ptr(dqc), _ptr(dh), z.numel())
            _call("pcfa_sepconv5_fwd_split", _ptr(dqc), C, None, 0, _ptr(b_q), _ptr(drh), C, 0, _ptr(d_rest),
                  rest_started, B, C + Cr, H, W, vertical)
            rest_started = 1
            for b in range(B):
                o, oz = b * n, b * 2 * n
                _call("pcfa_gru_gates_bwd_acc", _ptr_off(z, o), _ptr_off(r, o), _ptr_off(h, o), _ptr_off(dz, o),
                      _ptr_off(drh, o), _ptr_off(dh, o), _ptr_off(dzr, oz), _ptr_off(dzr, oz + n), _ptr_off(dh, o), n)
            if half == 0 and ctx.rest_relu:
                _call("pcfa_sepconv5_fwd_split_masked", _ptr(dzr), 2 * C, None, 0, _ptr(b_zr), _ptr(dh), C, 1,
                      _ptr(d_rest), 1, _ptr(ctx.saved_tensors[8]), ctx.rest_relu, B, C + Cr, H, W, vertical)
            else:
                _call("pcfa_sepconv5_fwd_split", _ptr(dzr), 2 * C, None, 0, _ptr(b_zr), _ptr(dh), C, 1, _ptr(d_rest), 1,
                      B, C + Cr, H, W, vertical)
            grads_p[2 * half], grads_p[2 * half + 1] = dzr, dqc
            g = dh
        return g, d_rest, None, grads_p[0], None, grads_p[1], None, grads_p[2], None, grads_p[3], None


class _Fanout(torch.autograd.Function):

    @staticmethod
    def forward(ctx, x, n):
        ctx.set_materialize_grads(False)
        return tuple(x.view_as(x) for _ in range(n))

    @staticmethod
    def backward(ctx, *grads):
        live = [g.contiguous() for g in grads if g is not None]
        if not live:
            return None, None
        if len(live) == 1:
            return live[0], None
        _dev(*live)
        out = torch.empty_like(live[0])
        for i in range(0, len(live), 15):
            part = ([out] if i else []) + live[i:i + 15]
            arr = (ctypes.c_void_p * len(part))(*[t.data_ptr() for t in part])
            _call("pcfa_sum_n", arr, len(part), _ptr(out), out.numel())
        return out, None


class _ConvexUpsample(torch.autograd.Function):
    @staticmethod
    def forward(ctx, flow, mask):
        _dev(flow, mask)
        N, C, H, W = flow.shape
        if C != 2 or tuple(mask.shape) != (N, 576, H, W):
            raise ValueError("convex_upsample: flow %s / mask %s (expected [N,2,H,W] and [N,576,H,W])"
                             % (tuple(flow.shape), tuple(mask.shape)))
        flow, mask = flow.contiguous(), mask.contiguous()
        out = torch.empty((N, 2, 8 * H, 8 * W), device=flow.device, dtype=torch.float32)
        _call("pcfa_convex_upsample_fwd", _ptr(flow), _ptr(mask), _ptr(out), N, H, W)
        ctx.save_for_backward(flow, mask)
        return out

    @staticmethod
    @torch.autograd.function.once_differentiable
    def backward(ctx, g):
        flow, mask = ctx.saved_tensors
        N, _, H, W = flow.shape
        g = g.contiguous()
        gflow, gmask = torch.empty_like(flow), torch.empty_like(mask)
        ws = torch.empty(int(_hip.load().pcfa_convex_upsample_workspace_floats(N, H, W)), device=g.device,
                         dtype=torch.float32)
        _call("pcfa_convex_upsample_bwd", _ptr(flow), _ptr(mask), _ptr(g), _ptr(gflow), _ptr(gmask), _ptr(ws), N, H, W)
        return gflow, gmask


def convex_upsample(flow, mask):
    return _ConvexUpsample.apply(flow, mask)


class _FlowStep(torch.autograd.Function):
    @staticmethod
    def forward(ctx, coords1, delta, coords0):
        _dev(coords1, delta, coords0)
        if not (coords1.shape == delta.shape == coords0.shape):
            raise ValueError("flow_step: shapes differ: %s %s %s" % (tuple(coords1.shape), tuple(delta.shape),
                                                                     tuple(coords0.shape)))
        c1, d, c0 = coords1.contiguous(), delta.contiguous(), coords0.contiguous()
        c1n, fl = torch.empty_like(c1), torch.empty_like(c1)
        _call("pcfa_flow_step", _ptr(c1), _ptr(d), _ptr(c0), _ptr(c1n), _ptr(fl), c1.numel())
        ctx.set_materialize_grads(False)
        return c1n, fl

    @staticmethod
    def backward(ctx, g1, g2):
        g = g1 if g2 is None else g2 if g1 is None else g1 + g2
        return (g if ctx.needs_input_grad[0] else None, g if ctx.needs_input_grad[1] else None,
                (None if g is None else -g) if ctx.needs_input_grad[2] else None)


def flow_step(coords1, delta, coords0):
    return _FlowStep.apply(coords1, delta, coords0)


def fanout(x, n):
    return _Fanout.apply(x, n) if n > 1 else (x,)


def gru_step(h, rest, halves, rest_relu_channels=0):
    (a, b, c, d), (e, f, g_, i_) = halves
    return _GruStep.apply(h, rest, a, b, c, d, e, f, g_, i_, int(rest_relu_channels))


def sepconv5(a, b, weight):
    return _SepConv5.apply(a, b, weight)


def gru_gates_packed(zr, h, bias_zr=None, add_zr=None):
    return _GruGatesPacked.apply(zr, h, bias_zr, add_zr)


def gru_gates(zc, rc, h, bias_z=None, bias_r=None, add_z=None, add_r=None):
    return _GruGates.apply(zc, rc, h, bias_z, bias_r, add_z, add_r)


def gru_update(z, qc, h, bias_q=None, add_q=None):
    return _GruUpdate.apply(z, qc, h, bias_q, add_q)


def bias_relu(x, bias=None):
    return _BiasRelu.apply(x, bias)
```

Measured before the change: 7.562 attack_steps/s.

## Batch RAFT motion-encoder backward convs across all GRU iterations

Adds a MotionSteps path that stores each iteration's motion-encoder activations and upstream gradients into per-iteration slabs. The backward pass then runs the 3x3 conv input-gradient convs once, batched over all iterations, through a new strided conv3x3 entry point, instead of issuing small per-iteration launches. The GRU backward writes d_rest straight into the slab to avoid a copy. This trades extra memory for the slabs and a flush-token autograd structure for fewer, larger launches with better GPU occupancy.

```diff
diff --git a/include/pcfa_hip.h b/include/pcfa_hip.h
--- a/include/pcfa_hip.h
+++ b/include/pcfa_hip.h
@@ -263,6 +263,10 @@
 PCFA_API int pcfa_conv3x3_run(const float* x, const float* packed, const float* bias, const float* mask,
                      const float* addend, float* out, int B, int K, int N, int H, int W, int act, float slope,
                      int mask_channels, void* workspace, size_t workspace_bytes, void* stream);
+PCFA_API int pcfa_conv3x3_run_strided(const float* x, long long x_img_stride, const float* packed, const float* bias,
+                     const float* mask, long long mask_img_stride, const float* addend, long long addend_img_stride,
+                     float* out, long long out_img_stride, int B, int K, int N, int H, int W, int act, float slope,
+                     int mask_channels, void* workspace, size_t workspace_bytes, void* stream);
 
 PCFA_API int pcfa_bias_relu_fwd(const float* x, const float* bias, float* out, long long n, int plane, int channels,
                        void* stream);
diff --git a/pcfa_amd/_hip.py b/pcfa_amd/_hip.py
--- a/pcfa_amd/_hip.py
+++ b/pcfa_amd/_hip.py
@@ -123,6 +123,8 @@
     "pcfa_conv3x3_algo": (c_int, [c_int] * 5),
     "pcfa_conv3x3_workspace_bytes": (c_size_t, [c_int] * 5),
     "pcfa_conv3x3_run": (c_int, [_P] * 6 + [c_int] * 6 + [c_float, c_int, _P, c_size_t, _P]),
+    "pcfa_conv3x3_run_strided": (c_int, [_P, c_longlong, _P, _P, _P, c_longlong, _P, c_longlong, _P, c_longlong]
+                                 + [c_int] * 6 + [c_float, c_int, _P, c_size_t, _P]),
     "pcfa_conv3x3_packed_floats": (c_longlong, [c_int, c_int]),
     "pcfa_conv3x3_pack_weights": (c_int, [_P, _P, _P, c_int, c_int, _P]),
     "pcfa_conv3x3_fwd": (c_int, [_P, _P, _P, _P, c_int, c_int, c_int, c_int, c_int, c_int, _P]),
diff --git a/pcfa_amd/config.py b/pcfa_amd/config.py
--- a/pcfa_amd/config.py
+++ b/pcfa_amd/config.py
@@ -21,6 +21,7 @@
     conv1x1: str = "lib"
     corr: str = "all_pairs"
     ondemand_lookup: str = "per_query"
+    motion_bwd: str = "batched"
     mfma: str = "f32"
     dilated_as_subgrids: tuple = (2, 4, 8, 16)
     deconv_fewout: bool = True
@@ -43,6 +44,7 @@
                    conv1x1=os.environ.get("PCFA_CONV1X1", "lib"),
                    corr=os.environ.get("PCFA_CORR", "all_pairs"),
                    ondemand_lookup=os.environ.get("PCFA_ONDEMAND_LOOKUP", "per_query"),
+                   motion_bwd=os.environ.get("PCFA_MOTION_BWD", "batched"),
                    mfma=os.environ.get("PCFA_MFMA", "f32"),
                    spynet_ops=os.environ.get("PCFA_SPYNET_OPS", "lib"),
                    flownet2_ops=os.environ.get("PCFA_FLOWNET2_OPS", "lib"),
@@ -59,6 +61,8 @@
             raise ValueError("Config.corr must be 'all_pairs' or 'on_demand', got %r" % (self.corr,))
         if self.ondemand_lookup not in ("per_query", "tiled"):
             raise ValueError("Config.ondemand_lookup must be 'per_query' or 'tiled', got %r" % (self.ondemand_lookup,))
+        if self.motion_bwd not in ("batched", "per_iteration"):
+            raise ValueError("Config.motion_bwd must be 'batched' or 'per_iteration', got %r" % (self.motion_bwd,))
         if self.mfma not in ("f32", "bf16x3"):
             raise ValueError("Config.mfma must be 'f32' or 'bf16x3', got %r" % (self.mfma,))
         if self.spynet_ops not in ("lib", "hip"):
diff --git a/pcfa_amd/csrc/conv3x3.hip b/pcfa_amd/csrc/conv3x3.hip
--- a/pcfa_amd/csrc/conv3x3.hip
+++ b/pcfa_amd/csrc/conv3x3.hip
@@ -71,6 +71,7 @@
   int ksl;
   int cper;
   PcfaXcdMap xcd;
+  long long x_img, out_img, mask_img, addend_img;
 };
 
 template <int ACT, int CBT, int MT, bool KFULL, int NRING, int KS = 1>
@@ -117,10 +118,10 @@
   if (n0 >= N) return;
   const long long plane = (long long)H * W;
   const int ksl = second.ksl, img = blockIdx.z / ksl, slice = blockIdx.z - img * ksl;
-  x += (long long)img * K * plane;
-  out += ((long long)slice * (gridDim.z / ksl) + img) * N * plane;
-  if (mask != nullptr) mask += (long long)img * N * plane;
-  if (addend != nullptr) addend += (long long)img * N * plane;
+  x += (long long)img * second.x_img;
+  out += ((long long)slice * (gridDim.z / ksl) + img) * second.out_img;
+  if (mask != nullptr) mask += (long long)img * second.mask_img;
+  if (addend != nullptr) addend += (long long)img * second.addend_img;
 
   unsigned praw[RAW_LOADS];
   int rdst[RAW_LOADS];
@@ -436,7 +437,8 @@
 static int conv3x3_launch(const float* x, const float* packed, const float* bias, const float* mask, float* out, int B,
                           int K, int N, int H, int W, int act, float slope, void* stream, const float* x2 = nullptr,
                           const float* packed2 = nullptr, const float* bias2 = nullptr, float* out2 = nullptr,
-                          int K2 = 0, int N2 = 0, const float* addend = nullptr, int mask_n = 0, int ksl = 1);
+                          int K2 = 0, int N2 = 0, const float* addend = nullptr, int mask_n = 0, int ksl = 1,
+                          const long long* img_strides = nullptr);
 
 extern "C" int pcfa_conv3x3_fwd(const float* x, const float* packed, const float* bias, float* out, int B, int K,
                                 int N, int H, int W, int relu, void* stream) {
@@ -543,10 +545,31 @@
                         nullptr, 0, 0, addend, mask_channels);
 }
 
+extern "C" int pcfa_conv3x3_run_strided(const float* x, long long x_img_stride, const float* packed, const float* bias,
+                                        const float* mask, long long mask_img_stride, const float* addend,
+                                        long long addend_img_stride, float* out, long long out_img_stride, int B, int K,
+                                        int N, int H, int W, int act, float slope, int mask_channels, void* workspace,
+                                        size_t workspace_bytes, void* stream) {
+  (void)workspace;
+  (void)workspace_bytes;
+  if (!x || !packed || !out || B < 1 || K < 1 || N < 1 || H < 1 || W < 1 || act < 0 || act > 2 || mask_channels < 0 ||
+      mask_channels > N || (mask_channels > 0 && (!mask || act != 0)) || (mask && act == 2))
+    return PCFA_ERR_INVALID_ARG;
+  const long long plane = (long long)H * W;
+  if (x_img_stride < K * plane || out_img_stride < N * plane || (mask && mask_img_stride < N * plane) ||
+      (addend && addend_img_stride < N * plane))
+    return PCFA_ERR_INVALID_ARG;
+  if (use_f43(B, K, N, H, W) || f23_kslices(B, K, N, H, W) > 1 || use_f43(1, K, N, H, W) || f23_kslices(1, K, N, H, W) > 1)
+    return PCFA_ERR_UNSUPPORTED;
+  const long long strides[4] = {x_img_stride, out_img_stride, mask ? mask_img_stride : 0, addend ? addend_img_stride : 0};
+  return conv3x3_launch(x, packed, bias, mask, out, B, K, N, H, W, act, slope, stream, nullptr, nullptr, nullptr, nullptr,
+                        0, 0, addend, mask_channels, 1, strides);
+}
+
 static int conv3x3_launch(const float* x, const float* packed, const float* bias, const float* mask, float* out, int B,
                           int K, int N, int H, int W, int act, float slope, void* stream, const float* x2,
                           const float* packed2, const float* bias2, float* out2, int K2, int N2, const float* addend,
-                          int mask_n, int ksl) {
+                          int mask_n, int ksl, const long long* img_strides) {
   if (act < 0 || act > 2 || mask_n < 0 || (mask_n > 0 && (act != 0 || !mask))) return PCFA_ERR_INVALID_ARG;
   if (!x || !packed || !out || B < 1 || K < 1 || N < 1 || H < 1 || W < 1 || !aligned16(packed))
     return PCFA_ERR_INVALID_ARG;
@@ -573,14 +596,20 @@
     grid.z = (unsigned)(B * ksl);
     if (grid.z > 65535) return PCFA_ERR_UNSUPPORTED;
   }
-  Second second{x2, packed2, bias2, out2, K2, N2, (int)grid.y, mask_n, ksl, cper, PcfaXcdMap{0, 0, 0, 0}};
+  const long long dense_x = (long long)K * H * W, dense_n = (long long)N * H * W;
+  Second second{x2, packed2, bias2, out2, K2, N2, (int)grid.y, mask_n, ksl, cper, PcfaXcdMap{0, 0, 0, 0},
+                img_strides ? img_strides[0] : dense_x, img_strides ? img_strides[1] : dense_n,
+                img_strides ? img_strides[2] : dense_n, img_strides ? img_strides[3] : dense_n};
+  if (img_strides != nullptr && (ksl > 1 || x2 != nullptr)) return PCFA_ERR_INVALID_ARG;
   if (x2 != nullptr) {
     grid.y += (unsigned)((N2 + CB - 1) / CB * CB / 32);
     if (grid.y > 65535) return PCFA_ERR_UNSUPPORTED;
   }
   const long long nwg = (long long)grid.x * grid.y * grid.z;
+  const long long nwg_ks = img_strides != nullptr ? nwg / grid.z : nwg;
   static const bool xcd_on = !(getenv("PCFA_XCD_MAP") && atoi(getenv("PCFA_XCD_MAP")) == 0);
-  if (xcd_on && mt == 1 && (long long)grid.x * grid.y >= 1024) {
+  static const long long xcd_min = getenv("PCFA_XCD_MAP_MIN") ? atoll(getenv("PCFA_XCD_MAP_MIN")) : 1024;
+  if (xcd_on && mt == 1 && (long long)grid.x * grid.y >= xcd_min) {
     second.xcd = pcfa_xcd_pick((int)grid.x, (int)grid.y, 4.0 * K * H * W, 4.0 * 16 * K * 32 * grid.y);
     if (second.xcd.a != 0) {
       grid.x = pcfa_xcd_grid(second.xcd);
@@ -596,7 +625,7 @@
   } while (0)
   const bool kfull = K % KC == 0;
   static const int ks_env = getenv("PCFA_CONV3X3_KS") ? atoi(getenv("PCFA_CONV3X3_KS")) : 0;
-  if (ksl == 1 && mt == 1 && x2 == nullptr && K % (2 * KC) == 0 && (ks_env ? ks_env == 2 : nwg <= 256)) {
+  if (ksl == 1 && mt == 1 && x2 == nullptr && K % (2 * KC) == 0 && (ks_env ? ks_env == 2 : nwg_ks <= 256)) {
     block.x = 512;
     if (act == 1) pcfa_launch(conv3x3_winograd_kernel<1, 32, 1, true, 2, 2>, PCFA_C3_ARGS);
     else if (act == 2) pcfa_launch(conv3x3_winograd_kernel<2, 32, 1, true, 2, 2>, PCFA_C3_ARGS);
diff --git a/pcfa_amd/nets/raft.py b/pcfa_amd/nets/raft.py
--- a/pcfa_amd/nets/raft.py
+++ b/pcfa_amd/nets/raft.py
@@ -303,9 +303,11 @@
         fans = {tag: ops.get().fanout(p, iters) for tag, (_, p) in ctx.items()}
         return [{tag: (ctx[tag][0], fans[tag][i]) for tag in ctx} for i in range(iters)]
 
-    def step(self, h, ctx, rest, rest_relu_channels=0):
-        return ops.get().gru_step(h, rest, tuple(ctx[zr] + ctx[q] for zr, q in (("zr1", "q1"), ("zr2", "q2"))),
-                                  rest_relu_channels)
+    def step(self, h, ctx, rest, rest_relu_channels=0, d_rest_dst=None):
+        halves = tuple(ctx[zr] + ctx[q] for zr, q in (("zr1", "q1"), ("zr2", "q2")))
+        if d_rest_dst is not None:
+            return ops.get().gru_step(h, rest, halves, rest_relu_channels, d_rest_dst=d_rest_dst)
+        return ops.get().gru_step(h, rest, halves, rest_relu_channels)
 
 
 class LookupRef:
@@ -389,13 +391,26 @@
         self.mask = _mask_head()
         self._mask_cache = {}
 
-    def forward(self, net, inp, corr, flow, want_mask=True, gru_ctx=None):
-        defer = cfg(self).defer_relu and gru_ctx is not None and self.encoder.can_defer_relu(flow)
-        motion_features = self.encoder(flow, corr, defer_relu=defer)
-        if gru_ctx is not None:
-            net = self.gru.step(net, gru_ctx, motion_features, self.encoder.RELU_CHANNELS if defer else 0)
+    def motion_steps(self, corr_fn, flow, iters, gru_ctx):
+        c, enc = cfg(self), self.encoder
+        make = getattr(ops.get(), "motion_steps", None)
+        if (make is None or c.motion_bwd != "batched" or not c.defer_relu or not c.fused_lookup or c.corr == "on_demand"
+                or gru_ctx is None or not flow.is_cuda or not enc.can_defer_relu(flow)):
+            return None
+        return make(corr_fn, iters, *((m.weight, m.bias) for m in (enc.convc1, enc.convc2, enc.convf1, enc.convf2, enc.conv)))
+
+    def forward(self, net, inp, corr, flow, want_mask=True, gru_ctx=None, motion=None):
+        if motion is not None:
+            steps, itr = motion
+            net = self.gru.step(net, gru_ctx, steps.step(itr, corr.coords, flow), self.encoder.RELU_CHANNELS,
+                                d_rest_dst=steps.d_rest_dst(itr))
         else:
-            net = self.gru(net, torch.cat([inp, motion_features], dim=1))
+            defer = cfg(self).defer_relu and gru_ctx is not None and self.encoder.can_defer_relu(flow)
+            motion_features = self.encoder(flow, corr, defer_relu=defer)
+            if gru_ctx is not None:
+                net = self.gru.step(net, gru_ctx, motion_features, self.encoder.RELU_CHANNELS if defer else 0)
+            else:
+                net = self.gru(net, torch.cat([inp, motion_features], dim=1))
         delta_flow = self.flow_head(net)
         mask = mask_logits(self.mask, net, self._mask_cache) if want_mask else None
         return net, mask, delta_flow
@@ -472,13 +487,15 @@
         flow_predictions = []
         flow_up = None
         flow_cur = coords1 - coords0
+        steps = self.update_block.motion_steps(corr_fn, flow_cur, iters, gru_ctx)
         for itr in range(iters):
             coords1 = coords1.detach()
             corr = LookupRef(corr_fn, coords1)
             flow = flow_cur.detach()
             need_up = (not test_mode) or itr == iters - 1
             net, up_mask, delta_flow = self.update_block(net, inp, corr, flow, want_mask=need_up,
-                                                         gru_ctx=None if gru_ctx is None else gru_ctx[itr])
+                                                         gru_ctx=None if gru_ctx is None else gru_ctx[itr],
+                                                         motion=None if steps is None else (steps, itr))
             coords1, flow_cur = ops.get().flow_step(coords1, delta_flow, coords0)
             if need_up:
                 flow_up = convex_upsample(flow_cur, up_mask)
diff --git a/pcfa_amd/ops/conv.py b/pcfa_amd/ops/conv.py
--- a/pcfa_amd/ops/conv.py
+++ b/pcfa_amd/ops/conv.py
@@ -482,6 +482,35 @@
 _PAIR_LAUNCH = os.environ.get("PCFA_CONV3X3_PAIR", "1") != "0"
 
 
+def _conv3x3_cat_fill(xs, ws, bs, tails, buf):
+    H, W = buf.shape[2:]
+    plane = H * W
+    off, packs, fwds, offs = 0, [], [], []
+    for x, w, b in zip(xs, ws, bs):
+        if tuple(x.shape) != (1, w.shape[1], H, W) or tuple(w.shape[2:]) != (3, 3):
+            raise ValueError("conv3x3_cat: input %s does not fit weight %s" % (tuple(x.shape), tuple(w.shape)))
+        fwd, bwd = _conv3x3_packed(w)
+        fwds.append(fwd)
+        offs.append(off)
+        packs.append((bwd, w.shape[1], w.shape[0], off))
+        off += w.shape[0]
+    lib = _hip.load()
+    f23 = all(lib.pcfa_conv3x3_algo(1, w.shape[1], w.shape[0], H, W) == 23 for w in ws)
+    if len(ws) == 2 and (ws[0].shape[1] % 8 == 0) == (ws[1].shape[1] % 8 == 0) and _PAIR_LAUNCH and f23:
+        i, j = (0, 1) if ws[0].shape[0] * ws[0].shape[1] >= ws[1].shape[0] * ws[1].shape[1] else (1, 0)
+        _call("pcfa_conv3x3_act_fwd_pair", _ptr(xs[i]), _ptr(fwds[i]), _ptr(bs[i]), _ptr_off(buf, offs[i] * plane),
+              ws[i].shape[1], ws[i].shape[0], _ptr(xs[j]), _ptr(fwds[j]), _ptr(bs[j]),
+              _ptr_off(buf, offs[j] * plane), ws[j].shape[1], ws[j].shape[0], H, W, 1, 0.)
+    else:
+        for x, w, b, fwd, o_ in zip(xs, ws, bs, fwds, offs):
+            _conv3x3_run(x.device, _ptr(x), fwd, _ptr(b), None, None, _ptr_off(buf, o_ * plane), 1, w.shape[1],
+                         w.shape[0], H, W, 1, 0.)
+    for t in tails:
+        buf[:, off:off + t.shape[1]].copy_(t)
+        off += t.shape[1]
+    return packs
+
+
 class _Conv3x3Cat(torch.autograd.Function):
 
     @staticmethod
@@ -494,32 +523,9 @@
         B, _, H, W = xs[0].shape
         if B != 1:
             raise ValueError("conv3x3_cat: batch size 1 only")
-        plane = H * W
         widths = [w.shape[0] for w in ws] + [t.shape[1] for t in tails]
         buf = torch.empty((1, sum(widths), H, W), device=xs[0].device, dtype=torch.float32)
-        off, packs, fwds, offs = 0, [], [], []
-        for x, w, b in zip(xs, ws, bs):
-            if tuple(x.shape) != (1, w.shape[1], H, W) or tuple(w.shape[2:]) != (3, 3):
-                raise ValueError("conv3x3_cat: input %s does not fit weight %s" % (tuple(x.shape), tuple(w.shape)))
-            fwd, bwd = _conv3x3_packed(w)
-            fwds.append(fwd)
-            offs.append(off)
-            packs.append((bwd, w.shape[1], w.shape[0], off))
-            off += w.shape[0]
-        lib = _hip.load()
-        f23 = all(lib.pcfa_conv3x3_algo(1, w.shape[1], w.shape[0], H, W) == 23 for w in ws)
-        if n_conv == 2 and (ws[0].shape[1] % 8 == 0) == (ws[1].shape[1] % 8 == 0) and _PAIR_LAUNCH and f23:
-            i, j = (0, 1) if ws[0].shape[0] * ws[0].shape[1] >= ws[1].shape[0] * ws[1].shape[1] else (1, 0)
-            _call("pcfa_conv3x3_act_fwd_pair", _ptr(xs[i]), _ptr(fwds[i]), _ptr(bs[i]), _ptr_off(buf, offs[i] * plane),
-                  ws[i].shape[1], ws[i].shape[0], _ptr(xs[j]), _ptr(fwds[j]), _ptr(bs[j]),
-                  _ptr_off(buf, offs[j] * plane), ws[j].shape[1], ws[j].shape[0], H, W, 1, 0.)
-        else:
-            for x, w, b, fwd, o_ in zip(xs, ws, bs, fwds, offs):
-                _conv3x3_run(x.device, _ptr(x), fwd, _ptr(b), None, None, _ptr_off(buf, o_ * plane), 1, w.shape[1],
-                             w.shape[0], H, W, 1, 0.)
-        for t in tails:
-            buf[:, off:off + t.shape[1]].copy_(t)
-            off += t.shape[1]
+        packs = _conv3x3_cat_fill(xs, ws, bs, tails, buf)
         ctx.packs, ctx.dims, ctx.n_conv, ctx.tail_widths = packs, (H, W), n_conv, [t.shape[1] for t in tails]
         ctx.save_for_backward(buf, *(xs if ctx.mask_input_grads else ()))
         return buf
diff --git a/pcfa_amd/ops/corr.py b/pcfa_amd/ops/corr.py
--- a/pcfa_amd/ops/corr.py
+++ b/pcfa_amd/ops/corr.py
@@ -5,6 +5,7 @@
 
 from .. import _hip
 from . import core
+from .conv import FEWIN_SHAPES, _conv3x3_cat_fill, _conv3x3_packed, _conv3x3_run, conv_fewin
 from .core import _call, _dev, _note_work, _pair, _ptr, _ptr_off, _stream, cached_pack
 
 
@@ -149,6 +150,141 @@
         return _token_grad(st, g.device), None, None, None, None, None
 
 
+class _MotionState:
+    __slots__ = ("iters", "H", "W", "corr", "w", "cor1", "cf", "rest", "d_rest", "coords", "arrived", "token_grad", "packs")
+
+
+def _slab_image(slab, i):
+    n = slab[0].numel()
+    return torch.empty(0, device=slab.device, dtype=slab.dtype).set_(
+        slab.untyped_storage(), slab.storage_offset() + i * n, (1,) + tuple(slab.shape[1:]))
+
+
+class _MotionFlush(torch.autograd.Function):
+
+    @staticmethod
+    def forward(ctx, token, ms):
+        ctx.ms = ms
+        return token.view_as(token)
+
+    @staticmethod
+    def backward(ctx, grad_token):
+        ms = ctx.ms
+        st = ms.corr
+        live = [i for i in range(ms.iters) if ms.arrived[i]]
+        ms.arrived = [False] * ms.iters
+        ms.token_grad = None
+        if not live:
+            return None, None
+        H, W, plane = ms.H, ms.W, ms.H * ms.W
+        (bwd_c, k_c, n_c), (bwd_c2, k_c2, n_c2) = ms.packs
+        dev = ms.rest.device
+        wr = ms.rest.shape[1]
+        lib = _hip.load()
+        n = ms.iters
+        direct = lambda b, k, n_: (lib.pcfa_conv3x3_algo(b, k, n_, H, W) == 23
+                                   and lib.pcfa_conv3x3_workspace_bytes(b, k, n_, H, W) == 0)
+        batched = (len(live) == n and all(direct(b, k, n_) for b in (1, n)
+                                          for k, n_ in ((n_c, k_c), (n_c, n_c2), (n_c2, k_c2))))
+        d_cor1 = torch.empty((n, k_c2, H, W), device=dev, dtype=torch.float32)
+        if batched:
+            d_cf = torch.empty((n, n_c2, H, W), device=dev, dtype=torch.float32)
+            _call("pcfa_conv3x3_run_strided", _ptr(ms.d_rest), wr * plane, _ptr(bwd_c), None, _ptr(ms.cf), k_c * plane, None, 0,
+                  _ptr(d_cf), n_c2 * plane, n, n_c, n_c2, H, W, 0, 0., 0, None, ctypes.c_size_t(0))
+            _call("pcfa_conv3x3_run_strided", _ptr(d_cf), n_c2 * plane, _ptr(bwd_c2), None, _ptr(ms.cor1), k_c2 * plane, None, 0,
+                  _ptr(d_cor1), k_c2 * plane, n, n_c2, k_c2, H, W, 0, 0., 0, None, ctypes.c_size_t(0))
+        if st.dpyr is None:
+            st.dpyr = torch.zeros_like(st.pyr)
+            st.coords_bwd = []
+        packed = _convc1_packed(ms.w["convc1"][0])
+        for i in reversed(live):
+            if not batched:
+                d_cf = torch.empty((1, k_c, H, W), device=dev, dtype=torch.float32)
+                _conv3x3_run(dev, _ptr_off(ms.d_rest, i * wr * plane), bwd_c, None, _ptr_off(ms.cf, i * k_c * plane), None,
+                             _ptr(d_cf), 1, n_c, k_c, H, W)
+                _conv3x3_run(dev, _ptr(d_cf), bwd_c2, None, _ptr_off(ms.cor1, i * k_c2 * plane), None,
+                             _ptr_off(d_cor1, i * k_c2 * plane), 1, n_c2, k_c2, H, W)
+            st.coords_bwd.append(ms.coords[i])
+            _call("pcfa_lookup_convc1_bwd", _ptr(st.dpyr), _ptr(ms.coords[i]), _ptr(packed), _ptr_off(ms.cor1, i * k_c2 * plane),
+                  _ptr_off(d_cor1, i * k_c2 * plane), st.B, st.H, st.W, st.L, st.r, k_c2, 1)
+        return grad_token, None
+
+
+class _MotionStep(torch.autograd.Function):
+
+    @staticmethod
+    def forward(ctx, token, coords, flow, ms, i):
+        st = ms.corr
+        c = coords.contiguous()
+        (wc1, bc1), (wc2, bc2), (wf1, bf1), (wf2, bf2), (wc, bc) = (ms.w[k] for k in ("convc1", "convc2", "convf1", "convf2", "conv"))
+        cor1, cf, rest = _slab_image(ms.cor1, i), _slab_image(ms.cf, i), _slab_image(ms.rest, i)
+        _call("pcfa_lookup_convc1_fwd", _ptr(st.pyr), _ptr(c), _ptr(_convc1_packed(wc1)), _ptr(bc1), _ptr(cor1), st.B, st.H,
+              st.W, st.L, st.r, wc1.shape[0], 1)
+        flo1 = conv_fewin(flow, wf1, bf1, True)
+        _conv3x3_cat_fill([cor1, flo1.contiguous()], [wc2, wf2], [bc2, bf2], (), cf)
+        _conv3x3_cat_fill([cf], [wc], [bc], (flow,), rest)
+        ms.coords[i] = c
+        ctx.ms, ctx.i = ms, i
+        ctx.set_materialize_grads(False)
+        return rest
+
+    @staticmethod
+    def backward(ctx, g):
+        ms, i = ctx.ms, ctx.i
+        if g is None:
+            return None, None, None, None, None
+        dst = _slab_image(ms.d_rest, i)
+        if g.data_ptr() != dst.data_ptr() or not g.is_contiguous():
+            dst.copy_(g)
+        ms.arrived[i] = True
+        tg = None
+        if ms.token_grad is None:
+            tg = ms.token_grad = torch.zeros(1, device=g.device, dtype=torch.float32)
+        return tg, None, None, None, None
+
+
+class MotionSteps:
+
+    def __init__(self, ms, token):
+        self._ms, self._token = ms, token
+
+    def step(self, i, coords, flow):
+        _dev(coords, flow)
+        if coords.requires_grad and torch.is_grad_enabled():
+            raise RuntimeError("motion_steps: coords.requires_grad is not supported (detach the coordinates, as "
+                               "models/raft/raft.py:122-123 does)")
+        if flow.requires_grad and torch.is_grad_enabled():
+            raise RuntimeError("motion_steps: the flow must be detached (models/raft/raft.py:122-123)")
+        return _MotionStep.apply(self._token, coords, flow, self._ms, i)
+
+    def d_rest_dst(self, i):
+        return _slab_image(self._ms.d_rest, i)
+
+
+def motion_steps(corr_block, iters, convc1, convc2, convf1, convf2, conv):
+    if not isinstance(corr_block, CorrBlock) or iters < 1:
+        return None
+    st = corr_block._state
+    (wc1, bc1), (wc2, bc2), (wf1, bf1), (wf2, bf2), (wc, bc) = convc1, convc2, convf1, convf2, conv
+    if (st.B != 1 or st.L != 4 or st.r != 4 or bc1 is None or tuple(wc1.shape) != (256, 324, 1, 1)
+            or not corr_block._token.requires_grad
+            or any(t is None or t.requires_grad for t in (wc1, bc1, wc2, bc2, wf1, bf1, wf2, bf2, wc, bc))
+            or any(tuple(w.shape[2:]) != (3, 3) for w in (wc2, wf2, wc))
+            or (wf1.shape[1], wf1.shape[2]) not in FEWIN_SHAPES or wf1.shape[2] != wf1.shape[3]
+            or wc2.shape[1] != wc1.shape[0] or wf2.shape[1] != wf1.shape[0] or wc.shape[1] != wc2.shape[0] + wf2.shape[0]):
+        return None
+    dev = st.pyr.device
+    ms = _MotionState()
+    ms.iters, ms.H, ms.W, ms.corr = iters, st.H, st.W, st
+    ms.w = {"convc1": convc1, "convc2": convc2, "convf1": convf1, "convf2": convf2, "conv": conv}
+    new = lambda c: torch.empty((iters, c, st.H, st.W), device=dev, dtype=torch.float32)
+    ms.cor1, ms.cf = new(wc1.shape[0]), new(wc.shape[1])
+    ms.rest, ms.d_rest = new(wc.shape[0] + 2), new(wc.shape[0] + 2)
+    ms.coords, ms.arrived, ms.token_grad = [None] * iters, [False] * iters, None
+    ms.packs = ((_conv3x3_packed(wc)[1], wc.shape[1], wc.shape[0]), (_conv3x3_packed(wc2)[1], wc2.shape[1], wc2.shape[0]))
+    return MotionSteps(ms, _MotionFlush.apply(corr_block._token, ms))
+
+
 class CorrBlock:
 
     def __init__(self, fmap1, fmap2, num_levels=4, radius=4, bwd_windows=True, mfma="f32"):
diff --git a/pcfa_amd/ops/gru.py b/pcfa_amd/ops/gru.py
--- a/pcfa_amd/ops/gru.py
+++ b/pcfa_amd/ops/gru.py
@@ -127,7 +127,7 @@
 class _GruStep(torch.autograd.Function):
 
     @staticmethod
-    def forward(ctx, h, rest, w_zr1, p_zr1, w_q1, p_q1, w_zr2, p_zr2, w_q2, p_q2, rest_relu_channels=0):
+    def forward(ctx, h, rest, w_zr1, p_zr1, w_q1, p_q1, w_zr2, p_zr2, w_q2, p_q2, rest_relu_channels=0, d_rest_dst=None):
         _dev(h, rest, w_zr1, p_zr1, w_q1, p_q1, w_zr2, p_zr2, w_q2, p_q2)
         h, rest = h.contiguous(), rest.contiguous()
         B, C, H, W = h.shape
@@ -168,6 +168,10 @@
             raise ValueError("gru_step: rest_relu_channels %d outside [0, %d]" % (ctx.rest_relu, Cr))
         ctx.save_for_backward(*saved, *((rest,) if ctx.rest_relu else ()))
         ctx.packs, ctx.dims = packs, (B, C, Cr, H, W)
+        if d_rest_dst is not None and (tuple(d_rest_dst.shape) != tuple(rest.shape) or not d_rest_dst.is_contiguous()
+                                       or d_rest_dst.dtype != torch.float32 or d_rest_dst.device != rest.device):
+            raise ValueError("gru_step: d_rest_dst must be a contiguous float32 tensor of rest's shape %s" % (tuple(rest.shape),))
+        ctx.d_rest_dst = d_rest_dst
         return h
 
     @staticmethod
@@ -178,7 +182,7 @@
         n = C * H * W
         new = lambda c: torch.empty((B, c, H, W), device=g.device, dtype=torch.float32)
         g = g.contiguous()
-        d_rest = new(Cr)
+        d_rest = new(Cr) if ctx.d_rest_dst is None else ctx.d_rest_dst
         grads_p = [None, None, None, None]
         if C % 32 == 0 and _GRU_EPILOGUES:
             z1, r1, q1, h1 = ctx.saved_tensors[4:8]
@@ -199,7 +203,7 @@
             else:
                 _call("pcfa_sepconv5_fwd_split", _ptr(dzr0), 2 * C, None, 0, _ptr(b_zr0), _ptr(dh0), C, 1, _ptr(d_rest), 1,
                       B, C + Cr, H, W, v0)
-            return dh0, d_rest, None, dzr0, None, dqc0, None, dzr1, None, dqc1, None
+            return dh0, d_rest, None, dzr0, None, dqc0, None, dzr1, None, dqc1, None, None
         rest_started = 0
         for half in (1, 0):
             z, r, q, h = ctx.saved_tensors[4 * half: 4 * half + 4]
@@ -221,7 +225,7 @@
                       B, C + Cr, H, W, vertical)
             grads_p[2 * half], grads_p[2 * half + 1] = dzr, dqc
             g = dh
-        return g, d_rest, None, grads_p[0], None, grads_p[1], None, grads_p[2], None, grads_p[3], None
+        return g, d_rest, None, grads_p[0], None, grads_p[1], None, grads_p[2], None, grads_p[3], None, None
 
 
 class _Fanout(torch.autograd.Function):
@@ -306,9 +310,9 @@
     return _Fanout.apply(x, n) if n > 1 else (x,)
 
 
-def gru_step(h, rest, halves, rest_relu_channels=0):
+def gru_step(h, rest, halves, rest_relu_channels=0, d_rest_dst=None):
     (a, b, c, d), (e, f, g_, i_) = halves
-    return _GruStep.apply(h, rest, a, b, c, d, e, f, g_, i_, int(rest_relu_channels))
+    return _GruStep.apply(h, rest, a, b, c, d, e, f, g_, i_, int(rest_relu_channels), d_rest_dst)
 
 
 def sepconv5(a, b, weight):
```

After: 7.771 attack_steps/s, median of 6. +2.8%, better.
